# yjh0410/YOLO-Nano

Measured on NVIDIA B200. Metric: images/sec YOLO-Nano-1.0x 416 bs256 fp32-parity e2e (backbone+neck+head+decode+NMS), higher is better.
Workload: dtype f32 (tcgen05 3xTF32 split, fp32 accumulate)

## Files before the change

yolo_nano_b200/csrc/common.cuh:

```cuda
#pragma once
#include <cuda_bf16.h>
#include <cuda_runtime.h>
#include <stdint.h>
#include <limits.h>
#include <stdlib.h>

#include "yolonano_b200.h"

namespace ynb {

constexpr int kNumSMs = 148;

__device__ __forceinline__ float apply_act(float v, int act) {
  if (act == YNB_ACT_RELU) return fmaxf(v, 0.0f);
  if (act == YNB_ACT_LEAKY) return v > 0.0f ? v : 0.1f * v;
  return v;
}

__device__ __forceinline__ float softmax_exp(float d) { return __expf(d); }
__device__ __forceinline__ float class_score(float sum, float obj) { return __fmul_rn(__fdiv_rn(1.0f, sum), obj); }

struct ChanMap {
  int gap_at;
  int gap;
  __host__ __device__ __forceinline__ int slot(int j) const { return j + (j >= gap_at ? gap : 0); }
};
__host__ __device__ inline ChanMap dense_map() { return ChanMap{INT_MAX, 0}; }

using bf16 = __nv_bfloat16;

__device__ __forceinline__ float4 load4(const float* p) { return *reinterpret_cast<const float4*>(p); }
__device__ __forceinline__ float4 load4(const bf16* p) {
  const uint2 u = *reinterpret_cast<const uint2*>(p);
  return make_float4(__uint_as_float(u.x << 16), __uint_as_float(u.x & 0xffff0000u), __uint_as_float(u.y << 16),
                     __uint_as_float(u.y & 0xffff0000u));
}
__device__ __forceinline__ uint32_t pack_bf16x2(float lo, float hi) {
  const __nv_bfloat162 v = __floats2bfloat162_rn(lo, hi);
  return *reinterpret_cast<const uint32_t*>(&v);
}
__device__ __forceinline__ void store4(float* p, float4 v) { *reinterpret_cast<float4*>(p) = v; }
__device__ __forceinline__ void store4(bf16* p, float4 v) {
  *reinterpret_cast<uint2*>(p) = make_uint2(pack_bf16x2(v.x, v.y), pack_bf16x2(v.z, v.w));
}
__device__ __forceinline__ float to_float(float v) { return v; }
__device__ __forceinline__ float to_float(bf16 v) { return __bfloat162float(v); }

inline int round_up(int v, int m) { return (v + m - 1) / m * m; }
inline int64_t round_up64(int64_t v, int64_t m) { return (v + m - 1) / m * m; }

struct LaunchCounter {
  int64_t n = 0;
};
extern thread_local LaunchCounter* g_counter;

__device__ __forceinline__ void pdl_trigger() { asm volatile("griddepcontrol.launch_dependents;" ::: "memory"); }
__device__ __forceinline__ void pdl_wait() { asm volatile("griddepcontrol.wait;" ::: "memory"); }

inline bool pdl_enabled() {
  static int v = -1;
  if (v < 0) v = getenv("YNB_NO_PDL") ? 0 : 1;
  return v == 1;
}

template <typename... KArgs, typename... Args>
inline cudaError_t launch_pdl(void (*kern)(KArgs...), dim3 grid, dim3 block, size_t smem, cudaStream_t st,
                              Args&&... args) {
  cudaLaunchConfig_t cfg{};
  cfg.gridDim = grid;
  cfg.blockDim = block;
  cfg.dynamicSmemBytes = smem;
  cfg.stream = st;
  cudaLaunchAttribute attr[1];
  attr[0].id = cudaLaunchAttributeProgrammaticStreamSerialization;
  attr[0].val.programmaticStreamSerializationAllowed = 1;
  cfg.attrs = attr;
  cfg.numAttrs = pdl_enabled() ? 1 : 0;
  return cudaLaunchKernelEx(&cfg, kern, static_cast<KArgs>(args)...);
}

#define YNB_COUNT_LAUNCH()                  \
  do {                                      \
    if (::ynb::g_counter) ::ynb::g_counter->n++; \
  } while (0)

}
```

yolo_nano_b200/csrc/gemm_tc.cuh:

```cuda
#pragma once
#include <cuda.h>

#include <cstring>

#include "common.cuh"
#include "ptx_sm100.cuh"

namespace ynb {

constexpr int kTcThreads = 512;
constexpr int kTcSplitWarp0 = 8, kTcProducerWarp = 12, kTcMmaWarp = 13;
constexpr int kTcProducers = 3;
constexpr int kTcBM = 128;
constexpr int kTcBK = 32;
constexpr int kTcAStageBytes = kTcBM * 128;
constexpr int kTcMaxStages = 8;
constexpr int kTcSmemBudget = 232448;
constexpr int kTcMaxMain = 4;

struct TcGemmParams {
  int num_steps;
  int chunks_per_tap;
  int is3x3;
  int mode;
  int bf16_in;
  int out_bf16;
  int num_stages;
  int w_resident;
  int64_t M;
  int64_t num_tiles;
  int H, W, TH, TW, tiles_x, tiles_y;
  int N, Npad;
  int nmain;
  int nacc;
  int merge_corr;
  int ksub;
  int presplit;
  int a2_step;
  int stack_b;
  int acc_stages;
  uint32_t tmem_cols;
  uint32_t a_box_bytes;
  float* out;
  int out_ld, out_off, out_step;
  ChanMap omap;
  const float* bias;
  int act;
  const float* pass;
  int pass_ld;
  int tma_store;
  struct Decode {
    float* boxes;
    float* scores;
    int32_t* cls;
    int G, HW;
    float stride, input_size;
    float aw[3], ah[3];
    int64_t Ntot, level_off;
  } dec;
  int* err_flag;
  long long* trace;
  int trace_cap;
};

#define YNB_TRACE(role, a, b)                                                                        \
  do {                                                                                               \
    if (p.trace != nullptr && blockIdx.x == 0) {                                                     \
      const int _lt = (int)(((long long)(a) - (long long)blockIdx.x) / (long long)gridDim.x) & 63;   \
      long long* _e = p.trace + 1 + (long long)((((role) * 64 + _lt) * 32) + ((int)(b) & 31)) * 4;   \
      _e[0] = (role); _e[1] = (a); _e[2] = (b); _e[3] = clock64();                                   \
    }                                                                                                \
  } while (0)

struct TcSmemLayout {
  uint32_t stage_bytes;
  uint32_t w_chunk_bytes;
  uint32_t w_res_off;
  uint32_t bias_off;
  uint32_t stg_off;
  uint32_t bar_off;
  uint32_t total;
};
constexpr int kTcStgBytes = 8 * 4096;

__host__ __device__ inline TcSmemLayout tc_smem_layout(int Npad, int num_steps, int num_stages, bool w_resident,
                                                       bool split) {
  TcSmemLayout L;
  L.w_chunk_bytes = (uint32_t)Npad * 128;
  uint32_t a_bytes = kTcAStageBytes * (split ? 2 : 1);
  uint32_t w_bytes = w_resident ? 0 : L.w_chunk_bytes * (split ? 2 : 1);
  L.stage_bytes = a_bytes + w_bytes;
  L.w_res_off = L.stage_bytes * num_stages;
  uint32_t w_res = w_resident ? L.w_chunk_bytes * (split ? 2 : 1) * num_steps : 0;
  L.bias_off = L.w_res_off + w_res;
  L.stg_off = L.bias_off + 1024;
  L.bar_off = L.stg_off + kTcStgBytes;
  L.total = L.bar_off + 256 + 1024;
  return L;
}

__host__ __device__ __forceinline__ uint32_t rn_tf32_bits(uint32_t u) { return (u + 0x1000u) & 0xffffe000u; }

template <bool kPass, int kDecC>
__global__ void __launch_bounds__(kTcThreads, 1)
tc_gemm_kernel(const __grid_constant__ CUtensorMap tmA, const __grid_constant__ CUtensorMap tmAlo,
               const __grid_constant__ CUtensorMap tmWhi, const __grid_constant__ CUtensorMap tmWlo,
               const __grid_constant__ CUtensorMap tmOut, const TcGemmParams p) {
  extern __shared__ __align__(16) uint8_t smem_raw[];
  uint8_t* smem = smem_raw + ((1024u - (ptx::smem_u32(smem_raw) & 1023u)) & 1023u);

  const bool split = p.mode == YNB_GEMM_TC_3XTF32;
  const int kchunk = p.bf16_in ? 64 : kTcBK;
  const int box_alo = p.presplit ? 1 : -1;
  const int box_whi = p.w_resident ? -1 : 1 + (p.presplit ? 1 : 0);
  const int box_wlo = (p.w_resident || !split) ? -1 : box_whi + 1;
  const int nboxes = 1 + (box_alo >= 0) + (box_whi >= 0) + (box_wlo >= 0);
  const int nprod = nboxes < kTcProducers ? nboxes : kTcProducers;
  const TcSmemLayout lay = tc_smem_layout(p.Npad, p.num_steps, p.num_stages, p.w_resident != 0, split);
  const uint32_t w_chunk_bytes = lay.w_chunk_bytes;
  const uint32_t a_bytes = kTcAStageBytes * (split ? 2 : 1);
  const uint32_t stage_bytes = lay.stage_bytes;
  const uint32_t w_res_bytes = lay.bias_off - lay.w_res_off;
  float* s_bias = reinterpret_cast<float*>(smem + lay.bias_off);
  uint64_t* bars = reinterpret_cast<uint64_t*>(smem + lay.bar_off);
  uint64_t* full = bars;
  uint64_t* ready = bars + kTcMaxStages;
  uint64_t* empty = bars + 2 * kTcMaxStages;
  uint64_t* tmem_full = bars + 3 * kTcMaxStages;
  uint64_t* tmem_empty = bars + 3 * kTcMaxStages + 2;
  uint64_t* w_full = bars + 3 * kTcMaxStages + 4;
  uint32_t* tmem_ptr = reinterpret_cast<uint32_t*>(bars + 3 * kTcMaxStages + 5);

  const int warp = threadIdx.x >> 5, lane = threadIdx.x & 31;
  pdl_trigger();

  if (warp == kTcProducerWarp && lane == 0) {
    ptx::prefetch_tmap(&tmA);
    if (p.presplit || p.a2_step > 0) ptx::prefetch_tmap(&tmAlo);
    ptx::prefetch_tmap(&tmWhi);
    if (split) ptx::prefetch_tmap(&tmWlo);
    if (p.tma_store) ptx::prefetch_tmap(&tmOut);
    for (int s = 0; s < p.num_stages; ++s) {
      ptx::mbar_init(&full[s], nprod);
      ptx::mbar_init(&ready[s], 4);
      ptx::mbar_init(&empty[s], 1);
    }
    for (int a = 0; a < 2; ++a) {
      ptx::mbar_init(&tmem_full[a], 1);
      ptx::mbar_init(&tmem_empty[a], 4);
    }
    ptx::mbar_init(w_full, 1);
    ptx::fence_barrier_init();
  }
  if (warp == kTcMmaWarp) {
    ptx::tmem_alloc(tmem_ptr, p.tmem_cols);
    ptx::tmem_relinquish();
  }
  if (warp < 4) {
    for (int i = threadIdx.x; i < p.Npad; i += 128) s_bias[i] = i < p.N ? __ldg(p.bias + i) : 0.0f;
  }
  ptx::tc_fence_before_sync();
  __syncthreads();
  ptx::tc_fence_after_sync();
  const uint32_t tmem_base = *tmem_ptr;

  auto stage_a = [&](int s) { return smem + (size_t)s * stage_bytes; };
  auto stage_alo = [&](int s) { return smem + (size_t)s * stage_bytes + kTcAStageBytes; };
  auto w_hi_ptr = [&](int s, int step) {
    return p.w_resident ? smem + lay.w_res_off + (size_t)step * w_chunk_bytes * (split ? 2 : 1)
                        : smem + (size_t)s * stage_bytes + a_bytes;
  };
  auto w_lo_ptr = [&](int s, int step) { return w_hi_ptr(s, step) + w_chunk_bytes; };

  const int acc_cols = p.Npad * p.nacc;
  const uint32_t step_tx = p.a_box_bytes * (p.presplit ? 2 : 1) + (p.w_resident ? 0 : w_chunk_bytes * (split ? 2 : 1));
  const bool splitters_on = split && !p.presplit;

  if (warp == kTcProducerWarp && p.w_resident && ptx::elect_one()) {
    ptx::mbar_arrive_expect_tx(w_full, w_res_bytes);
    for (int st = 0; st < p.num_steps; ++st) {
      ptx::tma_load_2d(w_hi_ptr(0, st), &tmWhi, w_full, st * kchunk, 0);
      if (split) ptx::tma_load_2d(w_lo_ptr(0, st), &tmWlo, w_full, st * kchunk, 0);
    }
  }
  pdl_wait();

  const int prole = warp == kTcProducerWarp ? 0 : (warp == 14 ? 1 : (warp == 15 ? 2 : -1));
  if (prole >= 0) {
    if (prole < nprod && ptx::elect_one()) {
      const bool do_a = 0 % nprod == prole;
      const bool do_alo = box_alo >= 0 && box_alo % nprod == prole;
      const bool do_whi = box_whi >= 0 && box_whi % nprod == prole;
      const bool do_wlo = box_wlo >= 0 && box_wlo % nprod == prole;
      const uint32_t my_tx = (do_a ? p.a_box_bytes : 0u) + (do_alo ? p.a_box_bytes : 0u) +
                             (do_whi ? w_chunk_bytes : 0u) + (do_wlo ? w_chunk_bytes : 0u);
      int s = 0;
      uint32_t ph = 0;
      bool ok = true;
      for (int64_t tile = blockIdx.x; tile < p.num_tiles && ok; tile += gridDim.x) {
        int b = 0, y0 = 0, x0 = 0;
        if (p.is3x3) {
          int per_img = p.tiles_x * p.tiles_y;
          b = (int)(tile / per_img);
          int r = (int)(tile - (int64_t)b * per_img);
          y0 = (r / p.tiles_x) * p.TH;
          x0 = (r % p.tiles_x) * p.TW;
        }
        for (int st = 0; st < p.num_steps; ++st) {
          ok = ptx::mbar_wait(&empty[s], ph ^ 1, p.err_flag, 1);
          if (!ok) break;
          ptx::mbar_arrive_expect_tx(&full[s], my_tx);
          if (p.is3x3) {
            int tap = st / p.chunks_per_tap, kc = st - tap * p.chunks_per_tap;
            int dy = tap / 3, dx = tap - dy * 3;
            if (do_a) ptx::tma_load_4d(stage_a(s), &tmA, &full[s], kc * kchunk, x0 + dx - 1, y0 + dy - 1, b);
            if (do_alo) ptx::tma_load_4d(stage_alo(s), &tmAlo, &full[s], kc * kchunk, x0 + dx - 1, y0 + dy - 1, b);
          } else {
            if (do_a) {
              const bool second = p.a2_step > 0 && st >= p.a2_step;
              ptx::tma_load_2d(stage_a(s), second ? &tmAlo : &tmA, &full[s], (second ? st - p.a2_step : st) * kchunk,
                               (int)(tile * kTcBM));
            }
          }
          if (do_whi) ptx::tma_load_2d(w_hi_ptr(s, st), &tmWhi, &full[s], st * kchunk, 0);
          if (do_wlo) ptx::tma_load_2d(w_lo_ptr(s, st), &tmWlo, &full[s], st * kchunk, 0);
          if (prole == 0) YNB_TRACE(1, tile, st);
          if (++s == p.num_stages) { s = 0; ph ^= 1; }
        }
      }
    }
  } else if (warp == kTcMmaWarp) {
    if (ptx::elect_one()) {
      const uint32_t idesc = ptx::make_idesc(2 , kTcBM, p.Npad);
      const uint32_t idesc2 = ptx::make_idesc(2, kTcBM, 2 * p.Npad);
      const uint32_t idesc_bf = ptx::make_idesc(1 , kTcBM, p.Npad);
      int s = 0;
      uint32_t ph = 0;
      int acc = 0;
      uint32_t acc_ph = 0;
      bool ok = true;
      if (p.w_resident) ok = ptx::mbar_wait(w_full, 0, p.err_flag, 2);
      for (int64_t tile = blockIdx.x; tile < p.num_tiles && ok; tile += gridDim.x) {
        ok = ptx::mbar_wait(&tmem_empty[acc], acc_ph ^ 1, p.err_flag, 3);
        if (!ok) break;
        ptx::tc_fence_after_sync();
        const uint32_t d_tmem = tmem_base + (uint32_t)(acc * acc_cols);
        const uint32_t c_tmem = p.merge_corr ? d_tmem : d_tmem + (uint32_t)(p.nmain * p.Npad);
        int t = 0;
        for (int st = 0; st < p.num_steps; ++st) {
          ok = ptx::mbar_wait(splitters_on ? &ready[s] : &full[s], ph, p.err_flag, 4);
          if (!ok) break;
          ptx::tc_fence_after_sync();
          const uint32_t a_hi = ptx::smem_u32(stage_a(s));
          const uint32_t a_lo = ptx::smem_u32(stage_alo(s));
          const uint32_t b_hi = ptx::smem_u32(w_hi_ptr(s, st));
          const uint32_t b_lo = ptx::smem_u32(w_lo_ptr(s, st));
          const int nk = p.ksub > 0 ? min(kTcBK / 8, p.ksub - st * (kTcBK / 8)) : kTcBK / 8;
          if (p.bf16_in) {
#pragma unroll
            for (int k = 0; k < kTcBK / 8; ++k, ++t) {
              if (k >= nk) break;
              ptx::mma_bf16_ss(d_tmem, ptx::make_sw128_kmajor_desc(a_hi + k * 32), ptx::make_sw128_kmajor_desc(b_hi + k * 32),
                               idesc_bf, t != 0);
            }
          } else if (p.stack_b) {
#pragma unroll
            for (int k = 0; k < kTcBK / 8; ++k, ++t) {
              if (k >= nk) break;
              const uint64_t db = ptx::make_sw128_kmajor_desc(b_hi + k * 32);
              ptx::mma_tf32_ss(d_tmem, ptx::make_sw128_kmajor_desc(a_hi + k * 32), db, idesc2, t != 0);
              ptx::mma_tf32_ss(c_tmem, ptx::make_sw128_kmajor_desc(a_lo + k * 32), db, idesc, 1);
            }
          } else {
#pragma unroll
            for (int k = 0; k < kTcBK / 8; ++k, ++t) {
              if (k >= nk) break;
              const uint32_t ko = k * 32;
              const uint64_t da = ptx::make_sw128_kmajor_desc(a_hi + ko);
              const uint64_t db = ptx::make_sw128_kmajor_desc(b_hi + ko);
              const int slot = t % p.nmain;
              if (split) {
                ptx::mma_tf32_ss(c_tmem, ptx::make_sw128_kmajor_desc(a_lo + ko), db, idesc, t != 0);
                ptx::mma_tf32_ss(c_tmem, da, ptx::make_sw128_kmajor_desc(b_lo + ko), idesc, 1);
              }
              ptx::mma_tf32_ss(d_tmem + (uint32_t)(slot * p.Npad), da, db, idesc,
                               (split && p.merge_corr) ? 1 : (t >= p.nmain));
            }
          }
          YNB_TRACE(3, tile, st);
          ptx::mma_commit(&empty[s]);
          if (st == p.num_steps - 1) ptx::mma_commit(&tmem_full[acc]);
          if (++s == p.num_stages) { s = 0; ph ^= 1; }
        }
        if (++acc == p.acc_stages) { acc = 0; acc_ph ^= 1; }
      }
    }
  } else if (warp >= kTcSplitWarp0 && warp < kTcSplitWarp0 + 4) {
    if (splitters_on) {
      const int t = threadIdx.x - kTcSplitWarp0 * 32;
      int s = 0;
      uint32_t ph = 0;
      bool ok = true;
      for (int64_t tile = blockIdx.x; tile < p.num_tiles && ok; tile += gridDim.x) {
        for (int st = 0; st < p.num_steps; ++st) {
          ok = ptx::mbar_wait(&full[s], ph, p.err_flag, 5);
          if (!ok) break;
          uint4* a = reinterpret_cast<uint4*>(stage_a(s));
          uint4* lo = reinterpret_cast<uint4*>(stage_alo(s));
#pragma unroll
          for (int i = 0; i < kTcAStageBytes / 16 / 128; ++i) {
            const uint4 v = a[t + i * 128];
            uint4 h, l;
            h.x = rn_tf32_bits(v.x); h.y = rn_tf32_bits(v.y); h.z = rn_tf32_bits(v.z); h.w = rn_tf32_bits(v.w);
            l.x = rn_tf32_bits(__float_as_uint(__uint_as_float(v.x) - __uint_as_float(h.x)));
            l.y = rn_tf32_bits(__float_as_uint(__uint_as_float(v.y) - __uint_as_float(h.y)));
            l.z = rn_tf32_bits(__float_as_uint(__uint_as_float(v.z) - __uint_as_float(h.z)));
            l.w = rn_tf32_bits(__float_as_uint(__uint_as_float(v.w) - __uint_as_float(h.w)));
            a[t + i * 128] = h;
            lo[t + i * 128] = l;
          }
          ptx::fence_proxy_async_smem();
          __syncwarp();
          if (lane == 0) ptx::mbar_arrive(&ready[s]);
          if (t == 0) YNB_TRACE(2, tile, st);
          if (++s == p.num_stages) { s = 0; ph ^= 1; }
        }
      }
    }
  } else if (warp < 8) {
    const int group = warp >> 2;
    const int q = warp & 3;
    const int row = q * 32 + lane;
    const bool vec = p.out_step == 1 && p.omap.gap == 0;
    const float slope = p.act == YNB_ACT_RELU ? 0.0f : (p.act == YNB_ACT_LEAKY ? 0.1f : 1.0f);
    uint8_t* sbox = smem + lay.stg_off + warp * 4096;
    const int sw = lane & 7;
    const int nloc = (int64_t)blockIdx.x < p.num_tiles
                         ? (int)((p.num_tiles - blockIdx.x + gridDim.x - 1) / gridDim.x) : 0;
    const bool share_last = kDecC == 0;
    const int col_split = min(p.Npad, ((p.Npad / 2 + 31) / 32) * 32);
    bool ok = true;
    for (int lt = 0; lt < nloc && ok; ++lt) {
      const int64_t tile = blockIdx.x + (int64_t)lt * gridDim.x;
      const int acc = p.acc_stages == 2 ? (lt & 1) : 0;
      const bool shared = share_last && lt == nloc - 1 && col_split < p.Npad;
      if (!shared && group != acc) {
        if (p.acc_stages == 1 && share_last) ok = ptx::mbar_wait(&tmem_full[0], (uint32_t)(lt & 1), p.err_flag, 7);
        continue;
      }
      const int col_begin = shared && group == 1 ? col_split : 0;
      const int col_end = shared && group == 0 ? col_split : p.Npad;
      const uint32_t acc_ph = (uint32_t)((lt / p.acc_stages) & 1);
      int64_t m;
      bool valid;
      if (p.is3x3) {
        int per_img = p.tiles_x * p.tiles_y;
        int b = (int)(tile / per_img);
        int r = (int)(tile - (int64_t)b * per_img);
        int y = (r / p.tiles_x) * p.TH + row / p.TW;
        int x = (r % p.tiles_x) * p.TW + row % p.TW;
        valid = row < p.TH * p.TW && y < p.H && x < p.W;
        m = ((int64_t)b * p.H + y) * p.W + x;
      } else {
        m = tile * kTcBM + row;
        valid = m < p.M;
      }
      const int64_t m_base = tile * kTcBM + q * 32;
      float xa[16], xb[16];
      const int rows_left = (int)min((int64_t)32, p.M - m_base);
      auto fetch_x1 = [&](int c0, int r0, float (&x)[16]) {
        const int i = c0 + lane;
        const bool col_ok = kPass && i < p.N;
        const float* src = p.pass + (m_base + r0) * (int64_t)p.pass_ld + i;
        const int nr = col_ok ? rows_left - r0 : 0;
#pragma unroll
        for (int r = 0; r < 16; ++r) x[r] = r < nr ? __ldg(src + r * p.pass_ld) : 0.0f;
      };
      if (kPass) {
        fetch_x1(col_begin, 0, xa);
        fetch_x1(col_begin, 16, xb);
      }
      if (lane == 0 && q == 0) YNB_TRACE(4, tile, group);
      ok = ptx::mbar_wait(&tmem_full[acc], acc_ph, p.err_flag, 6);
      if (!ok) break;
      ptx::tc_fence_after_sync();
      if (lane == 0 && q == 0) YNB_TRACE(6, tile, group);
      const uint32_t t_base = tmem_base + ((uint32_t)(q * 32) << 16) + (uint32_t)(acc * acc_cols);
      if constexpr (kDecC > 0) {
        constexpr int A = 3, C = kDecC, CB = (C + 15) / 16;
        auto ld16 = [&](int c0, float (&v)[16]) {
          uint32_t r[16];
          ptx::tmem_ld_32x16(t_base + c0, r);
          if (p.nacc > 1) {
            for (int a2 = 1; a2 < p.nacc; ++a2) {
              uint32_t r2[16];
              ptx::tmem_ld_32x16(t_base + (uint32_t)(a2 * p.Npad) + c0, r2);
              ptx::tmem_ld_wait();
#pragma unroll
              for (int jj = 0; jj < 16; ++jj) r[jj] = __float_as_uint(__uint_as_float(r[jj]) + __uint_as_float(r2[jj]));
            }
          }
          ptx::tmem_ld_wait();
#pragma unroll
          for (int jj = 0; jj < 16; ++jj) v[jj] = __uint_as_float(r[jj]);
        };
        float objl[A], mx[A], sum[A], tb[4 * A];
        int am[A];
        {
          float v[16];
          ld16(0, v);
#pragma unroll
          for (int a = 0; a < A; ++a) objl[a] = v[a] + s_bias[a];
          constexpr int NPADC = (A * (1 + C + 4) + 15) / 16 * 16;
          constexpr int B0 = (A + A * C) < (NPADC - 16) ? (A + A * C) : (NPADC - 16);
          constexpr int BOFF = A + A * C - B0;
          ld16(B0, v);
#pragma unroll
          for (int k = 0; k < 4 * A; ++k) tb[k] = v[BOFF + k] + s_bias[A + A * C + k];
        }
#pragma unroll
        for (int a = 0; a < A; ++a) {
          const int cbase = A + a * C;
          float m = -INFINITY;
          int arg = 0;
#pragma unroll 1
          for (int blk = 0; blk < CB; ++blk) {
            float v[16];
            ld16(cbase + blk * 16, v);
            const float* bb = s_bias + cbase + blk * 16;
#pragma unroll
            for (int jj = 0; jj < 16; ++jj) {
              const int c = blk * 16 + jj;
              const float x = v[jj] + bb[jj];
              if ((C % 16 == 0 || c < C) && x > m) { m = x; arg = c; }
            }
          }
          float sm = 0.0f;
#pragma unroll 1
          for (int blk = 0; blk < CB; ++blk) {
            float v[16];
            ld16(cbase + blk * 16, v);
            const float* bb = s_bias + cbase + blk * 16;
#pragma unroll
            for (int jj = 0; jj < 16; ++jj) {
              const int c = blk * 16 + jj;
              if (C % 16 == 0 || c < C) sm += softmax_exp((v[jj] + bb[jj]) - m);
            }
          }
          mx[a] = m; am[a] = arg; sum[a] = sm;
        }
        (void)mx;
        {
          ptx::tc_fence_before_sync();
          __syncwarp();
          if (lane == 0) ptx::mbar_arrive(&tmem_empty[acc]);
        }
        if (valid) {
          const int b = (int)(m / p.dec.HW);
          const int pix = (int)(m - (int64_t)b * p.dec.HW);
          const int gy = pix / p.dec.G, gx = pix - gy * p.dec.G;
          const int64_t o0 = (int64_t)b * p.dec.Ntot + p.dec.level_off + (int64_t)pix * A;
#pragma unroll
          for (int a = 0; a < A; ++a) {
            const float obj = 1.0f / (1.0f + expf(-objl[a]));
            const float score = class_score(sum[a], obj);
            const float tx = tb[4 * a], ty = tb[4 * a + 1], tw = tb[4 * a + 2], th = tb[4 * a + 3];
            float cx = __fmul_rn(__fadd_rn(1.0f / (1.0f + expf(-tx)), (float)gx), p.dec.stride);
            float cy = __fmul_rn(__fadd_rn(1.0f / (1.0f + expf(-ty)), (float)gy), p.dec.stride);
            float w = __fmul_rn(expf(tw), p.dec.aw[a]);
            float h = __fmul_rn(expf(th), p.dec.ah[a]);
            float hw = __fmul_rn(w, 0.5f), hh = __fmul_rn(h, 0.5f);
            float x1 = __fdiv_rn(__fsub_rn(cx, hw), p.dec.input_size);
            float y1 = __fdiv_rn(__fsub_rn(cy, hh), p.dec.input_size);
            float x2 = __fdiv_rn(__fadd_rn(cx, hw), p.dec.input_size);
            float y2 = __fdiv_rn(__fadd_rn(cy, hh), p.dec.input_size);
            reinterpret_cast<float4*>(p.dec.boxes)[o0 + a] =
                make_float4(fminf(fmaxf(x1, 0.f), 1.f), fminf(fmaxf(y1, 0.f), 1.f), fminf(fmaxf(x2, 0.f), 1.f),
                            fminf(fmaxf(y2, 0.f), 1.f));
            p.dec.scores[o0 + a] = score;
            p.dec.cls[o0 + a] = am[a];
          }
        }
        if (lane == 0 && q == 0) YNB_TRACE(5, tile, group);
        continue;
      }
      auto box_free = [&]() {
        if (p.tma_store) {
          if (ptx::elect_one()) ptx::bulk_wait_read<0>();
          __syncwarp();
        }
      };
      auto drain16 = [&](int c0, int jc) {
        uint32_t r[16];
        ptx::tmem_ld_32x16(t_base + c0, r);
        if (p.nacc == 2) {
          uint32_t r2[16];
          ptx::tmem_ld_32x16(t_base + (uint32_t)p.Npad + c0, r2);
          ptx::tmem_ld_wait();
#pragma unroll
          for (int j = 0; j < 16; ++j) r[j] = __float_as_uint(__uint_as_float(r[j]) + __uint_as_float(r2[j]));
        } else if (p.nacc > 2) {
          for (int a = 1; a < p.nacc; ++a) {
            uint32_t r2[16];
            ptx::tmem_ld_32x16(t_base + (uint32_t)(a * p.Npad) + c0, r2);
            ptx::tmem_ld_wait();
#pragma unroll
            for (int j = 0; j < 16; ++j) r[j] = __float_as_uint(__uint_as_float(r[j]) + __uint_as_float(r2[j]));
          }
        } else {
          ptx::tmem_ld_wait();
        }
        if (jc == 0) box_free();
#pragma unroll
        for (int j = 0; j < 4; ++j) {
          const float4 b4 = *reinterpret_cast<const float4*>(s_bias + c0 + 4 * j);
          float x0 = __uint_as_float(r[4 * j]) + b4.x, x1 = __uint_as_float(r[4 * j + 1]) + b4.y;
          float x2 = __uint_as_float(r[4 * j + 2]) + b4.z, x3 = __uint_as_float(r[4 * j + 3]) + b4.w;
          *reinterpret_cast<float4*>(sbox + lane * 128 + (((jc + j) ^ sw) << 4)) =
              make_float4(fmaxf(x0, x0 * slope), fmaxf(x1, x1 * slope), fmaxf(x2, x2 * slope), fmaxf(x3, x3 * slope));
        }
      };
      auto staged = [&](int r, int l) {
        return *reinterpret_cast<const float*>(sbox + r * 128 + ((((l >> 2) ^ (r & 7)) << 4) | ((l & 3) << 2)));
      };

      auto drain16_bf16 = [&](int c0, int half) {
        uint32_t r[16];
        ptx::tmem_ld_32x16(t_base + c0, r);
        ptx::tmem_ld_wait();
        if (half == 0) box_free();
        uint32_t w[8];
#pragma unroll
        for (int j = 0; j < 8; ++j) {
          float x0 = __uint_as_float(r[2 * j]) + s_bias[c0 + 2 * j], x1 = __uint_as_float(r[2 * j + 1]) + s_bias[c0 + 2 * j + 1];
          w[j] = pack_bf16x2(fmaxf(x0, x0 * slope), fmaxf(x1, x1 * slope));
        }
        uint4* dst = reinterpret_cast<uint4*>(sbox + lane * 64 + half * 32);
        dst[0] = make_uint4(w[0], w[1], w[2], w[3]);
        dst[1] = make_uint4(w[4], w[5], w[6], w[7]);
      };
      const bool bf16_box = p.out_bf16 && p.tma_store && !kPass;
      bf16* const out_bf = reinterpret_cast<bf16*>(p.out);

      for (int c0 = col_begin; c0 < col_end; c0 += 32) {
        if (bf16_box) {
          drain16_bf16(c0, 0);
          if (c0 + 16 < col_end) drain16_bf16(c0 + 16, 1);
        } else {
          drain16(c0, 0);
          if (c0 + 16 < col_end) drain16(c0 + 16, 4);
        }
        if (c0 + 32 >= col_end && !shared) {
          ptx::tc_fence_before_sync();
          __syncwarp();
          if (lane == 0) ptx::mbar_arrive(&tmem_empty[acc]);
        }
        if (!kPass && p.tma_store) {
          ptx::fence_proxy_async_smem();
          __syncwarp();
          if (ptx::elect_one()) {
            ptx::tma_store_2d(&tmOut, sbox, c0, (int)m_base);
            ptx::bulk_commit();
          }
          continue;
        }
        __syncwarp();
        const int i = c0 + lane;
        const bool col_ok = i < p.N;
        if (kPass) {
          const int nrow = col_ok ? (int)min((int64_t)32, p.M - m_base) : 0;
          float* o = p.out + m_base * p.out_ld + p.omap.slot(2 * (col_ok ? i : 0));
#pragma unroll
          for (int r = 0; r < 16; ++r, o += p.out_ld)
            if (r < nrow) *reinterpret_cast<float2*>(o) = make_float2(xa[r], staged(r, lane));
          if (c0 + 32 < col_end) fetch_x1(c0 + 32, 0, xa);
#pragma unroll
          for (int r = 16; r < 32; ++r, o += p.out_ld)
            if (r < nrow) *reinterpret_cast<float2*>(o) = make_float2(xb[r - 16], staged(r, lane));
          if (c0 + 32 < col_end) fetch_x1(c0 + 32, 16, xb);
        } else {
          const int col = vec ? p.out_off + i : p.omap.slot(p.out_off + (col_ok ? i : 0) * p.out_step);
          if (!p.is3x3) {
            const int nrow = col_ok ? (int)min((int64_t)32, p.M - m_base) : 0;
            if (p.out_bf16) {
              bf16* o = out_bf + m_base * p.out_ld + col;
#pragma unroll 8
              for (int r = 0; r < 32; ++r, o += p.out_ld)
                if (r < nrow) *o = __float2bfloat16_rn(staged(r, lane));
            } else {
              float* o = p.out + m_base * p.out_ld + col;
#pragma unroll 8
              for (int r = 0; r < 32; ++r, o += p.out_ld)
                if (r < nrow) *o = staged(r, lane);
            }
          } else {
            const int64_t off = valid ? m * p.out_ld : -1;
#pragma unroll 8
            for (int r = 0; r < 32; ++r) {
              const int64_t offr = __shfl_sync(0xffffffffu, off, r);
              if (col_ok && offr >= 0) {
                if (p.out_bf16) out_bf[offr + col] = __float2bfloat16_rn(staged(r, lane));
                else p.out[offr + col] = staged(r, lane);
              }
            }
          }
        }
        __syncwarp();
      }
      if (lane == 0 && q == 0) YNB_TRACE(5, tile, group);
    }
    __syncwarp();
    if (p.tma_store && ptx::elect_one()) ptx::bulk_wait<0>();
  }

  ptx::tc_fence_before_sync();
  __syncthreads();
  if (warp == kTcMmaWarp) {
    ptx::tc_fence_after_sync();
    ptx::tmem_dealloc(tmem_base, p.tmem_cols);
  }
}

typedef CUresult (*PFN_encodeTiled)(CUtensorMap*, CUtensorMapDataType, cuuint32_t, void*, const cuuint64_t*,
                                    const cuuint64_t*, const cuuint32_t*, const cuuint32_t*,
                                    CUtensorMapInterleave, CUtensorMapSwizzle, CUtensorMapL2promotion,
                                    CUtensorMapFloatOOBfill);

inline PFN_encodeTiled get_encode_tiled() {
  static PFN_encodeTiled fn = nullptr;
  if (!fn) {
    void* p = nullptr;
    cudaDriverEntryPointQueryResult qres;
    if (cudaGetDriverEntryPoint("cuTensorMapEncodeTiled", &p, cudaEnableDefault, &qres) == cudaSuccess &&
        qres == cudaDriverEntryPointSuccess)
      fn = reinterpret_cast<PFN_encodeTiled>(p);
  }
  return fn;
}

inline bool make_tmap_2d(CUtensorMap* m, const void* base, uint64_t k, uint64_t rows, uint64_t row_stride_elems,
                         uint32_t box_rows, bool bf16 = false) {
  PFN_encodeTiled enc = get_encode_tiled();
  if (!enc) return false;
  const uint64_t es = bf16 ? 2 : 4;
  cuuint64_t dims[2] = {k, rows};
  cuuint64_t strides[1] = {row_stride_elems * es};
  cuuint32_t box[2] = {(cuuint32_t)(128 / es), box_rows};
  cuuint32_t estr[2] = {1, 1};
  return enc(m, bf16 ? CU_TENSOR_MAP_DATA_TYPE_BFLOAT16 : CU_TENSOR_MAP_DATA_TYPE_FLOAT32, 2, const_cast<void*>(base), dims,
             strides, box, estr, CU_TENSOR_MAP_INTERLEAVE_NONE, CU_TENSOR_MAP_SWIZZLE_128B,
             CU_TENSOR_MAP_L2_PROMOTION_L2_128B, CU_TENSOR_MAP_FLOAT_OOB_FILL_NONE) == CUDA_SUCCESS;
}

inline bool make_tmap_nhwc(CUtensorMap* m, const void* base, int C, int W, int H, int B, int ld, int box_w,
                           int box_h, bool bf16 = false, bool swizzle = true) {
  PFN_encodeTiled enc = get_encode_tiled();
  if (!enc) return false;
  const uint64_t es = bf16 ? 2 : 4;
  cuuint64_t dims[4] = {(cuuint64_t)C, (cuuint64_t)W, (cuuint64_t)H, (cuuint64_t)B};
  cuuint64_t strides[3] = {(cuuint64_t)ld * es, (cuuint64_t)ld * es * W, (cuuint64_t)ld * es * W * H};
  cuuint32_t box[4] = {(cuuint32_t)(128 / es), (cuuint32_t)box_w, (cuuint32_t)box_h, 1};
  cuuint32_t estr[4] = {1, 1, 1, 1};
  return enc(m, bf16 ? CU_TENSOR_MAP_DATA_TYPE_BFLOAT16 : CU_TENSOR_MAP_DATA_TYPE_FLOAT32, 4, const_cast<void*>(base), dims,
             strides, box, estr, CU_TENSOR_MAP_INTERLEAVE_NONE,
             swizzle ? CU_TENSOR_MAP_SWIZZLE_128B : CU_TENSOR_MAP_SWIZZLE_NONE,
             CU_TENSOR_MAP_L2_PROMOTION_L2_128B, CU_TENSOR_MAP_FLOAT_OOB_FILL_NONE) == CUDA_SUCCESS;
}

inline bool make_tmap_stem_input(CUtensorMap* m, const float* x, int S, int B) {
  PFN_encodeTiled enc = get_encode_tiled();
  if (!enc || (reinterpret_cast<uintptr_t>(x) & 15u) || (S & 3)) return false;
  cuuint64_t dims[4] = {(cuuint64_t)S, (cuuint64_t)S, 3, (cuuint64_t)B};
  cuuint64_t strides[3] = {(cuuint64_t)S * 4, (cuuint64_t)S * S * 4, (cuuint64_t)S * S * 12};
  cuuint32_t box[4] = {40, 35, 3, 1};
  cuuint32_t estr[4] = {1, 1, 1, 1};
  return enc(m, CU_TENSOR_MAP_DATA_TYPE_FLOAT32, 4, const_cast<float*>(x), dims, strides, box, estr,
             CU_TENSOR_MAP_INTERLEAVE_NONE, CU_TENSOR_MAP_SWIZZLE_NONE, CU_TENSOR_MAP_L2_PROMOTION_L2_128B,
             CU_TENSOR_MAP_FLOAT_OOB_FILL_NONE) == CUDA_SUCCESS;
}

inline bool make_tmap_out(CUtensorMap* m, void* base, uint64_t cols, uint64_t rows, uint64_t ld, bool bf16 = false) {
  PFN_encodeTiled enc = get_encode_tiled();
  if (!enc) return false;
  const uint64_t es = bf16 ? 2 : 4;
  cuuint64_t dims[2] = {cols, rows};
  cuuint64_t strides[1] = {ld * es};
  cuuint32_t box[2] = {32, 32};
  cuuint32_t estr[2] = {1, 1};
  return enc(m, bf16 ? CU_TENSOR_MAP_DATA_TYPE_BFLOAT16 : CU_TENSOR_MAP_DATA_TYPE_FLOAT32, 2, base, dims, strides, box,
             estr, CU_TENSOR_MAP_INTERLEAVE_NONE, bf16 ? CU_TENSOR_MAP_SWIZZLE_NONE : CU_TENSOR_MAP_SWIZZLE_128B,
             CU_TENSOR_MAP_L2_PROMOTION_NONE, CU_TENSOR_MAP_FLOAT_OOB_FILL_NONE) == CUDA_SUCCESS;
}

struct TcWeights {
  float* hi = nullptr;
  float* lo = nullptr;
  bf16* bw = nullptr;
  int N = 0, Npad = 0, Kpad = 0;
  CUtensorMap tm_hi, tm_lo;
};

inline void split_tf32_host(float v, float* hi, float* lo) {
  uint32_t u;
  memcpy(&u, &v, 4);
  uint32_t h = rn_tf32_bits(u);
  float hf;
  memcpy(&hf, &h, 4);
  float l = v - hf;
  uint32_t lu;
  memcpy(&lu, &l, 4);
  lu = rn_tf32_bits(lu);
  memcpy(lo, &lu, 4);
  *hi = hf;
}

struct TcGemmLaunch {
  CUtensorMap tmA;
  CUtensorMap tmOut;
  const TcWeights* w = nullptr;
  CUtensorMap tmAlo;
  TcGemmParams p;
  uint32_t smem = 0;
  unsigned grid = 0;
  int dec_classes = 0;
};

inline void tc_plan_tmem(TcGemmParams& p, bool allow_merge = false) {
  const bool split = p.mode == YNB_GEMM_TC_3XTF32;
  p.merge_corr = 0;
  static const bool merge_all = getenv("YNB_TC_MERGE_ALL") != nullptr;
  if (split && ((allow_merge && p.num_steps * (kTcBK / 8) <= 16) || merge_all) && 2 * p.Npad <= 512) {
    p.merge_corr = 1;
    p.stack_b = 0;
    p.nmain = 1; p.nacc = 1; p.acc_stages = 2;
    p.tmem_cols = 32;
    while ((int)p.tmem_cols < 2 * p.Npad) p.tmem_cols <<= 1;
    return;
  }
  const int corr = split ? 1 : 0;
  int want = 1;
  if (split) {
    const int ksteps = p.num_steps * (kTcBK / 8);
    want = ksteps >= 64 ? 4 : (ksteps >= 24 ? 3 : (ksteps >= 12 ? 2 : 1));
    static const int nmain_cap = getenv("YNB_TC_NMAIN_MAX") ? atoi(getenv("YNB_TC_NMAIN_MAX")) : 1;
    if (want > nmain_cap) want = nmain_cap;
  }
  p.nmain = want;
  while (p.nmain > 1 && (p.nmain + corr) * p.Npad > 512) p.nmain--;
  p.nacc = p.nmain + corr;
  p.acc_stages = 2 * p.nacc * p.Npad <= 512 ? 2 : 1;
  if (p.acc_stages == 1 && want <= 2 && p.nmain > 1 && 2 * (p.nmain - 1 + corr) * p.Npad <= 512) {
    p.nmain--;
    p.nacc--;
    p.acc_stages = 2;
  }
  p.tmem_cols = 32;
  while ((int)p.tmem_cols < p.acc_stages * p.nacc * p.Npad) p.tmem_cols <<= 1;
  static const bool no_stack = getenv("YNB_TC_NO_STACK") != nullptr;
  p.stack_b = (split && !no_stack && p.nmain == 1 && p.nacc == 2 && 2 * p.Npad <= 256 && (2 * p.Npad) % 16 == 0) ? 1 : 0;
}

inline bool tc_plan_smem(TcGemmLaunch& L) {
  TcGemmParams& p = L.p;
  const bool split = p.mode == YNB_GEMM_TC_3XTF32;
  for (int resident = 1; resident >= 0; --resident) {
    for (int stages = kTcMaxStages; stages >= 2; --stages) {
      if (stages > p.num_steps * 4 && stages > 2) continue;
      TcSmemLayout lay = tc_smem_layout(p.Npad, p.num_steps, stages, resident != 0, split);
      static const bool res2 = getenv("YNB_TC_RES2") != nullptr;
      if (lay.total <= (uint32_t)kTcSmemBudget && (resident == 0 || stages >= 3 || p.num_steps <= 2 || res2)) {
        p.num_stages = stages;
        p.w_resident = resident;
        L.smem = lay.total;
        return true;
      }
    }
  }
  return false;
}

inline cudaError_t launch_tc_gemm(const TcGemmLaunch& L, cudaStream_t st) {
  using KernelT = void (*)(CUtensorMap, CUtensorMap, CUtensorMap, CUtensorMap, CUtensorMap, TcGemmParams);
  static const KernelT kernels[4] = {tc_gemm_kernel<false, 0>, tc_gemm_kernel<true, 0>, tc_gemm_kernel<false, 80>,
                                     tc_gemm_kernel<false, 20>};
  static bool attr_set = false;
  if (!attr_set) {
    for (KernelT k : kernels) {
      cudaError_t e = cudaFuncSetAttribute(k, cudaFuncAttributeMaxDynamicSharedMemorySize, kTcSmemBudget);
      if (e != cudaSuccess) return e;
    }
    attr_set = true;
  }
  const CUtensorMap& tmo = L.p.tma_store ? L.tmOut : L.tmA;
  KernelT kern = L.dec_classes == 80 ? kernels[2] : (L.dec_classes == 20 ? kernels[3] : kernels[L.p.pass != nullptr ? 1 : 0]);
  const CUtensorMap& tmalo = (L.p.presplit || L.p.a2_step > 0) ? L.tmAlo : L.tmA;
  cudaError_t r = launch_pdl(kern, dim3(L.grid), dim3(kTcThreads), (size_t)L.smem, st, L.tmA, tmalo, L.w->tm_hi,
                             L.w->tm_lo, tmo, L.p);
  YNB_COUNT_LAUNCH();
  return r;
}

inline void tc_pick_tile(int H, int W, int* TH, int* TW) {
  double best = -1;
  for (int tw = 4; tw <= 64 && tw <= W + 3; ++tw) {
    int th = 128 / tw;
    if (th < 1) continue;
    if (th > H) th = H;
    double eff = (double)H * W / ((double)((W + tw - 1) / tw) * ((H + th - 1) / th) * 128.0);
    if (eff > best + 1e-9) { best = eff; *TH = th; *TW = tw; }
  }
}

}
```

yolo_nano_b200/csrc/ptx_sm100.cuh:

```cuda
#pragma once
#include <cuda.h>
#include <cuda_runtime.h>
#include <stdint.h>

namespace ynb {
namespace ptx {

__device__ __forceinline__ uint32_t smem_u32(const void* p) {
  return (uint32_t)__cvta_generic_to_shared(p);
}

__device__ __forceinline__ void mbar_init(uint64_t* bar, uint32_t count) {
  asm volatile("mbarrier.init.shared::cta.b64 [%0], %1;" ::"r"(smem_u32(bar)), "r"(count));
}
__device__ __forceinline__ void fence_barrier_init() {
  asm volatile("fence.mbarrier_init.release.cluster;" ::: "memory");
}
__device__ __forceinline__ void mbar_arrive(uint64_t* bar) {
  asm volatile("mbarrier.arrive.shared::cta.b64 _, [%0];" ::"r"(smem_u32(bar)) : "memory");
}
__device__ __forceinline__ void mbar_arrive_expect_tx(uint64_t* bar, uint32_t bytes) {
  asm volatile("mbarrier.arrive.expect_tx.shared::cta.b64 _, [%0], %1;" ::"r"(smem_u32(bar)), "r"(bytes)
               : "memory");
}
__device__ __forceinline__ bool mbar_try_wait(uint64_t* bar, uint32_t parity) {
  uint32_t ok;
  asm volatile(
      "{\n\t.reg .pred p;\n\t"
      "mbarrier.try_wait.parity.shared::cta.b64 p, [%1], %2;\n\t"
      "selp.u32 %0, 1, 0, p;\n\t}"
      : "=r"(ok)
      : "r"(smem_u32(bar)), "r"(parity)
      : "memory");
  return ok != 0;
}
__device__ __forceinline__ uint64_t globaltimer_ns() {
  uint64_t t;
  asm volatile("mov.u64 %0, %%globaltimer;" : "=l"(t));
  return t;
}
__device__ __forceinline__ bool mbar_wait(uint64_t* bar, uint32_t parity, int* timeout_flag, int code) {
  uint64_t t0 = 0;
#pragma unroll 1
  for (uint32_t spin = 0;; ++spin) {
    if (mbar_try_wait(bar, parity)) return true;
    if ((spin & 4095u) == 4095u) {
      const uint64_t now = globaltimer_ns();
      if (t0 == 0) t0 = now;
      else if (now - t0 > 2000000000ull) break;
    }
  }
  if (timeout_flag) atomicCAS(timeout_flag, 0, code);
  return false;
}

__device__ __forceinline__ void fence_proxy_async_smem() {
  asm volatile("fence.proxy.async.shared::cta;" ::: "memory");
}
__device__ __forceinline__ void tc_fence_before_sync() {
  asm volatile("tcgen05.fence::before_thread_sync;" ::: "memory");
}
__device__ __forceinline__ void tc_fence_after_sync() {
  asm volatile("tcgen05.fence::after_thread_sync;" ::: "memory");
}

__device__ __forceinline__ void prefetch_tmap(const CUtensorMap* m) {
  asm volatile("prefetch.tensormap [%0];" ::"l"(reinterpret_cast<uint64_t>(m)) : "memory");
}
__device__ __forceinline__ void tma_load_2d(void* smem_dst, const CUtensorMap* m, uint64_t* bar, int c0, int c1) {
  asm volatile(
      "cp.async.bulk.tensor.2d.shared::cluster.global.mbarrier::complete_tx::bytes [%0], [%1, {%3, %4}], [%2];"
      ::"r"(smem_u32(smem_dst)), "l"(reinterpret_cast<uint64_t>(m)), "r"(smem_u32(bar)), "r"(c0), "r"(c1)
      : "memory");
}
__device__ __forceinline__ void tma_load_4d(void* smem_dst, const CUtensorMap* m, uint64_t* bar, int c0, int c1,
                                            int c2, int c3) {
  asm volatile(
      "cp.async.bulk.tensor.4d.shared::cluster.global.mbarrier::complete_tx::bytes [%0], [%1, {%3, %4, %5, %6}], [%2];"
      ::"r"(smem_u32(smem_dst)), "l"(reinterpret_cast<uint64_t>(m)), "r"(smem_u32(bar)), "r"(c0), "r"(c1),
      "r"(c2), "r"(c3)
      : "memory");
}

__device__ __forceinline__ void tma_prefetch_4d(const CUtensorMap* m, int c0, int c1, int c2, int c3) {
  asm volatile("cp.async.bulk.prefetch.tensor.4d.L2.global.tile [%0, {%1, %2, %3, %4}];"
               ::"l"(reinterpret_cast<uint64_t>(m)), "r"(c0), "r"(c1), "r"(c2), "r"(c3)
               : "memory");
}

__device__ __forceinline__ void cp_async_16(void* smem_dst, const void* gsrc, uint32_t src_bytes) {
  asm volatile("cp.async.cg.shared.global [%0], [%1], 16, %2;" ::"r"(smem_u32(smem_dst)), "l"(gsrc), "r"(src_bytes)
               : "memory");
}
__device__ __forceinline__ void cp_async_commit() { asm volatile("cp.async.commit_group;" ::: "memory"); }
__device__ __forceinline__ void cp_async_wait_all() { asm volatile("cp.async.wait_group 0;" ::: "memory"); }

__device__ __forceinline__ void tma_store_2d(const CUtensorMap* m, const void* smem_src, int c0, int c1) {
  asm volatile("cp.async.bulk.tensor.2d.global.shared::cta.bulk_group [%0, {%2, %3}], [%1];"
               ::"l"(reinterpret_cast<uint64_t>(m)), "r"(smem_u32(smem_src)), "r"(c0), "r"(c1)
               : "memory");
}
__device__ __forceinline__ void tma_store_4d(const CUtensorMap* m, const void* smem_src, int c0, int c1, int c2, int c3) {
  asm volatile("cp.async.bulk.tensor.4d.global.shared::cta.bulk_group [%0, {%2, %3, %4, %5}], [%1];"
               ::"l"(reinterpret_cast<uint64_t>(m)), "r"(smem_u32(smem_src)), "r"(c0), "r"(c1), "r"(c2), "r"(c3)
               : "memory");
}
__device__ __forceinline__ void bulk_commit() { asm volatile("cp.async.bulk.commit_group;" ::: "memory"); }
template <int N>
__device__ __forceinline__ void bulk_wait_read() {
  asm volatile("cp.async.bulk.wait_group.read %0;" ::"n"(N) : "memory");
}
template <int N>
__device__ __forceinline__ void bulk_wait() {
  asm volatile("cp.async.bulk.wait_group %0;" ::"n"(N) : "memory");
}

__device__ __forceinline__ void tmem_alloc(uint32_t* smem_result, uint32_t ncols) {
  asm volatile("tcgen05.alloc.cta_group::1.sync.aligned.shared::cta.b32 [%0], %1;" ::"r"(smem_u32(smem_result)),
               "r"(ncols)
               : "memory");
}
__device__ __forceinline__ void tmem_relinquish() {
  asm volatile("tcgen05.relinquish_alloc_permit.cta_group::1.sync.aligned;" ::: "memory");
}
__device__ __forceinline__ void tmem_dealloc(uint32_t taddr, uint32_t ncols) {
  asm volatile("tcgen05.dealloc.cta_group::1.sync.aligned.b32 %0, %1;" ::"r"(taddr), "r"(ncols) : "memory");
}

__device__ __forceinline__ uint64_t make_sw128_kmajor_desc(uint32_t smem_addr) {
  uint64_t d = 0;
  d |= (uint64_t)((smem_addr & 0x3FFFF) >> 4);
  d |= (uint64_t)1 << 16;
  d |= (uint64_t)(1024 >> 4) << 32;
  d |= (uint64_t)1 << 46;
  d |= (uint64_t)2 << 61;
  return d;
}
__host__ __device__ __forceinline__ uint32_t make_idesc(int fmt, int M, int N) {
  return (1u << 4) | ((uint32_t)fmt << 7) | ((uint32_t)fmt << 10) | ((uint32_t)(N >> 3) << 17) |
         ((uint32_t)(M >> 4) << 24);
}
__device__ __forceinline__ void mma_tf32_ss(uint32_t tmem_d, uint64_t adesc, uint64_t bdesc, uint32_t idesc,
                                            uint32_t accumulate) {
  asm volatile(
      "{\n\t.reg .pred p;\n\t"
      "setp.ne.b32 p, %4, 0;\n\t"
      "tcgen05.mma.cta_group::1.kind::tf32 [%0], %1, %2, %3, p;\n\t}"
      ::"r"(tmem_d), "l"(adesc), "l"(bdesc), "r"(idesc), "r"(accumulate)
      : "memory");
}
__device__ __forceinline__ void mma_bf16_ss(uint32_t tmem_d, uint64_t adesc, uint64_t bdesc, uint32_t idesc,
                                            uint32_t accumulate) {
  asm volatile(
      "{\n\t.reg .pred p;\n\t"
      "setp.ne.b32 p, %4, 0;\n\t"
      "tcgen05.mma.cta_group::1.kind::f16 [%0], %1, %2, %3, p;\n\t}"
      ::"r"(tmem_d), "l"(adesc), "l"(bdesc), "r"(idesc), "r"(accumulate)
      : "memory");
}
__device__ __forceinline__ void mma_commit(uint64_t* bar) {
  asm volatile("tcgen05.commit.cta_group::1.mbarrier::arrive::one.shared::cluster.b64 [%0];" ::"r"(smem_u32(bar))
               : "memory");
}

__device__ __forceinline__ void tmem_ld_32x32(uint32_t taddr, uint32_t (&r)[32]) {
  asm volatile(
      "tcgen05.ld.sync.aligned.32x32b.x32.b32 "
      "{%0, %1, %2, %3, %4, %5, %6, %7, %8, %9, %10, %11, %12, %13, %14, %15, "
      "%16, %17, %18, %19, %20, %21, %22, %23, %24, %25, %26, %27, %28, %29, %30, %31}, [%32];"
      : "=r"(r[0]), "=r"(r[1]), "=r"(r[2]), "=r"(r[3]), "=r"(r[4]), "=r"(r[5]), "=r"(r[6]), "=r"(r[7]),
        "=r"(r[8]), "=r"(r[9]), "=r"(r[10]), "=r"(r[11]), "=r"(r[12]), "=r"(r[13]), "=r"(r[14]), "=r"(r[15]),
        "=r"(r[16]), "=r"(r[17]), "=r"(r[18]), "=r"(r[19]), "=r"(r[20]), "=r"(r[21]), "=r"(r[22]), "=r"(r[23]),
        "=r"(r[24]), "=r"(r[25]), "=r"(r[26]), "=r"(r[27]), "=r"(r[28]), "=r"(r[29]), "=r"(r[30]), "=r"(r[31])
      : "r"(taddr)
      : "memory");
}
__device__ __forceinline__ void tmem_ld_32x16(uint32_t taddr, uint32_t (&r)[16]) {
  asm volatile(
      "tcgen05.ld.sync.aligned.32x32b.x16.b32 "
      "{%0, %1, %2, %3, %4, %5, %6, %7, %8, %9, %10, %11, %12, %13, %14, %15}, [%16];"
      : "=r"(r[0]), "=r"(r[1]), "=r"(r[2]), "=r"(r[3]), "=r"(r[4]), "=r"(r[5]), "=r"(r[6]), "=r"(r[7]),
        "=r"(r[8]), "=r"(r[9]), "=r"(r[10]), "=r"(r[11]), "=r"(r[12]), "=r"(r[13]), "=r"(r[14]), "=r"(r[15])
      : "r"(taddr)
      : "memory");
}
__device__ __forceinline__ void tmem_ld_wait() {
  asm volatile("tcgen05.wait::ld.sync.aligned;" ::: "memory");
}

__device__ __forceinline__ void named_bar_sync(int id, int nthreads) {
  asm volatile("bar.sync %0, %1;" ::"r"(id), "r"(nthreads) : "memory");
}

template <int N>
__device__ __forceinline__ void setmaxnreg_inc() {
  asm volatile("setmaxnreg.inc.sync.aligned.u32 %0;" ::"n"(N));
}
template <int N>
__device__ __forceinline__ void setmaxnreg_dec() {
  asm volatile("setmaxnreg.dec.sync.aligned.u32 %0;" ::"n"(N));
}

__device__ __forceinline__ bool elect_one() {
  uint32_t pred;
  asm volatile(
      "{\n\t.reg .pred p;\n\t"
      "elect.sync _|p, 0xffffffff;\n\t"
      "selp.u32 %0, 1, 0, p;\n\t}"
      : "=r"(pred));
  return pred != 0;
}

}
}
```

yolo_nano_b200/csrc/ynb_api.cu:

```cuda
#include <cuda.h>
#include <cuda_runtime.h>

#include <cmath>
#include <cstdio>
#include <cstdlib>
#include <cstring>
#include <deque>
#include <functional>
#include <map>
#include <memory>
#include <string>
#include <tuple>
#include <vector>

#include "yolonano_b200.h"

#include "common.cuh"
#include "decode_nms.cuh"
#include "nms_grid.cuh"
#include "gemm_ffma.cuh"
#include "gemm_tc.cuh"
#include "unit_tc.cuh"
#include "kernels_basic.cuh"
#include "train_ops.cuh"
// ... 257 lines not shown
  for (int i = 0; i < h; ++i) {
    const int r1 = sl.map.slot(2 * i), r2 = sl.map.slot(2 * i + 1);
    for (int k = 0; k < c1.cin; ++k) w[(size_t)r1 * ktot + il1.map.slot(k)] = p1.w_host[(size_t)i * c1.cin + k];
    for (int k = 0; k < c2.cin; ++k) w[(size_t)r2 * ktot + k1p + il2.map.slot(k)] = p2.w_host[(size_t)i * c2.cin + k];
    b[r1] = p1.b_host[i];
    b[r2] = p2.b_host[i];
  }
  const int parts = (sl.ld + 239) / 240;
  const int npart = round_up((sl.ld + parts - 1) / parts, bf ? 8 : 4);
  for (auto& cc : e->cat[si]) {
    if (cc.pc.b_dev) cudaFree(cc.pc.b_dev);
    if (cc.pc.tc.hi) cudaFree(cc.pc.tc.hi);
    if (cc.pc.tc.lo) cudaFree(cc.pc.tc.lo);
    if (cc.pc.tc.bw) cudaFree(cc.pc.tc.bw);
  }
  e->cat[si].clear();
  e->cat[si].resize(parts);
  for (int pi = 0; pi < parts; ++pi) {
    ynb_engine::CatConv& cc = e->cat[si][pi];
    cc.n0 = pi * npart;
    const int n = std::min(npart, sl.ld - cc.n0);
    cc.k1p = k1p; cc.k2p = k2p;
    cc.pc.n = n; cc.pc.ktot = ktot; cc.pc.loaded = true;
    CUDA_TRY(e, cudaMalloc(&cc.pc.b_dev, round_up(n, 4) * 4));
    CUDA_TRY(e, cudaMemset(cc.pc.b_dev, 0, round_up(n, 4) * 4));
    CUDA_TRY(e, cudaMemcpy(cc.pc.b_dev, b.data() + cc.n0, n * 4, cudaMemcpyHostToDevice));
    int rc = pack_tc_matrix(e, cc.pc.tc, w.data() + (size_t)cc.n0 * ktot, n, ktot, 1, bk + "cat");
    if (rc) return rc;
  }
  return YNB_OK;
}

int pack_conv(ynb_engine* e, int i) {
  const ConvSpec& c = e->table[i];
  PackedConv& pc = e->convs[i];
  const bool bf = is_bf16(e);
  InLayout il = in_layout(c, bf);
  std::vector<float> w, b;
  if (c.kind == kDense3x3 && c.cin == 3) {
    w.assign(27 * 24, 0.f);
    for (int co = 0; co < 24; ++co)
      for (int ci = 0; ci < 3; ++ci)
        for (int t = 0; t < 9; ++t) w[(ci * 9 + t) * 24 + co] = pc.w_host[(co * 3 + ci) * 9 + t];
    b = pc.b_host;
    pc.n = 24; pc.ktot = 27;
    memcpy(e->stem_w.w, w.data(), sizeof(e->stem_w.w));
    memcpy(e->stem_w.b, b.data(), sizeof(e->stem_w.b));
  } else if (c.kind == kDw3x3) {
    int c4 = il.ktot;
    w.assign(9 * c4, 0.f);
    b.assign(c4, 0.f);
    for (int ch = 0; ch < c.cin; ++ch) {
      int s = il.map.slot(ch);
      for (int t = 0; t < 9; ++t) w[t * c4 + s] = pc.w_host[ch * 9 + t];
      b[s] = pc.b_host[ch];
    }
    pc.n = c4; pc.ktot = 9;
  } else if (c.kind == kPw1x1) {
    w.assign((size_t)c.cout * il.ktot, 0.f);
    for (int n = 0; n < c.cout; ++n)
      for (int k = 0; k < c.cin; ++k) w[(size_t)n * il.ktot + il.map.slot(k)] = pc.w_host[(size_t)n * c.cin + k];
    b = pc.b_host;
    pc.n = c.cout; pc.ktot = il.ktot;
  } else {
    w.assign((size_t)c.cout * 9 * c.cin, 0.f);
    for (int n = 0; n < c.cout; ++n)
      for (int ci = 0; ci < c.cin; ++ci)
        for (int t = 0; t < 9; ++t)
          w[((size_t)n * 9 + t) * c.cin + ci] = pc.w_host[((size_t)n * c.cin + ci) * 9 + t];
    b = pc.b_host;
    pc.n = c.cout; pc.ktot = 9 * c.cin;
  }
  if (pc.w_dev) cudaFree(pc.w_dev);
  if (pc.b_dev) cudaFree(pc.b_dev);
  pc.w_dev = pc.b_dev = nullptr;
  CUDA_TRY(e, cudaMalloc(&pc.w_dev, w.size() * 4));
  CUDA_TRY(e, cudaMalloc(&pc.b_dev, round_up((int)b.size(), 4) * 4));
  CUDA_TRY(e, cudaMemcpy(pc.w_dev, w.data(), w.size() * 4, cudaMemcpyHostToDevice));
  CUDA_TRY(e, cudaMemset(pc.b_dev, 0, round_up((int)b.size(), 4) * 4));
  CUDA_TRY(e, cudaMemcpy(pc.b_dev, b.data(), b.size() * 4, cudaMemcpyHostToDevice));

  if ((c.kind == kPw1x1) || (c.kind == kDense3x3 && c.cin != 3)) {
    int rc = pack_tc_matrix(e, pc.tc, w.data(), pc.n, pc.ktot, c.kind == kDense3x3 ? 9 : 1, c.name);
    if (rc) return rc;
  }
  return YNB_OK;
}

struct Bump {
  size_t off = 0;
  size_t take(size_t bytes) {
    size_t o = off;
    off += (bytes + 1023) & ~(size_t)1023;
    return o;
  }
};

size_t layout_workspace(ynb_engine* e, int batch, int S, char* base) {
  Bump bump;
  const bool bf = is_bf16(e);
  const int es_act = bf ? 2 : 4, al = bf ? 8 : 4;
  auto tensor = [&](const std::string& name, int C, int ld, int H, ChanMap map = dense_map(), int es = 0) {
    Tensor t;
    t.es = es ? es : es_act;
    t.C = C; t.ld = ld; t.H = H; t.W = H; t.map = map;
    size_t o = bump.take((size_t)batch * H * H * ld * t.es);
    t.p = base ? reinterpret_cast<float*>(base + o) : nullptr;
    e->taps[name] = t;
    return t;
  };
  e->taps.clear();
  const int H1 = S / 4;
  tensor("pool", 24, 24, H1);
  int hin = H1;
  int ld_in = 24;
  ChanMap map_in = dense_map();
  for (int si = 0; si < 3; ++si) {
    int cout = stage_channels()[si + 1], h = cout / 2, cin = stage_channels()[si];
    int hout = hin / 2;
    std::string st = "stage" + std::to_string(si + 2);
    const StageLayout sl = stage_layout(bf, si);
    int ld_h = round_up(h, al);
    tensor(st + ".b1dw", cin, ld_in, hout, map_in);
    tensor(st + ".b2pw", h, ld_h, hin);
    tensor(st + ".mid1", h, ld_h, hout);
    tensor(st + ".mid2", h, ld_h, hout);
    for (int bi = 0; bi < stage_repeats()[si]; ++bi) tensor(st + "." + std::to_string(bi), cout, sl.ld, hout, sl.map);
    hin = hout;
    ld_in = sl.ld;
    map_in = sl.map;
  }
  const int H3 = S / 8, H4 = S / 16, H5 = S / 32;
  const int hs[3] = {H3, H4, H5};
  for (int l = 0; l < 3; ++l) tensor("lat" + std::to_string(l + 3), 96, 96, hs[l]);
  tensor("sum4", 96, 96, H4); tensor("sum4.lo", 96, 96, H4); tensor("fpn4", 96, 96, H4);
  tensor("sum3", 96, 96, H3); tensor("sum3.lo", 96, 96, H3); tensor("p3", 96, 96, H3);
  tensor("sum4b", 96, 96, H4); tensor("sum4b.lo", 96, 96, H4); tensor("p4", 96, 96, H4);
  tensor("sum5", 96, 96, H5); tensor("sum5.lo", 96, 96, H5); tensor("p5", 96, 96, H5);
  const int ch = e->cfg.num_anchors * (1 + e->cfg.num_classes + 4);
  const char* pn[3] = {"pred_s", "pred_m", "pred_l"};
  for (int l = 0; l < 3; ++l) {
    tensor("head" + std::to_string(l) + ".a", 96, 96, hs[l]);
    tensor("head" + std::to_string(l) + ".b", 96, 96, hs[l]);
    tensor("head" + std::to_string(l) + ".c", 96, 96, hs[l]);
    e->raw[l] = tensor(pn[l], ch, round_up(ch, 4), hs[l], dense_map(), 4);
  }
  e->taps["c3"] = e->taps["stage2.3"];
  e->taps["c4"] = e->taps["stage3.7"];
  e->taps["c5"] = e->taps["stage4.3"];

  int64_t n = 0;
  for (int s : {8, 16, 32}) n += (int64_t)e->cfg.num_anchors * (S / s) * (S / s);
  auto raw = [&](size_t bytes) { size_t o = bump.take(bytes); return base ? base + o : nullptr; };
  e->d_boxes = (float*)raw((size_t)batch * n * 16);
  e->d_scores = (float*)raw((size_t)batch * n * 4);
  e->d_cls = (int32_t*)raw((size_t)batch * n * 4);
  e->nms_ws_bytes = std::max(nms_workspace_bytes(batch, n), grid_nms_workspace_bytes(batch, n));
  e->d_nms_ws = raw((size_t)e->nms_ws_bytes);
  for (int k = 0; k < 2; ++k) {
    e->slot[k].x = (float*)raw((size_t)batch * 3 * S * S * 4);
    e->slot[k].boxes = (float*)raw((size_t)batch * n * 16);
    e->slot[k].scores = (float*)raw((size_t)batch * n * 4);
    e->slot[k].cls = (int32_t*)raw((size_t)batch * n * 4);
    e->slot[k].counts = (int32_t*)raw((size_t)batch * 4);
    e->slot[k].img_u8 = (uint8_t*)raw((size_t)batch * 3 * S * S);
    e->slot[k].rects = (int32_t*)raw((size_t)batch * 16);
  }
  e->d_x = e->slot[0].x;
  e->d_out_boxes = e->slot[0].boxes;
  e->d_out_scores = e->slot[0].scores;
  e->d_out_cls = e->slot[0].cls;
  e->d_out_counts = e->slot[0].counts;
  e->d_err = (int*)raw(256);
  return bump.off;
}

int ensure_workspace(ynb_engine* e, int batch) {
  if (e->ws && e->ws_batch >= batch && e->ws_S == e->S) return YNB_OK;
  int nb = std::max(batch, std::max(e->ws_batch, (int)e->cfg.max_batch));
  CUDA_TRY(e, cudaDeviceSynchronize());
  e->plans.clear();
  e->tc_store.clear(); e->dp_store.clear(); e->dw_maps.clear(); e->stem_maps.clear();
  for (auto& kv : e->graphs) cudaGraphExecDestroy(kv.second);
  e->graphs.clear();
  e->graph_seen.clear();
  if (e->ws) { cudaFree(e->ws); e->ws = nullptr; }
  size_t bytes = layout_workspace(e, nb, e->S, nullptr);
  CUDA_TRY(e, cudaMalloc(&e->ws, bytes));
  CUDA_TRY(e, cudaMemset(e->ws, 0, bytes));
  layout_workspace(e, nb, e->S, e->ws);
  e->ws_bytes = bytes;
  e->ws_batch = nb;
  e->ws_S = e->S;
  return YNB_OK;
}

struct Planner {
  ynb_engine* e;
  int B;
  Plan* plan;
  std::deque<TcGemmLaunch>* tc;
  std::deque<DwPwLaunch>* dp;
  std::string error;
  std::vector<Op>* dst = nullptr;
  std::vector<Op>& ops() { return dst ? *dst : plan->net; }

  const PackedConv& conv(const std::string& name) const { return e->convs[e->index.at(name)]; }
  const ConvSpec& spec(const std::string& name) const { return e->table[e->index.at(name)]; }
  Tensor T(const std::string& name) const { return e->taps.at(name); }

  void dw(const std::string& name, const Tensor& in, int in_off, const Tensor& out) {
    const PackedConv& pc = conv(name);
    const ConvSpec& c = spec(name);
    int B_ = B, c4 = pc.n, stride = c.stride, act = c.act;
    const float *w = pc.w_dev, *b = pc.b_dev;
    double px_in = (double)B * in.H * in.W, px_out = (double)B * out.H * out.W;
    const bool bf = is_bf16(e);
    const double bytes = (double)in.es * c.cin * (px_in + px_out) + 40.0 * c.cin, flops = 18.0 * c.cin * px_out;
    static const bool no_tma = getenv("YNB_DW_NO_TMA") != nullptr;
    e->dw_maps.emplace_back();
    CUtensorMap* tm = &e->dw_maps.back();
    if ((!no_tma || bf) && make_tmap_dw(tm, in.p, in.ld, in_off, B, in.H, in.W, c4, stride, bf)) {
      plan->net.push_back({name, "dwconv3x3", bytes, flops, [=](cudaStream_t st) {
        return launch_dwconv3x3_tma(*tm, out.p, out.ld, 0, w, b, B_, in.H, in.W, c4, stride, act, st, false, bf);
      }});
      return;
    }
    if (bf) { error = "bf16 depthwise conv needs a 16-byte aligned view: " + name; return; }
    plan->net.push_back({name, "dwconv3x3", bytes, flops, [=](cudaStream_t st) {
      return launch_dwconv3x3(in.p, in.ld, in_off, out.p, out.ld, 0, w, b, B_, in.H, in.W, c4, stride, act, st);
    }});
  }

  void passthrough(const std::string& name, const Tensor& x, const Tensor& out, int half) {
    int64_t M = (int64_t)B * x.H * x.W;
    Tensor ps = x, o = out;
    Op op{name + "+passthrough", "interleave_copy", 8.0 * M * half, 0.0, [=](cudaStream_t st) {
      return launch_interleave_copy(ps.p, ps.ld, o.p, o.ld, o.map, M, half, st);
    }};
    op.side = true;
    plan->net.push_back(op);
  }

  void pw(const std::string& name, const Tensor& in, int in_off, const Tensor& out, int out_off, int out_step,
          bool join = false, const Tensor* pass = nullptr, const TcGemmParams::Decode* dec = nullptr) {
    const PackedConv& pc = conv(name);
    const ConvSpec& c = spec(name);
    int64_t M = (int64_t)B * in.H * in.W;
    const bool tc_mode = e->cfg.gemm_mode != YNB_GEMM_FP32_FFMA;
    const bool bf = is_bf16(e);
    const double abytes = (double)in.es * M * c.cin + (double)out.es * M * (c.cout + (pass && tc_mode ? 2.0 * c.cout : 0.0)) +
                          (bf ? 2.0 : 4.0) * c.cin * c.cout + 4.0 * c.cout;
    const double aflops = 2.0 * M * c.cin * c.cout;
    if (e->cfg.gemm_mode == YNB_GEMM_FP32_FFMA) {
      GemmParams g{};
      g.a = in.p; g.a_ld = in.ld; g.a_off = in_off; g.a2 = nullptr; g.a2_mode = 0;
      g.w = pc.w_dev; g.bias = pc.b_dev; g.out = out.p; g.out_ld = out.ld;
      g.out_off = out_off; g.out_step = out_step; g.omap = out.map;
      g.M = M; g.N = pc.n; g.Ktot = pc.ktot; g.act = c.act;
      if (pass) { g.out_off = 1; g.out_step = 2; }
      Op op{name, "pw_ffma", abytes, aflops, [=](cudaStream_t st) { return launch_gemm_ffma(g, false, st); }};
      op.join = join;
      ops().push_back(op);
      return;
    }
    tc->emplace_back();
    TcGemmLaunch& L = tc->back();
    L.w = &pc.tc;
    TcGemmParams& p = L.p;
    memset(&p, 0, sizeof(p));
    p.mode = e->cfg.gemm_mode;
    p.is3x3 = 0;
    p.bf16_in = bf ? 1 : 0;
    p.out_bf16 = out.es == 2 ? 1 : 0;
    if (bf && pass) { error = "bf16 mode: the pass-through GEMM epilogue is not built (unit tails go through dwpw): " + name; return; }
    p.num_steps = pc.tc.Kpad / (bf ? 64 : kTcBK);
    p.chunks_per_tap = p.num_steps;
    p.ksub = bf ? (pc.ktot + 15) / 16 : (pc.ktot + 7) / 8;
    p.M = M;
    p.num_tiles = (M + kTcBM - 1) / kTcBM;
    p.N = pc.n; p.Npad = pc.tc.Npad;
    tc_plan_tmem(p, name.size() > 2 && name.compare(0, 8, "head_det") == 0 && name.compare(name.size() - 2, 2, ".4") == 0);
    p.a_box_bytes = kTcAStageBytes;
    p.out = out.p; p.out_ld = out.ld; p.out_off = out_off; p.out_step = out_step; p.omap = out.map;
    p.bias = pc.b_dev; p.act = c.act;
    p.pass = pass ? pass->p : nullptr; p.pass_ld = pass ? pass->ld : 0;
    p.err_flag = e->d_err;
    if (dec) {
      p.dec = *dec;
      L.dec_classes = e->cfg.num_classes;
    }
    const int oal = 16 / out.es;
    p.tma_store = (!dec && !pass && out_step == 1 && out.map.gap == 0 && out_off % oal == 0 && out.ld % oal == 0) ? 1 : 0;
    if (p.tma_store && !make_tmap_out(&L.tmOut, out.at(out_off), (uint64_t)round_up(pc.n, oal), (uint64_t)M,
                                      (uint64_t)out.ld, out.es == 2)) {
      error = "cuTensorMapEncodeTiled failed for output of " + name;
      return;
    }
    if (!make_tmap_2d(&L.tmA, in.at(in_off), (uint64_t)pc.ktot, (uint64_t)M, (uint64_t)in.ld, kTcBM, bf)) {
      error = "cuTensorMapEncodeTiled failed for input of " + name;
      return;
    }
    if (!tc_plan_smem(L)) { error = "no smem configuration for " + name; return; }
    L.grid = (unsigned)std::min<int64_t>(p.num_tiles, kNumSMs);
    const TcGemmLaunch* Lp = &L;
    const double obytes = dec ? abytes - (double)out.es * M * c.cout + 24.0 * M * 3 : abytes;
    Op op{dec ? name + "+decode" : name, dec ? "pw_decode_tcgen05" : "pw_tcgen05", obytes, aflops,
          [=](cudaStream_t st) { return launch_tc_gemm(*Lp, st); }};
    op.join = join;
    ops().push_back(op);
  }

  bool catpw(int si, const std::string& unit, const Tensor& b1dw, const Tensor& mid2, const Tensor& out) {
    static const bool off = getenv("YNB_NO_CAT_GEMM") != nullptr;
    if (off || e->cfg.gemm_mode == YNB_GEMM_FP32_FFMA || e->cat[si].empty()) return false;
    const bool bf = is_bf16(e);
    const int64_t M = (int64_t)B * out.H * out.W;
    const ConvSpec& c1 = spec(unit + "branch1.2");
    const ConvSpec& c2 = spec(unit + "branch2.5");
    for (size_t pi = 0; pi < e->cat[si].size(); ++pi) {
      const ynb_engine::CatConv& cc = e->cat[si][pi];
      tc->emplace_back();
      TcGemmLaunch& L = tc->back();
      L.w = &cc.pc.tc;
      TcGemmParams& p = L.p;
      memset(&p, 0, sizeof(p));
      p.mode = e->cfg.gemm_mode;
      p.bf16_in = bf ? 1 : 0;
      p.out_bf16 = out.es == 2 ? 1 : 0;
      const int ch = bf ? 64 : kTcBK;
      p.num_steps = cc.pc.tc.Kpad / ch;
      p.chunks_per_tap = p.num_steps;
      p.a2_step = cc.k1p / ch;
      p.ksub = 0;
      p.M = M;
      p.num_tiles = (M + kTcBM - 1) / kTcBM;
      p.N = cc.pc.n; p.Npad = cc.pc.tc.Npad;
      tc_plan_tmem(p);
      p.a_box_bytes = kTcAStageBytes;
      p.out = out.p; p.out_ld = out.ld; p.out_off = cc.n0; p.out_step = 1; p.omap = dense_map();
      p.bias = cc.pc.b_dev; p.act = c1.act;
      p.err_flag = e->d_err;
      p.tma_store = 1;
      const int oal = 16 / out.es;
      if (!make_tmap_out(&L.tmOut, out.at(cc.n0), (uint64_t)round_up(cc.pc.n, oal), (uint64_t)M, (uint64_t)out.ld, out.es == 2) ||
          !make_tmap_2d(&L.tmA, b1dw.p, (uint64_t)b1dw.ld, (uint64_t)M, (uint64_t)b1dw.ld, kTcBM, bf) ||
          !make_tmap_2d(&L.tmAlo, mid2.p, (uint64_t)mid2.ld, (uint64_t)M, (uint64_t)mid2.ld, kTcBM, bf)) {
        error = "cuTensorMapEncodeTiled failed for the merged stride-2 conv of " + unit;
        return true;
      }
      if (!tc_plan_smem(L)) { error = "no smem configuration for the merged stride-2 conv of " + unit; return true; }
      L.grid = (unsigned)std::min<int64_t>(p.num_tiles, kNumSMs);
      const TcGemmLaunch* Lp = &L;
      const double frac = (double)cc.pc.n / out.ld;
      const double bytes = (double)b1dw.es * M * (c1.cin + c2.cin) + (double)out.es * M * 2.0 * c1.cout * frac +
                           (bf ? 2.0 : 4.0) * (c1.cin + c2.cin) * c1.cout;
      const double flops = 2.0 * M * (c1.cin + c2.cin) * c1.cout * frac;
      ops().push_back({unit + "branch1.2|branch2.5" + (e->cat[si].size() > 1 ? "." + std::to_string(pi) : ""), "pw_tcgen05", bytes,
                       flops, [=](cudaStream_t st) { return launch_tc_gemm(*Lp, st); }});
    }
    return true;
  }

  bool dwpw(const std::string& dw_name, const std::string& pw_name, const Tensor& in, const Tensor& out,
            const Tensor* pass) {
    static const bool off = getenv("YNB_NO_FUSED_DWPW") != nullptr;
    if (off || e->cfg.gemm_mode == YNB_GEMM_FP32_FFMA) return false;
    const PackedConv& dc = conv(dw_name);
    const PackedConv& pc = conv(pw_name);
    const ConvSpec& ds = spec(dw_name);
    const ConvSpec& ps = spec(pw_name);
    if (ds.stride != 1 || dc.n != pc.ktot) return false;
    dp->emplace_back();
    DwPwLaunch& L = dp->back();
    DwPwParams& p = L.p;
    memset(&p, 0, sizeof(p));
    p.dw_w = dc.w_dev; p.dw_b = dc.b_dev; p.dw_act = ds.act;
    p.out = out.p; p.out_ld = out.ld; p.out_off = 0; p.omap = out.map;
    p.bias = pc.b_dev; p.act = ps.act;
    p.pass = pass ? pass->p : nullptr; p.pass_ld = pass ? pass->ld : 0;
    p.err_flag = e->d_err;
    if (!plan_dwpw(L, in.p, in.ld, B, in.H, in.W, ds.cin, dc.n, &pc.tc, e->cfg.gemm_mode)) {
      dp->pop_back();
      return false;
    }
    const double M = (double)B * in.H * in.W;
    const double bytes = (double)in.es * M * (ds.cin + ps.cout * (pass ? 3.0 : 1.0)) + (double)in.es * ps.cin * ps.cout +
                         4.0 * ps.cout + 40.0 * ds.cin;
    const double flops = 2.0 * M * ps.cin * ps.cout + 18.0 * M * ds.cin;
    const DwPwLaunch* Lp = &L;
    ops().push_back({dw_name + "+pw", "dwpw_tcgen05", bytes, flops,
                     [=](cudaStream_t st) { return launch_dwpw_tc(*Lp, st); }});
    return true;
  }

  void conv3(const std::string& name, const Tensor& a, const Tensor* a2, int a2_mode, const Tensor& sum,
             const Tensor& sum_lo, const Tensor& out) {
    const PackedConv& pc = conv(name);
    const ConvSpec& c = spec(name);
    int64_t M = (int64_t)B * a.H * a.W;
    const bool bf = is_bf16(e);
    const double eb = a.es;
    const double wbytes = eb * 9 * c.cin * c.cout + 4.0 * c.cout;
    const double aflops = 2.0 * M * 9 * c.cin * c.cout;
    const double a2bytes = a2 ? eb * c.cin * M * (a2_mode == 1 ? 0.25 : 1.0) : 0.0;
    if (e->cfg.gemm_mode == YNB_GEMM_FP32_FFMA) {
      GemmParams g{};
      g.a = a.p; g.a_ld = a.ld; g.a_off = 0;
      g.a2 = a2 ? a2->p : nullptr; g.a2_ld = a2 ? a2->ld : 0; g.a2_mode = a2 ? a2_mode : 0;
      g.H = a.H; g.W = a.W; g.C = c.cin;
      g.w = pc.w_dev; g.bias = pc.b_dev; g.out = out.p; g.out_ld = out.ld; g.out_off = 0; g.out_step = 1;
      g.omap = dense_map(); g.M = M; g.N = pc.n; g.Ktot = pc.ktot; g.act = c.act;
      plan->net.push_back({name, "conv3x3_ffma", 4.0 * M * (c.cin + c.cout) + a2bytes + wbytes, aflops,
                           [=](cudaStream_t st) { return launch_gemm_ffma(g, true, st); }});
      return;
    }
    Tensor src = a;
    static const bool no_presplit = getenv("YNB_TC_NO_PRESPLIT") != nullptr;
    const bool presplit = a2 != nullptr && e->cfg.gemm_mode == YNB_GEMM_TC_3XTF32 && !no_presplit;
    if (a2) {
      Tensor a_ = a, a2_ = *a2, s_ = sum, sl_ = sum_lo;
      int B_ = B;
      plan->net.push_back({name + "+merge", "resample_add", (presplit ? 3.0 : 2.0) * eb * M * c.cin + a2bytes,
                           1.0 * M * c.cin, [=](cudaStream_t st) {
        return launch_resample_add(a_.p, a2_.p, s_.p, presplit ? sl_.p : nullptr, B_, a_.H, a_.W, a_.ld, a2_mode, st, bf);
      }});
      src = sum;
    }
    tc->emplace_back();
    TcGemmLaunch& L = tc->back();
    L.w = &pc.tc;
    TcGemmParams& p = L.p;
    memset(&p, 0, sizeof(p));
    p.mode = e->cfg.gemm_mode;
    p.is3x3 = 1;
    p.bf16_in = bf ? 1 : 0;
    p.out_bf16 = out.es == 2 ? 1 : 0;
    p.chunks_per_tap = bf ? (c.cin + 63) / 64 : c.cin / kTcBK;
    p.num_steps = 9 * p.chunks_per_tap;
    p.H = a.H; p.W = a.W;
    tc_pick_tile(p.H, p.W, &p.TH, &p.TW);
    p.tiles_x = (p.W + p.TW - 1) / p.TW;
    p.tiles_y = (p.H + p.TH - 1) / p.TH;
    p.num_tiles = (int64_t)B * p.tiles_x * p.tiles_y;
    p.M = M;
    p.N = pc.n; p.Npad = pc.tc.Npad;
    tc_plan_tmem(p);
    p.a_box_bytes = (uint32_t)(p.TH * p.TW * 128);
    p.out = out.p; p.out_ld = out.ld; p.out_off = 0; p.out_step = 1; p.omap = dense_map();
    p.bias = pc.b_dev; p.act = c.act;
    p.err_flag = e->d_err;
    if (!make_tmap_nhwc(&L.tmA, src.p, c.cin, src.W, src.H, B, src.ld, p.TW, p.TH, bf) ||
        (presplit && !make_tmap_nhwc(&L.tmAlo, sum_lo.p, c.cin, src.W, src.H, B, src.ld, p.TW, p.TH))) {
      error = "cuTensorMapEncodeTiled failed for input of " + name;
      return;
    }
    p.presplit = presplit ? 1 : 0;
    if (!tc_plan_smem(L)) { error = "no smem configuration for " + name; return; }
    L.grid = (unsigned)std::min<int64_t>(p.num_tiles, kNumSMs);
    const TcGemmLaunch* Lp = &L;
    plan->net.push_back({name, "conv3x3_tcgen05", eb * M * (c.cin + c.cout) + wbytes, aflops,
                         [=](cudaStream_t st) { return launch_tc_gemm(*Lp, st); }});
  }
};

int build_plan(ynb_engine* e, int B, Plan** out) {
  auto it = e->plans.find(B);
  if (it != e->plans.end()) { *out = it->second.get(); return YNB_OK; }
  auto plan = std::make_unique<Plan>();
  plan->batch = B;
  e->tc_store.emplace_back();
  e->dp_store.emplace_back();
  Planner P{e, B, plan.get(), &e->tc_store.back(), &e->dp_store.back(), ""};
  const int S = e->S;

  {
    Tensor pool = P.T("pool");
    double px = (double)B * S * S;
    const bool bf = is_bf16(e);
    plan->net.push_back({"backbone.conv1.0+maxpool", "stem_pool", 4.0 * 3 * px + (bf ? 2.0 : 4.0) * 24 * px / 16 + 4.0 * 27 * 24,
                         2.0 * 27 * 24 * px / 4, [=](cudaStream_t st) {
      const float* xin = e->d_x_bound;
      auto key = std::make_tuple(xin, B, S);
      auto it = e->stem_maps.find(key);
      if (it == e->stem_maps.end()) {
        ynb_engine::StemMap sm{};
        sm.ok = make_tmap_stem_input(&sm.tm, xin, S, B) ? 1 : 0;
        if (e->stem_maps.size() > 64) e->stem_maps.clear();
        it = e->stem_maps.emplace(key, sm).first;
      }
      return launch_stem_pool(xin, pool.p, bf, e->stem_w, it->second.tm, it->second.ok, B, S, st);
    }});
  }
  Tensor x = P.T("pool");
  for (int si = 0; si < 3; ++si) {
    std::string st = "stage" + std::to_string(si + 2);
    std::string bk = "backbone." + st + ".";
    int h = stage_channels()[si + 1] / 2;
    Tensor b1dw = P.T(st + ".b1dw"), b2pw = P.T(st + ".b2pw"), mid1 = P.T(st + ".mid1"), mid2 = P.T(st + ".mid2");
    Tensor o0 = P.T(st + ".0");
    P.dw(bk + "0.branch1.0", x, 0, b1dw);
    if (si > 0) plan->net.back().join = true;
    P.pw(bk + "0.branch2.0", x, 0, b2pw, 0, 1);
    P.dw(bk + "0.branch2.3", b2pw, 0, mid2);
    if (!P.catpw(si, bk + "0.", b1dw, mid2, o0)) {
      P.pw(bk + "0.branch1.2", b1dw, 0, o0, 0, 2);
      P.pw(bk + "0.branch2.5", mid2, 0, o0, 1, 2);
    }
    x = o0;
    for (int bi = 1; bi < stage_repeats()[si]; ++bi) {
      std::string u = bk + std::to_string(bi);
      Tensor o = P.T(st + "." + std::to_string(bi));
      const int x2_off = x2_window(stage_layout(is_bf16(e), si), h, is_bf16(e) ? 8 : 4).off;
      const bool ffma = e->cfg.gemm_mode == YNB_GEMM_FP32_FFMA;
      P.pw(u + ".branch2.0", x, x2_off, mid1, 0, 1, ffma && bi > 1);
      if (ffma) {
        plan->net.back().mark = true;
        P.passthrough(u, x, o, h);
      }
      if (!P.dwpw(u + ".branch2.3", u + ".branch2.5", mid1, o, &x)) {
        P.dw(u + ".branch2.3", mid1, 0, mid2);
        P.pw(u + ".branch2.5", mid2, 0, o, 1, 2, false, &x);
      }
      x = o;
    }
  }
  Tensor c3 = P.T("c3"), c4 = P.T("c4"), c5 = P.T("c5");
  Tensor lat3 = P.T("lat3"), lat4 = P.T("lat4"), lat5 = P.T("lat5");
  P.pw("conv1x1_0.convs.0", c3, 0, lat3, 0, 1, true);
  P.pw("conv1x1_1.convs.0", c4, 0, lat4, 0, 1);
  P.pw("conv1x1_2.convs.0", c5, 0, lat5, 0, 1);
  Tensor fpn4 = P.T("fpn4"), p3 = P.T("p3"), p4 = P.T("p4"), p5 = P.T("p5");
  P.conv3("smooth_0.convs.0", lat4, &lat5, 1, P.T("sum4"), P.T("sum4.lo"), fpn4);
  P.conv3("smooth_1.convs.0", lat3, &fpn4, 1, P.T("sum3"), P.T("sum3.lo"), p3);
  P.conv3("smooth_2.convs.0", fpn4, &p3, 2, P.T("sum4b"), P.T("sum4b.lo"), p4);
  P.conv3("smooth_3.convs.0", lat5, &p4, 2, P.T("sum5"), P.T("sum5.lo"), p5);
  Tensor feats[3] = {p3, p4, p5};
  Tensor head_in[3];
  for (int l = 0; l < 3; ++l) {
    std::string hd = "head_det_" + std::to_string(l + 1);
    Tensor ta = P.T("head" + std::to_string(l) + ".a"), tb = P.T("head" + std::to_string(l) + ".b");
    if (!P.dwpw(hd + ".0.convs.0", hd + ".1.convs.0", feats[l], ta, nullptr)) {
      P.dw(hd + ".0.convs.0", feats[l], 0, tb);
      P.pw(hd + ".1.convs.0", tb, 0, ta, 0, 1);
    }
    if (!P.dwpw(hd + ".2.convs.0", hd + ".3.convs.0", ta, tb, nullptr)) {
      Tensor tc2 = P.T("head" + std::to_string(l) + ".c");
      P.dw(hd + ".2.convs.0", ta, 0, tc2);
      P.pw(hd + ".3.convs.0", tc2, 0, tb, 0, 1);
    }
    head_in[l] = tb;
  }
  P.dst = &plan->raw_tail;
  for (int l = 0; l < 3; ++l) P.pw("head_det_" + std::to_string(l + 1) + ".4", head_in[l], 0, e->raw[l], 0, 1);
  plan->fused = e->cfg.gemm_mode != YNB_GEMM_FP32_FFMA && e->cfg.num_anchors == 3 &&
                (e->cfg.num_classes == 80 || e->cfg.num_classes == 20) && !getenv("YNB_NO_FUSED_DECODE");
  if (plan->fused) {
    P.dst = &plan->fused_tail;
    int64_t off = 0;
    for (int l = 0; l < 3; ++l) {
      TcGemmParams::Decode d{};
      const int stride = 8 << l;
      d.boxes = e->d_boxes; d.scores = e->d_scores; d.cls = e->d_cls;
      d.G = S / stride; d.HW = d.G * d.G;
      d.stride = (float)stride; d.input_size = (float)S;
      for (int a = 0; a < 3; ++a) {
        d.aw[a] = e->cfg.anchors[(l * 3 + a) * 2];
        d.ah[a] = e->cfg.anchors[(l * 3 + a) * 2 + 1];
      }
      d.Ntot = e->N(); d.level_off = off;
      off += (int64_t)d.HW * 3;
      P.pw("head_det_" + std::to_string(l + 1) + ".4", head_in[l], 0, e->raw[l], 0, 1, false, nullptr, &d);
    }
  }
  P.dst = nullptr;
  if (!P.error.empty()) return fail(e, YNB_ERR_CUDA, P.error);
  int64_t N = e->N(), off = 0;
  for (int l = 0; l < 3; ++l) {
    DecodeParams d{};
    int stride = 8 << l;
    d.raw = e->raw[l].p; d.ld = e->raw[l].ld;
    d.boxes = e->d_boxes; d.scores = e->d_scores; d.cls = e->d_cls;
    d.batch = B; d.G = S / stride; d.A = e->cfg.num_anchors; d.C = e->cfg.num_classes;
    d.stride = (float)stride; d.input_size = (float)S;
    for (int a = 0; a < d.A; ++a) {
      d.anchor_w[a] = e->cfg.anchors[(l * d.A + a) * 2];
      d.anchor_h[a] = e->cfg.anchors[(l * d.A + a) * 2 + 1];
    }
    d.N = N; d.level_off = off;
    off += (int64_t)d.G * d.G * d.A;
    double cells = (double)B * d.G * d.G;
    plan->decode.push_back({"decode.level" + std::to_string(l), "decode",
                            4.0 * cells * d.A * (1 + d.C + 4) + 24.0 * cells * d.A, 0.0,
                            [=](cudaStream_t st) { return launch_decode_level(d, st); }});
  }
  *out = plan.get();
  e->plans[B] = std::move(plan);
  return YNB_OK;
}

int check_ready(ynb_engine* e, int batch) {
  if (!e) return YNB_ERR_INVALID;
  if (!e->committed) return fail(e, YNB_ERR_STATE, "weights not committed (ynb_load_conv x77, ynb_commit_weights)");
  if (batch <= 0) return fail(e, YNB_ERR_INVALID, "batch must be positive");
  return YNB_OK;
}

cudaEvent_t next_event(ynb_engine* e) {
  cudaEvent_t ev = e->events[e->ev_next];
  e->ev_next = (e->ev_next + 1) % e->events.size();
  return ev;
}

struct SideState {
  cudaEvent_t mark = nullptr, done = nullptr;
};

int run_ops(ynb_engine* e, const std::vector<Op>& ops, SideState* ss = nullptr) {
  cudaStream_t st = e->s_main;
  SideState local;
  if (!ss) ss = &local;
  if (!e->profiling) {
    for (const Op& op : ops) {
      if (op.mark) {
        ss->mark = next_event(e);
        CUDA_TRY(e, cudaEventRecord(ss->mark, st));
      }
      if (op.join && ss->done) {
        CUDA_TRY(e, cudaStreamWaitEvent(st, ss->done, 0));
        ss->done = nullptr;
      }
      cudaError_t r;
      if (op.side) {
        if (!ss->mark) {
          ss->mark = next_event(e);
          CUDA_TRY(e, cudaEventRecord(ss->mark, st));
        }
        CUDA_TRY(e, cudaStreamWaitEvent(e->s_side, ss->mark, 0));
        r = op.fn(e->s_side);
        ss->done = next_event(e);
        CUDA_TRY(e, cudaEventRecord(ss->done, e->s_side));
      } else {
        r = op.fn(st);
      }
      if (r != cudaSuccess)
        return fail(e, YNB_ERR_CUDA, "kernel launch (" + op.name + "): " + cudaGetErrorString(r));
    }
    if (ss == &local && ss->done) CUDA_TRY(e, cudaStreamWaitEvent(st, ss->done, 0));
    return YNB_OK;
  }
  std::vector<cudaEvent_t> ev(ops.size() + 1);
  for (auto& x : ev) CUDA_TRY(e, cudaEventCreate(&x));
  CUDA_TRY(e, cudaEventRecord(ev[0], st));
  for (size_t i = 0; i < ops.size(); ++i) {
    cudaError_t r = ops[i].fn(st);
    if (r != cudaSuccess)
      return fail(e, YNB_ERR_CUDA, "kernel launch (" + ops[i].name + "): " + cudaGetErrorString(r));
    CUDA_TRY(e, cudaEventRecord(ev[i + 1], st));
  }
  CUDA_TRY(e, cudaEventSynchronize(ev.back()));
  for (size_t i = 0; i < ops.size(); ++i) {
    float ms = 0;
    CUDA_TRY(e, cudaEventElapsedTime(&ms, ev[i], ev[i + 1]));
    e->prof.push_back({ops[i].name, ops[i].kind, ops[i].bytes, ops[i].flops, ms});
  }
  for (auto& x : ev) cudaEventDestroy(x);
  return YNB_OK;
}

int enter(ynb_engine* e, cudaStream_t user) {
  CUDA_TRY(e, cudaEventRecord(e->ev_in, user));
  CUDA_TRY(e, cudaStreamWaitEvent(e->s_main, e->ev_in, 0));
  return YNB_OK;
}
int leave(ynb_engine* e, cudaStream_t user) {
  CUDA_TRY(e, cudaEventRecord(e->ev_out, e->s_main));
  CUDA_TRY(e, cudaStreamWaitEvent(user, e->ev_out, 0));
  return YNB_OK;
}

int prepare(ynb_engine* e, int batch, Plan** plan_out) {
  int rc = check_ready(e, batch);
  if (rc) return rc;
  CUDA_TRY(e, cudaSetDevice(e->cfg.device));
  if ((rc = ensure_workspace(e, batch))) return rc;
  return build_plan(e, batch, plan_out);
}

int run_network(ynb_engine* e, const float* x_dev, Plan* plan) {
  e->d_x_bound = x_dev;
  e->prof.clear();
  int rc = run_ops(e, plan->net);
  return rc ? rc : run_ops(e, plan->raw_tail);
}

int run_decoded(ynb_engine* e, const float* x_dev, Plan* plan) {
  if (!plan->fused) {
    int rc = run_network(e, x_dev, plan);
    return rc ? rc : run_ops(e, plan->decode);
  }
  e->d_x_bound = x_dev;
  e->prof.clear();
  int rc = run_ops(e, plan->net);
  return rc ? rc : run_ops(e, plan->fused_tail);
}

int check_device_error(ynb_engine* e) {
  cudaStream_t st = e->s_main;
  int flag = 0;
  CUDA_TRY(e, cudaMemcpyAsync(&flag, e->d_err, 4, cudaMemcpyDeviceToHost, st));
  CUDA_TRY(e, cudaStreamSynchronize(st));
  if (flag != 0) {
    cudaMemsetAsync(e->d_err, 0, 4, st);
    return fail(e, YNB_ERR_CUDA, "tensor-core pipeline timed out waiting on mbarrier (code " +
                                     std::to_string(flag) + ")");
  }
  return YNB_OK;
}

}

static void drop_graphs(ynb_engine* e);

YNB_EXPORT int ynb_abi_version(void) { return YNB_ABI_VERSION; }

YNB_EXPORT const char* ynb_last_error(const ynb_engine* e) { return e ? e->err.c_str() : g_create_error.c_str(); }

YNB_EXPORT int ynb_create(const ynb_config* cfg, ynb_engine** out) {
  if (!cfg || !out) return fail(nullptr, YNB_ERR_INVALID, "null argument");
  *out = nullptr;
  if (cfg->abi_version != YNB_ABI_VERSION) return fail(nullptr, YNB_ERR_INVALID, "ABI version mismatch");
  if (cfg->num_anchors != 3) return fail(nullptr, YNB_ERR_UNSUPPORTED, "num_anchors must be 3");
  if (cfg->num_classes < 1 || cfg->num_classes > 255) return fail(nullptr, YNB_ERR_INVALID, "num_classes out of range");
  if (cfg->input_size < 32 || cfg->input_size % 32 || cfg->input_size > 1024)
    return fail(nullptr, YNB_ERR_INVALID, "input_size must be a multiple of 32 in [32, 1024]");
  if (cfg->gemm_mode < 0 || cfg->gemm_mode > YNB_GEMM_TC_BF16) return fail(nullptr, YNB_ERR_INVALID, "bad gemm_mode");
  int ndev = 0;
  cudaError_t st = cudaGetDeviceCount(&ndev);
  if (st != cudaSuccess || ndev == 0)
    return fail(nullptr, YNB_ERR_NO_DEVICE,
                std::string("no CUDA device: ") + (st != cudaSuccess ? cudaGetErrorString(st) : "count is 0") +
                    " (this library has no CPU path)");
  if (cfg->device < 0 || cfg->device >= ndev) return fail(nullptr, YNB_ERR_INVALID, "device ordinal out of range");
  cudaDeviceProp prop;
  if (cudaGetDeviceProperties(&prop, cfg->device) != cudaSuccess || prop.major != 10)
    return fail(nullptr, YNB_ERR_NO_DEVICE, "device is not compute capability 10.x (built for sm_100a only)");
  if (cudaSetDevice(cfg->device) != cudaSuccess) return fail(nullptr, YNB_ERR_CUDA, "cudaSetDevice failed");
  ynb_engine* e = new ynb_engine();
  e->cfg = *cfg;
  if (e->cfg.max_batch < 1) e->cfg.max_batch = 1;
  e->S = cfg->input_size;
  {
    const float mean[3] = {0.406f, 0.456f, 0.485f}, stdv[3] = {0.225f, 0.224f, 0.229f};
    make_prelut(&e->prelut, mean, stdv);
  }
  e->table = conv_table(cfg->num_classes, cfg->num_anchors);
  e->convs.resize(e->table.size());
  for (size_t i = 0; i < e->table.size(); ++i) e->index[e->table[i].name] = (int)i;
  bool ok = cudaStreamCreateWithFlags(&e->s_main, cudaStreamNonBlocking) == cudaSuccess &&
            cudaStreamCreateWithFlags(&e->s_side, cudaStreamNonBlocking) == cudaSuccess &&
            cudaEventCreateWithFlags(&e->ev_in, cudaEventDisableTiming) == cudaSuccess &&
            cudaEventCreateWithFlags(&e->ev_out, cudaEventDisableTiming) == cudaSuccess;
// ... 237 lines not shown
    cudaGraphExec_t exec = nullptr;
    ce = cudaGraphInstantiate(&exec, graph, 0);
    cudaGraphDestroy(graph);
    if (ce != cudaSuccess) return fail(e, YNB_ERR_CUDA, std::string("cudaGraphInstantiate: ") + cudaGetErrorString(ce));
    it = e->graphs.emplace(key, exec).first;
  }
  CUDA_TRY(e, cudaGraphLaunch(it->second, e->s_main));
  e->counter.n += e->graph_launches[batch];
  return YNB_OK;
}

YNB_EXPORT int ynb_forward_detect(ynb_engine* e, const float* x_dev, int32_t batch, float* ob, float* os,
                                  int32_t* oc, int32_t* on, void* stream) {
  if (!e || !x_dev || !ob || !os || !oc || !on) return fail(e, YNB_ERR_INVALID, "null argument");
  cudaStream_t user = (cudaStream_t)stream;
  CounterScope cs(e);
  int rc = check_ready(e, batch);
  if (rc || (rc = enter(e, user)) || (rc = detect_device(e, x_dev, batch, ob, os, oc, on))) return rc;
  return leave(e, user);
}

static int submit_host_common(ynb_engine* e, int32_t slot_id, const float* x_host, const uint8_t* img_host,
                              const int32_t* rects_host, int32_t batch, float* ob, float* os, int32_t* oc,
                              int32_t* on, void* stream) {
  if (!e || (!x_host && !img_host) || !ob || !os || !oc || !on) return fail(e, YNB_ERR_INVALID, "null argument");
  if (slot_id < 0 || slot_id > 1) return fail(e, YNB_ERR_INVALID, "slot must be 0 or 1");
  cudaStream_t user = (cudaStream_t)stream;
  CounterScope cs(e);
  Plan* plan = nullptr;
  int rc = prepare(e, batch, &plan);
  if (rc) return rc;
  ynb_engine::HostSlot& sl = e->slot[slot_id];
  if (sl.busy) return fail(e, YNB_ERR_STATE, "slot still in flight: call ynb_wait_host first");
  const size_t px = (size_t)3 * e->S * e->S;
  CUDA_TRY(e, cudaEventRecord(e->ev_in, user));
  CUDA_TRY(e, cudaStreamWaitEvent(e->s_copy, e->ev_in, 0));
  if (x_host) {
    const size_t total = px * 4 * batch, half = (total / 2) & ~(size_t)255;
    CUDA_TRY(e, cudaStreamWaitEvent(e->s_copy2, e->ev_in, 0));
    CUDA_TRY(e, cudaMemcpyAsync(sl.x, x_host, half, cudaMemcpyHostToDevice, e->s_copy));
    CUDA_TRY(e, cudaMemcpyAsync(reinterpret_cast<char*>(sl.x) + half, reinterpret_cast<const char*>(x_host) + half,
                                total - half, cudaMemcpyHostToDevice, e->s_copy2));
    CUDA_TRY(e, cudaEventRecord(e->ev_copy2, e->s_copy2));
    CUDA_TRY(e, cudaStreamWaitEvent(e->s_copy, e->ev_copy2, 0));
  } else {
    CUDA_TRY(e, cudaMemcpyAsync(sl.img_u8, img_host, px * batch, cudaMemcpyHostToDevice, e->s_copy));
    if (rects_host)
      CUDA_TRY(e, cudaMemcpyAsync(sl.rects, rects_host, (size_t)batch * 16, cudaMemcpyHostToDevice, e->s_copy));
  }
  CUDA_TRY(e, cudaEventRecord(sl.h2d, e->s_copy));
  CUDA_TRY(e, cudaStreamWaitEvent(e->s_main, sl.h2d, 0));
  if (!x_host)
    CUDA_TRY(e, launch_preprocess_u8(sl.img_u8, rects_host ? sl.rects : nullptr, sl.x, e->d_prelut, batch, e->S,
                                     e->s_main));
  if ((rc = detect_device(e, sl.x, batch, sl.boxes, sl.scores, sl.cls, sl.counts))) return rc;
  CUDA_TRY(e, cudaMemcpyAsync(on, sl.counts, (size_t)batch * 4, cudaMemcpyDeviceToHost, e->s_main));
  CUDA_TRY(e, cudaMemcpyAsync(sl.flag_host, e->d_err, 4, cudaMemcpyDeviceToHost, e->s_main));
  CUDA_TRY(e, cudaEventRecord(sl.done, e->s_main));
  sl.busy = true; sl.batch = batch; sl.ob = ob; sl.os = os; sl.oc = oc; sl.on = on;
  return YNB_OK;
}

YNB_EXPORT int ynb_submit_host(ynb_engine* e, int32_t slot_id, const float* x_host, int32_t batch, float* ob,
                               float* os, int32_t* oc, int32_t* on, void* stream) {
  if (!x_host) return fail(e, YNB_ERR_INVALID, "null argument");
  return submit_host_common(e, slot_id, x_host, nullptr, nullptr, batch, ob, os, oc, on, stream);
}

YNB_EXPORT int ynb_submit_host_u8(ynb_engine* e, int32_t slot_id, const uint8_t* img_host, const int32_t* rects_host,
                                  int32_t batch, float* ob, float* os, int32_t* oc, int32_t* on, void* stream) {
  if (!img_host) return fail(e, YNB_ERR_INVALID, "null argument");
  return submit_host_common(e, slot_id, nullptr, img_host, rects_host, batch, ob, os, oc, on, stream);
}

YNB_EXPORT int ynb_set_normalization(ynb_engine* e, const float* mean_bgr, const float* std_bgr) {
  if (!e || !mean_bgr || !std_bgr) return fail(e, YNB_ERR_INVALID, "null argument");
  for (int c = 0; c < 3; ++c)
    if (!(std_bgr[c] > 0.0f)) return fail(e, YNB_ERR_INVALID, "std must be positive");
  make_prelut(&e->prelut, mean_bgr, std_bgr);
  CUDA_TRY(e, cudaSetDevice(e->cfg.device));
  CUDA_TRY(e, cudaDeviceSynchronize());
  CUDA_TRY(e, cudaMemcpy(e->d_prelut, &e->prelut, sizeof(PreLut), cudaMemcpyHostToDevice));
  return YNB_OK;
}

YNB_EXPORT int ynb_preprocess_u8(ynb_engine* e, const uint8_t* img_dev, const int32_t* rects_dev, int32_t batch,
                                 float* x_dev, void* stream) {
  if (!e || !img_dev || !x_dev || batch <= 0) return fail(e, YNB_ERR_INVALID, "null argument");
  CUDA_TRY(e, cudaSetDevice(e->cfg.device));
  cudaError_t r = launch_preprocess_u8(img_dev, rects_dev, x_dev, e->d_prelut, batch, e->S, (cudaStream_t)stream);
  if (r != cudaSuccess) return fail(e, YNB_ERR_CUDA, std::string("preprocess_u8: ") + cudaGetErrorString(r));
  return YNB_OK;
}

static_assert(sizeof(ynb_image_desc) == sizeof(ImageDesc), "ynb_image_desc and the kernel's ImageDesc must agree");

YNB_EXPORT int ynb_preprocess_letterbox_u8(ynb_engine* e, const uint8_t* src_dev, const ynb_image_desc* descs_dev,
                                           int32_t batch, float* x_dev, void* stream) {
  if (!e || !src_dev || !descs_dev || !x_dev || batch <= 0) return fail(e, YNB_ERR_INVALID, "null argument");
  CUDA_TRY(e, cudaSetDevice(e->cfg.device));
  cudaError_t r = launch_letterbox_preprocess(src_dev, reinterpret_cast<const ImageDesc*>(descs_dev), x_dev, e->d_prelut,
                                              batch, e->S, (cudaStream_t)stream);
  if (r != cudaSuccess) return fail(e, YNB_ERR_CUDA, std::string("letterbox_preprocess: ") + cudaGetErrorString(r));
  return YNB_OK;
}

YNB_EXPORT int ynb_map_boxes(float* boxes_dev, const int32_t* counts_dev, const double* maps_dev, int32_t batch,
                             int64_t n_per_image, void* stream) {
  if (!boxes_dev || !counts_dev || !maps_dev || batch <= 0 || n_per_image <= 0)
    return fail(nullptr, YNB_ERR_INVALID, "ynb_map_boxes: bad arguments");
  cudaError_t r = launch_map_boxes(boxes_dev, counts_dev, maps_dev, batch, n_per_image, (cudaStream_t)stream);
  if (r != cudaSuccess) return fail(nullptr, YNB_ERR_CUDA, std::string("map_boxes: ") + cudaGetErrorString(r));
  return YNB_OK;
}

YNB_EXPORT int ynb_wait_host(ynb_engine* e, int32_t slot_id) {
  if (!e || slot_id < 0 || slot_id > 1) return fail(e, YNB_ERR_INVALID, "bad slot");
  ynb_engine::HostSlot& sl = e->slot[slot_id];
  if (!sl.busy) return fail(e, YNB_ERR_STATE, "nothing submitted on this slot");
  CUDA_TRY(e, cudaSetDevice(e->cfg.device));
  CUDA_TRY(e, cudaEventSynchronize(sl.done));
  sl.busy = false;
  if (*sl.flag_host != 0) {
    int code = *sl.flag_host;
    cudaMemsetAsync(e->d_err, 0, 4, e->s_main);
    return fail(e, YNB_ERR_CUDA, "tensor-core pipeline timed out waiting on mbarrier (code " + std::to_string(code) + ")");
  }
  const int64_t n = e->N();
  size_t kmax = 0;
  for (int b = 0; b < sl.batch; ++b) kmax = std::max(kmax, (size_t)sl.on[b]);
  if (kmax > 0) {
    CUDA_TRY(e, cudaMemcpy2DAsync(sl.ob, (size_t)n * 16, sl.boxes, (size_t)n * 16, kmax * 16, sl.batch,
                                  cudaMemcpyDeviceToHost, e->s_d2h));
    CUDA_TRY(e, cudaMemcpy2DAsync(sl.os, (size_t)n * 4, sl.scores, (size_t)n * 4, kmax * 4, sl.batch,
                                  cudaMemcpyDeviceToHost, e->s_d2h));
    CUDA_TRY(e, cudaMemcpy2DAsync(sl.oc, (size_t)n * 4, sl.cls, (size_t)n * 4, kmax * 4, sl.batch,
                                  cudaMemcpyDeviceToHost, e->s_d2h));
    CUDA_TRY(e, cudaStreamSynchronize(e->s_d2h));
  }
  return YNB_OK;
}

YNB_EXPORT int ynb_detect_host(ynb_engine* e, const float* x_host, int32_t batch, float* ob, float* os,
                               int32_t* oc, int32_t* on, void* stream) {
  if (!e) return YNB_ERR_INVALID;
  if (e->slot[0].busy) return fail(e, YNB_ERR_STATE, "slot 0 in flight (ynb_submit_host without ynb_wait_host)");
  int rc = ynb_submit_host(e, 0, x_host, batch, ob, os, oc, on, stream);
  return rc ? rc : ynb_wait_host(e, 0);
}

YNB_EXPORT int ynb_tap_shape(const ynb_engine* e, const char* tap, int32_t* c, int32_t* h, int32_t* w) {
  if (!e || !tap || !c || !h || !w) return YNB_ERR_INVALID;
  ynb_engine* me = const_cast<ynb_engine*>(e);
  if (me->taps.empty()) {
    ynb_engine tmp;
    tmp.cfg = e->cfg;
    layout_workspace(&tmp, 1, e->S, nullptr);
    me->taps = tmp.taps;
  }
  auto it = me->taps.find(tap);
  if (it == me->taps.end()) return fail(me, YNB_ERR_INVALID, std::string("unknown tap ") + tap);
  int hh = it->second.H;
  if (me->ws_S != me->S) {
    ynb_engine tmp;
    tmp.cfg = e->cfg;
    layout_workspace(&tmp, 1, e->S, nullptr);
    hh = tmp.taps.at(tap).H;
  }
  *c = it->second.C; *h = hh; *w = hh;
  return YNB_OK;
}

YNB_EXPORT int ynb_read_tap(ynb_engine* e, const char* tap, int32_t batch, float* out_dev, void* stream) {
  if (!e || !tap || !out_dev) return fail(e, YNB_ERR_INVALID, "null argument");
  if (!e->ws || e->ws_S != e->S || batch > e->ws_batch) return fail(e, YNB_ERR_STATE, "run a forward first");
  auto it = e->taps.find(tap);
  if (it == e->taps.end() || !it->second.p) return fail(e, YNB_ERR_INVALID, std::string("unknown tap ") + tap);
  const Tensor& t = it->second;
  CounterScope cs(e);
  int rc = enter(e, (cudaStream_t)stream);
  if (rc) return rc;
  CUDA_TRY(e, launch_nhwc_to_nchw(t.p, t.ld, t.map, out_dev, batch, t.C, t.H * t.W, e->s_main, t.es == 2));
  return leave(e, (cudaStream_t)stream);
}

YNB_EXPORT int64_t ynb_launch_count(const ynb_engine* e) { return e ? e->counter.n : 0; }

YNB_EXPORT int ynb_set_profiling(ynb_engine* e, int32_t on) {
  if (!e) return YNB_ERR_INVALID;
  e->profiling = on != 0;
  return YNB_OK;
}

YNB_EXPORT int32_t ynb_profile_count(const ynb_engine* e) { return e ? (int32_t)e->prof.size() : 0; }

YNB_EXPORT int ynb_profile_entry(const ynb_engine* e, int32_t i, const char** name, const char** kind, float* ms,
                                 double* bytes, double* flops) {
  if (!e || i < 0 || i >= (int32_t)e->prof.size() || !name || !kind || !ms || !bytes || !flops) return YNB_ERR_INVALID;
  const ProfEntry& p = e->prof[i];
  *name = p.name.c_str(); *kind = p.kind.c_str(); *ms = p.ms; *bytes = p.bytes; *flops = p.flops;
  return YNB_OK;
}

static thread_local std::string g_unit_error;
#define UNIT_TRY(call)                                                       \
  do {                                                                       \
    cudaError_t _st = (call);                                                \
    if (_st != cudaSuccess) {                                                \
      g_create_error = std::string(#call) + ": " + cudaGetErrorString(_st);  \
      return YNB_ERR_CUDA;                                                   \
    }                                                                        \
  } while (0)

YNB_EXPORT int ynb_dwconv3x3(const float* in, int32_t in_ld, int32_t in_off, float* out, int32_t out_ld,
                             int32_t out_off, int32_t out_step, const float* w, const float* b, int32_t batch,
                             int32_t h_in, int32_t w_in, int32_t channels, int32_t stride, int32_t act, void* stream) {
  if (!in || !out || !w || !b || channels % 4 || in_ld % 4 || in_off % 4 || out_ld % 4 || out_off % 4 ||
      out_step != 1 || (stride != 1 && stride != 2))
    return fail(nullptr, YNB_ERR_INVALID, "ynb_dwconv3x3: channels/ld/off must be multiples of 4, out_step 1");
  CUtensorMap tm;
  if (!getenv("YNB_DW_NO_TMA") && make_tmap_dw(&tm, in, in_ld, in_off, batch, h_in, w_in, channels, stride)) {
    UNIT_TRY(launch_dwconv3x3_tma(tm, out, out_ld, out_off, w, b, batch, h_in, w_in, channels, stride, act,
                                  (cudaStream_t)stream));
    return YNB_OK;
  }
  UNIT_TRY(launch_dwconv3x3(in, in_ld, in_off, out, out_ld, out_off, w, b, batch, h_in, w_in, channels, stride, act,
                            (cudaStream_t)stream));
  return YNB_OK;
}

YNB_EXPORT int ynb_resize_bilinear(const float* in_dev, int32_t batch, int32_t h_in, int32_t w_in, float* out_dev,
                                   int32_t s_out, int32_t with_flip, void* stream) {
  if (!in_dev || !out_dev || batch <= 0 || h_in <= 0 || w_in <= 0 || s_out <= 0)
    return fail(nullptr, YNB_ERR_INVALID, "ynb_resize_bilinear: bad arguments");
  UNIT_TRY(launch_resize_bilinear(in_dev, out_dev, batch, h_in, w_in, s_out, with_flip, (cudaStream_t)stream));
  return YNB_OK;
}

YNB_EXPORT int ynb_pwconv(const float* in, int32_t in_ld, int32_t in_off, float* out, int32_t out_ld,
                          int32_t out_off, int32_t out_step, const float* w, const float* b, int64_t pixels,
                          int32_t cin, int32_t cout, int32_t act, void* stream) {
  if (!in || !out || !w || !b || cin % 4 || in_ld % 4 || in_off % 4)
    return fail(nullptr, YNB_ERR_INVALID, "ynb_pwconv: cin / in_ld / in_off must be multiples of 4");
  GemmParams g{};
  g.a = in; g.a_ld = in_ld; g.a_off = in_off; g.w = w; g.bias = b; g.out = out; g.out_ld = out_ld;
  g.out_off = out_off; g.out_step = out_step; g.omap = dense_map(); g.M = pixels; g.N = cout; g.Ktot = cin;
  g.act = act;
  UNIT_TRY(launch_gemm_ffma(g, false, (cudaStream_t)stream));
  return YNB_OK;
}

YNB_EXPORT int ynb_pwconv_tc(const float* in, int32_t in_ld, int32_t in_off, float* out, int32_t out_ld,
                             int32_t out_off, int32_t out_step, const float* w_dev, const float* b_dev,
                             int64_t pixels, int32_t cin, int32_t cout, int32_t act, int32_t mode, void* stream) {
  if (!in || !out || !w_dev || !b_dev || cin % 4 || in_ld % 4 || in_off % 4 || out_ld % 4 ||
      (out_step == 1 && out_off % 4) || cout > 256 || (mode != YNB_GEMM_TC_3XTF32 && mode != YNB_GEMM_TC_TF32))
    return fail(nullptr, YNB_ERR_INVALID, "ynb_pwconv_tc: bad arguments");
  cudaStream_t st = (cudaStream_t)stream;
  std::vector<float> w((size_t)cout * cin);
  UNIT_TRY(cudaMemcpy(w.data(), w_dev, w.size() * 4, cudaMemcpyDeviceToHost));
  TcWeights t;
  t.N = cout; t.Npad = round_up(cout, 16); t.Kpad = round_up(cin, kTcBK);
  std::vector<float> hi((size_t)t.Npad * t.Kpad, 0.f), lo((size_t)t.Npad * t.Kpad, 0.f);
  for (int n = 0; n < cout; ++n)
    for (int k = 0; k < cin; ++k)
      split_tf32_host(w[(size_t)n * cin + k], &hi[(size_t)n * t.Kpad + k], &lo[(size_t)n * t.Kpad + k]);
  int* d_err = nullptr;
  UNIT_TRY(cudaMalloc(&t.hi, hi.size() * 4));
  UNIT_TRY(cudaMalloc(&t.lo, lo.size() * 4));
  UNIT_TRY(cudaMalloc(&d_err, 4));
  UNIT_TRY(cudaMemset(d_err, 0, 4));
  UNIT_TRY(cudaMemcpy(t.hi, hi.data(), hi.size() * 4, cudaMemcpyHostToDevice));
  UNIT_TRY(cudaMemcpy(t.lo, lo.data(), lo.size() * 4, cudaMemcpyHostToDevice));
  int rc = YNB_OK;
  TcGemmLaunch L;
  L.w = &t;
  TcGemmParams& p = L.p;
  memset(&p, 0, sizeof(p));
  p.mode = mode; p.num_steps = t.Kpad / kTcBK; p.chunks_per_tap = p.num_steps; p.ksub = (cin + 7) / 8;
  p.M = pixels; p.num_tiles = (pixels + kTcBM - 1) / kTcBM; p.N = cout; p.Npad = t.Npad;
  tc_plan_tmem(p);
  p.a_box_bytes = kTcAStageBytes;
  p.out = out; p.out_ld = out_ld; p.out_off = out_off; p.out_step = out_step; p.omap = dense_map();
  p.bias = b_dev; p.act = act; p.err_flag = d_err;
  long long* d_trace = nullptr;
  const int trace_cap = 8 * 64 * 32;
  const bool want_trace = getenv("YNB_TC_TRACE") != nullptr;
  if (want_trace) {
    UNIT_TRY(cudaMalloc(&d_trace, (1 + 4 * trace_cap) * 8));
    UNIT_TRY(cudaMemset(d_trace, 0, (1 + 4 * trace_cap) * 8));
    p.trace = d_trace; p.trace_cap = trace_cap;
  }
  p.tma_store = (out_step == 1 && out_off % 4 == 0 && getenv("YNB_TC_NO_TMA_STORE") == nullptr) ? 1 : 0;
  if (getenv("YNB_TC_PASS") != nullptr && cin >= cout && out_ld >= 2 * cout) {
    p.pass = in; p.pass_ld = in_ld; p.tma_store = 0; p.out_off = 1; p.out_step = 2;
  }
  if (!make_tmap_2d(&t.tm_hi, t.hi, t.Kpad, t.Npad, t.Kpad, t.Npad) ||
      !make_tmap_2d(&t.tm_lo, t.lo, t.Kpad, t.Npad, t.Kpad, t.Npad) ||
      (p.tma_store && !make_tmap_out(&L.tmOut, out + out_off, (uint64_t)round_up(cout, 4), (uint64_t)pixels,
                                     (uint64_t)out_ld)) ||
      !make_tmap_2d(&L.tmA, in + in_off, cin, pixels, in_ld, kTcBM) || !tc_plan_smem(L)) {
    rc = fail(nullptr, YNB_ERR_CUDA, "ynb_pwconv_tc: tensor map / smem planning failed");
  } else {
    L.grid = (unsigned)std::min<int64_t>(p.num_tiles, kNumSMs);
    cudaError_t r = launch_tc_gemm(L, st);
    if (r == cudaSuccess) r = cudaStreamSynchronize(st);
    int flag = 0;
    if (r == cudaSuccess) r = cudaMemcpy(&flag, d_err, 4, cudaMemcpyDeviceToHost);
    if (r != cudaSuccess) rc = fail(nullptr, YNB_ERR_CUDA, std::string("ynb_pwconv_tc: ") + cudaGetErrorString(r));
    else if (flag) rc = fail(nullptr, YNB_ERR_CUDA, "ynb_pwconv_tc: mbarrier timeout code " + std::to_string(flag));
    if (want_trace && r == cudaSuccess) {
      std::vector<long long> h(1 + 4 * trace_cap);
      cudaMemcpy(h.data(), d_trace, h.size() * 8, cudaMemcpyDeviceToHost);
      int n = 0;
      for (int i = 0; i < trace_cap; ++i) n += h[4 + 4 * i] != 0;
      fprintf(stderr, "YNB_TC_TRACE stages=%d resident=%d nmain=%d acc_stages=%d steps=%d grid=%u events=%d\n",
              p.num_stages, p.w_resident, p.nmain, p.acc_stages, p.num_steps, L.grid, n);
      for (int i = 0; i < trace_cap; ++i)
        if (h[4 + 4 * i] != 0)
          fprintf(stderr, "TRACE %lld %lld %lld %lld\n", h[1 + 4 * i], h[2 + 4 * i], h[3 + 4 * i], h[4 + 4 * i]);
    }
  }
  if (d_trace) cudaFree(d_trace);
  cudaFree(t.hi); cudaFree(t.lo); cudaFree(d_err);
  return rc;
}

YNB_EXPORT int ynb_dwpw_tc(const float* in, int32_t in_ld, const float* dw_w, const float* dw_b, int32_t dw_act,
                           const float* pw_w, const float* pw_b, int32_t act, float* out, int32_t out_ld,
                           const float* pass, int32_t pass_ld, int32_t batch, int32_t h, int32_t w_, int32_t channels,
                           int32_t cout, int32_t mode, void* stream) {
  const bool bfm = mode == YNB_GEMM_TC_BF16;
  const int al = bfm ? 8 : 4;
  if (!in || !dw_w || !dw_b || !pw_w || !pw_b || !out || channels % al || in_ld % al || out_ld % al || cout > (bfm ? 240 : 128) ||
      cout < 1 || batch < 1 || h < 1 || w_ < 1 ||
      (mode != YNB_GEMM_TC_3XTF32 && mode != YNB_GEMM_TC_TF32 && mode != YNB_GEMM_TC_BF16) ||
      (pass && (out_ld < 2 * cout || pass_ld < cout || pass_ld % 4 || ((uintptr_t)pass & 15u))) || (!pass && out_ld < cout) ||
      ((uintptr_t)out & 15u))
    return fail(nullptr, YNB_ERR_INVALID, "ynb_dwpw_tc: bad arguments");
  cudaStream_t st = (cudaStream_t)stream;
  std::vector<float> wv((size_t)cout * channels);
  UNIT_TRY(cudaMemcpy(wv.data(), pw_w, wv.size() * 4, cudaMemcpyDeviceToHost));
  TcWeights t;
  t.N = cout; t.Npad = round_up(cout, 16); t.Kpad = round_up(channels, bfm ? 64 : kTcBK);
  std::vector<float> hi((size_t)t.Npad * t.Kpad, 0.f), lo((size_t)t.Npad * t.Kpad, 0.f);
  std::vector<bf16> bwv((size_t)t.Npad * t.Kpad, __float2bfloat16(0.0f));
  for (int n = 0; n < cout; ++n)
    for (int k = 0; k < channels; ++k) {
      split_tf32_host(wv[(size_t)n * channels + k], &hi[(size_t)n * t.Kpad + k], &lo[(size_t)n * t.Kpad + k]);
      bwv[(size_t)n * t.Kpad + k] = __float2bfloat16_rn(wv[(size_t)n * channels + k]);
    }
  int* d_err = nullptr;
  UNIT_TRY(cudaMalloc(&t.hi, hi.size() * 4));
  UNIT_TRY(cudaMalloc(&t.lo, lo.size() * 4));
  UNIT_TRY(cudaMalloc(&d_err, 4));
  UNIT_TRY(cudaMemset(d_err, 0, 4));
  UNIT_TRY(cudaMemcpy(t.hi, hi.data(), hi.size() * 4, cudaMemcpyHostToDevice));
  UNIT_TRY(cudaMemcpy(t.lo, lo.data(), lo.size() * 4, cudaMemcpyHostToDevice));
  if (bfm) UNIT_TRY(cudaMemcpy(t.hi, bwv.data(), bwv.size() * 2, cudaMemcpyHostToDevice));
  int rc = YNB_OK;
  DwPwLaunch L;
  DwPwParams& p = L.p;
  memset(&p, 0, sizeof(p));
  p.dw_w = dw_w; p.dw_b = dw_b; p.dw_act = dw_act;
  p.out = out; p.out_ld = out_ld; p.out_off = 0; p.omap = dense_map();
  p.bias = pw_b; p.act = act; p.pass = pass; p.pass_ld = pass ? pass_ld : 0; p.err_flag = d_err;
  long long* d_trace = nullptr;
  const bool want_trace = getenv("YNB_DP_TRACE") != nullptr;
  if (want_trace) {
    UNIT_TRY(cudaMalloc(&d_trace, 6 * 16 * 8 * 8));
    UNIT_TRY(cudaMemset(d_trace, 0, 6 * 16 * 8 * 8));
    p.trace = d_trace;
  }
  if (!make_tmap_2d(&t.tm_hi, t.hi, t.Kpad, t.Npad, t.Kpad, t.Npad, bfm) ||
      !make_tmap_2d(&t.tm_lo, t.lo, t.Kpad, t.Npad, t.Kpad, t.Npad) ||
      !plan_dwpw(L, in, in_ld, batch, h, w_, channels, channels, &t, mode)) {
    rc = fail(nullptr, YNB_ERR_CUDA, "ynb_dwpw_tc: tensor map / smem planning failed");
  } else {
    cudaError_t r = launch_dwpw_tc(L, st);
    if (r == cudaSuccess) r = cudaStreamSynchronize(st);
    int flag = 0;
    if (r == cudaSuccess) r = cudaMemcpy(&flag, d_err, 4, cudaMemcpyDeviceToHost);
    if (r != cudaSuccess) rc = fail(nullptr, YNB_ERR_CUDA, std::string("ynb_dwpw_tc: ") + cudaGetErrorString(r));
    else if (flag) rc = fail(nullptr, YNB_ERR_CUDA, "ynb_dwpw_tc: mbarrier timeout code " + std::to_string(flag));
    if (want_trace && r == cudaSuccess) {
      std::vector<long long> h(6 * 16 * 8);
      cudaMemcpy(h.data(), d_trace, h.size() * 8, cudaMemcpyDeviceToHost);
      long long t0 = 0;
      for (long long v : h) if (v && (!t0 || v < t0)) t0 = v;
      fprintf(stderr, "YNB_DP_TRACE chunks=%d a_stages=%d raw_stages=%d resident=%d lgTW=%d tiles=%lld grid=%u\n", L.p.num_chunks,
              L.p.a_stages, L.p.raw_stages, L.p.w_resident, L.p.lgTW, (long long)L.p.num_tiles, L.grid);
      const char* names[6] = {"raw_issued", "raw_landed", "A_written", "mma_issued", "acc_ready", "epi_done"};
      for (int lt = 0; lt < 16; ++lt)
        for (int role = 0; role < 6; ++role) {
          std::string line;
          for (int kc = 0; kc < 8; ++kc)
            if (h[(role * 16 + lt) * 8 + kc]) line += " " + std::to_string(h[(role * 16 + lt) * 8 + kc] - t0);
          if (!line.empty()) fprintf(stderr, "TRACE tile %2d %-11s%s\n", lt, names[role], line.c_str());
        }
    }
  }
  if (d_trace) cudaFree(d_trace);
  cudaFree(t.hi); cudaFree(t.lo); cudaFree(d_err);
  return rc;
}

YNB_EXPORT int ynb_stem_pool(const float* x, float* out, const float* w, const float* b, int32_t batch,
                             int32_t input_size, void* stream) {
  if (!x || !out || !w || !b || input_size % 32) return fail(nullptr, YNB_ERR_INVALID, "ynb_stem_pool: bad arguments");
  StemWeights wt;
  UNIT_TRY(cudaMemcpy(wt.w, w, sizeof(wt.w), cudaMemcpyDeviceToHost));
  UNIT_TRY(cudaMemcpy(wt.b, b, sizeof(wt.b), cudaMemcpyDeviceToHost));
  CUtensorMap tmx{};
  const int use_tma = make_tmap_stem_input(&tmx, x, input_size, batch) ? 1 : 0;
  UNIT_TRY(launch_stem_pool(x, out, false, wt, tmx, use_tma, batch, input_size, (cudaStream_t)stream));
  return YNB_OK;
}

YNB_EXPORT int ynb_decode_level(const float* raw, int32_t raw_ld, float* boxes, float* scores, int32_t* cls,
                                int32_t batch, int32_t grid, int32_t stride_px, int32_t input_size,
                                const float* anchors_wh, int32_t num_anchors, int32_t num_classes,
                                int64_t boxes_per_image, int64_t level_off, void* stream) {
  if (!raw || !boxes || !scores || !cls || !anchors_wh || num_anchors > 4)
    return fail(nullptr, YNB_ERR_INVALID, "ynb_decode_level: bad arguments");
  DecodeParams d{};
  d.raw = raw; d.ld = raw_ld; d.boxes = boxes; d.scores = scores; d.cls = cls; d.batch = batch; d.G = grid;
  d.A = num_anchors; d.C = num_classes; d.stride = (float)stride_px; d.input_size = (float)input_size;
  for (int a = 0; a < num_anchors; ++a) { d.anchor_w[a] = anchors_wh[2 * a]; d.anchor_h[a] = anchors_wh[2 * a + 1]; }
  d.N = boxes_per_image; d.level_off = level_off;
  UNIT_TRY(launch_decode_level(d, (cudaStream_t)stream));
  return YNB_OK;
}

YNB_EXPORT int64_t ynb_nms_workspace_bytes(int32_t batch, int64_t n) { return nms_workspace_bytes(batch, n); }

YNB_EXPORT int64_t ynb_nms_grid_workspace_bytes(int32_t batch, int32_t input_size) {
  return grid_nms_workspace_bytes(batch, make_grid_geom(input_size).N);
}

YNB_EXPORT int ynb_nms_grid(const float* boxes, const float* scores, const int32_t* cls, int32_t batch,
                            int32_t input_size, int32_t num_classes, float conf, float thr, int32_t diou, float* ob,
                            float* os, int32_t* oc, int32_t* on, uint8_t* keep, void* ws, int64_t ws_bytes,
                            void* stream) {
  if (!boxes || !scores || !cls || !ob || !os || !oc || !on || !ws || input_size <= 0 || input_size % 32 ||
      ws_bytes < ynb_nms_grid_workspace_bytes(batch, input_size))
    return fail(nullptr, YNB_ERR_INVALID, "ynb_nms_grid: bad arguments / workspace too small");
  GridNmsWorkspace w = grid_nms_carve(ws, batch, make_grid_geom(input_size).N);
  UNIT_TRY(launch_nms_grid(boxes, scores, cls, batch, input_size, num_classes, conf, thr, diou, ob, os, oc, on, keep,
                           w, (cudaStream_t)stream));
  return YNB_OK;
}

YNB_EXPORT int ynb_nms(const float* boxes, const float* scores, const int32_t* cls, int32_t batch, int64_t n,
                       int32_t num_classes, float conf, float thr, int32_t diou, float* ob, float* os, int32_t* oc,
                       int32_t* on, uint8_t* keep, void* ws, int64_t ws_bytes, void* stream) {
  if (!boxes || !scores || !cls || !ob || !os || !oc || !on || !ws || ws_bytes < nms_workspace_bytes(batch, n))
    return fail(nullptr, YNB_ERR_INVALID, "ynb_nms: bad arguments / workspace too small");
  NmsWorkspace w = nms_carve(ws, batch, n);
  UNIT_TRY(launch_nms(boxes, scores, cls, batch, n, num_classes, conf, thr, diou, ob, os, oc, on, keep, w,
                      (cudaStream_t)stream));
  return YNB_OK;
}


namespace {
bool level_geometry(int input_size, int grid[3], int stride[3]) {
  if (input_size <= 0 || input_size % 32) return false;
  const int st[3] = {8, 16, 32};
  for (int l = 0; l < 3; ++l) { stride[l] = st[l]; grid[l] = input_size / st[l]; }
  return true;
}
}

YNB_EXPORT int64_t ynb_train_loss_workspace_bytes(int32_t batch, int32_t input_size) {
  return (int64_t)train_loss_blocks(batch, input_size) * 4 * sizeof(double);
}

YNB_EXPORT int ynb_train_loss(const float* raw_s, const float* raw_m, const float* raw_l, int32_t raw_ld,
                              const float* target, int32_t batch, int32_t input_size, const float* anchors_wh,
                              int32_t num_anchors, int32_t num_classes, float* losses, float* grad_s, float* grad_m,
                              float* grad_l, void* ws, int64_t ws_bytes, void* stream) {
  TrainLossParams p{};
  if (!raw_s || !raw_m || !raw_l || !target || !anchors_wh || !losses || !grad_s || !grad_m || !grad_l || !ws ||
      batch <= 0 || num_anchors <= 0 || num_anchors > kTrainMaxAnchors || num_classes <= 0 ||
      raw_ld < num_anchors * (1 + num_classes + 4) || !level_geometry(input_size, p.grid, p.stride) ||
      ws_bytes < ynb_train_loss_workspace_bytes(batch, input_size))
    return fail(nullptr, YNB_ERR_INVALID, "ynb_train_loss: bad arguments / workspace too small");
  p.raw[0] = raw_s; p.raw[1] = raw_m; p.raw[2] = raw_l;
  p.grad[0] = grad_s; p.grad[1] = grad_m; p.grad[2] = grad_l;
  p.target = target; p.partials = (double*)ws; p.ld = raw_ld; p.B = batch; p.A = num_anchors; p.C = num_classes;
  p.S = input_size;
  int off = 0;
  for (int l = 0; l < 3; ++l) {
    p.cells[l] = p.grid[l] * p.grid[l];
    p.cell_off[l] = off;
    off += p.cells[l];
    for (int a = 0; a < num_anchors; ++a) {
      p.anchors[l][a][0] = anchors_wh[(l * num_anchors + a) * 2];
      p.anchors[l][a][1] = anchors_wh[(l * num_anchors + a) * 2 + 1];
    }
  }
  p.cells_total = off;
  UNIT_TRY(launch_train_loss(p, losses, (cudaStream_t)stream));
  return YNB_OK;
}

YNB_EXPORT int ynb_build_targets(const float* labels, const int32_t* counts, int32_t batch, int32_t max_labels,
                                 int32_t input_size, const float* anchors_wh, int32_t num_anchors, float* target,
                                 void* stream) {
  TargetParams p{};
  if (!labels || !target || !anchors_wh || batch <= 0 || max_labels < 0 || num_anchors <= 0 ||
      num_anchors > kTrainMaxAnchors || !level_geometry(input_size, p.grid, p.stride))
    return fail(nullptr, YNB_ERR_INVALID, "ynb_build_targets: bad arguments");
  p.labels = labels; p.counts = counts; p.target = target; p.B = batch; p.L = max_labels; p.A = num_anchors;
  p.S = input_size;
  long long off = 0;
  for (int l = 0; l < 3; ++l) {
    p.row_off[l] = off;
    off += (long long)p.grid[l] * p.grid[l] * num_anchors;
  }
  p.N = off;
  for (int k = 0; k < 3 * num_anchors; ++k) {
    p.anchors[k][0] = (double)anchors_wh[2 * k];
    p.anchors[k][1] = (double)anchors_wh[2 * k + 1];
  }
  UNIT_TRY(launch_build_targets(p, (cudaStream_t)stream));
  return YNB_OK;
}

YNB_EXPORT int ynb_sgd_step(float* params, const float* grads, float* momentum_buf, int64_t n, float lr,
                            float momentum, float weight_decay, int32_t first_step, float grad_scale, void* stream) {
  if (!params || !grads || !momentum_buf || n <= 0 || ((uintptr_t)params | (uintptr_t)grads | (uintptr_t)momentum_buf) % 16)
    return fail(nullptr, YNB_ERR_INVALID, "ynb_sgd_step: null / unaligned (16 B) buffers");
  UNIT_TRY(launch_sgd_step(params, grads, momentum_buf, n, lr, momentum, weight_decay, first_step, grad_scale,
                           (cudaStream_t)stream));
  return YNB_OK;
}

YNB_EXPORT int32_t ynb_ema_chunk_elems(void) { return kEmaChunk; }

YNB_EXPORT int ynb_ema_update(const uint64_t* ema_ptrs_dev, const uint64_t* model_ptrs_dev, const int64_t* sizes_dev,
                              const int32_t* chunk_tensor_dev, const int32_t* chunk_index_dev, int32_t num_chunks,
                              float d, float one_minus_d, void* stream) {
  if (!ema_ptrs_dev || !model_ptrs_dev || !sizes_dev || !chunk_tensor_dev || !chunk_index_dev || num_chunks < 0)
    return fail(nullptr, YNB_ERR_INVALID, "ynb_ema_update: bad arguments");
  UNIT_TRY(launch_ema_update(reinterpret_cast<const unsigned long long*>(ema_ptrs_dev),
                             reinterpret_cast<const unsigned long long*>(model_ptrs_dev),
                             reinterpret_cast<const long long*>(sizes_dev), chunk_tensor_dev, chunk_index_dev, num_chunks,
                             d, one_minus_d, (cudaStream_t)stream));
  return YNB_OK;
}

YNB_EXPORT int ynb_dwconv3x3_bwd_data(const float* dout, int32_t do_ld, int32_t do_off, float* din, int32_t di_ld,
                                      int32_t di_off, const float* w, int32_t batch, int32_t h_in, int32_t w_in,
                                      int32_t channels, int32_t stride, void* stream) {
  if (!dout || !din || !w || batch <= 0 || h_in <= 0 || w_in <= 0 || channels <= 0 || (stride != 1 && stride != 2))
    return fail(nullptr, YNB_ERR_INVALID, "ynb_dwconv3x3_bwd_data: bad arguments");
  cudaStream_t st = (cudaStream_t)stream;
  const bool vec = channels % 4 == 0 && do_ld % 4 == 0 && do_off % 4 == 0 && di_ld % 4 == 0 && di_off % 4 == 0 &&
                   ((uintptr_t)dout | (uintptr_t)din | (uintptr_t)w) % 16 == 0;
  CUtensorMap tm;
  if (stride == 1 && vec && !getenv("YNB_DW_NO_TMA") &&
      make_tmap_dw(&tm, dout, do_ld, do_off, batch, h_in, w_in, channels, 1)) {
    UNIT_TRY(launch_dwconv3x3_tma(tm, din, di_ld, di_off, w, nullptr, batch, h_in, w_in, channels, 1, YNB_ACT_NONE, st,
                                  true));
    return YNB_OK;
  }
  if (stride == 2 && vec && 9 * channels * 4 <= 48 * 1024) {
    const long long items = (long long)batch * ((h_in + 1) / 2) * ((w_in + 1) / 2) * (channels / 4);
    const int nb = (int)std::min<long long>((items + 255) / 256, (long long)kNumSMs * 8);
    dwconv3x3_s2_bwd_data_kernel<<<nb, 256, 9 * channels * sizeof(float), st>>>(dout, do_ld, do_off, din, di_ld, di_off, w,
                                                                               batch, h_in, w_in, channels);
    YNB_COUNT_LAUNCH();
    UNIT_TRY(cudaGetLastError());
    return YNB_OK;
  }
  const long long total = (long long)batch * h_in * w_in * ((channels + 3) / 4);
  const int blocks = (int)std::min<long long>((total + 255) / 256, (long long)kNumSMs * 16);
  if (vec)
    dwconv3x3_bwd_data_kernel<true><<<blocks, 256, 0, st>>>(dout, do_ld, do_off, din, di_ld, di_off, w, batch, h_in, w_in,
                                                            channels, stride);
  else
    dwconv3x3_bwd_data_kernel<false><<<blocks, 256, 0, st>>>(dout, do_ld, do_off, din, di_ld, di_off, w, batch, h_in, w_in,
                                                             channels, stride);
  YNB_COUNT_LAUNCH();
  UNIT_TRY(cudaGetLastError());
  return YNB_OK;
}

YNB_EXPORT int64_t ynb_dwconv3x3_bwd_weight_workspace_bytes(int32_t batch, int32_t h_in, int32_t w_in, int32_t channels,
                                                            int32_t stride) {
  const int h_out = (h_in - 1) / stride + 1, w_out = (w_in - 1) / stride + 1;
  return (int64_t)dw_bwd_chunks(batch, h_out, w_out) * 10 * channels * sizeof(float);
}

YNB_EXPORT int ynb_dwconv3x3_bwd_weight(const float* dout, int32_t do_ld, int32_t do_off, const float* in, int32_t in_ld,
                                        int32_t in_off, float* dwdb, int32_t batch, int32_t h_in, int32_t w_in,
                                        int32_t channels, int32_t stride, void* ws, int64_t ws_bytes, void* stream) {
  if (!dout || !in || !dwdb || !ws || batch <= 0 || h_in <= 0 || w_in <= 0 || channels <= 0 ||
      (stride != 1 && stride != 2) ||
      ws_bytes < ynb_dwconv3x3_bwd_weight_workspace_bytes(batch, h_in, w_in, channels, stride))
    return fail(nullptr, YNB_ERR_INVALID, "ynb_dwconv3x3_bwd_weight: bad arguments / workspace too small");
  const int h_out = (h_in - 1) / stride + 1, w_out = (w_in - 1) / stride + 1;
  const int chunks = dw_bwd_chunks(batch, h_out, w_out);
  const bool vec = channels % 4 == 0 && do_ld % 4 == 0 && do_off % 4 == 0 && in_ld % 4 == 0 && in_off % 4 == 0 &&
                   ((uintptr_t)dout | (uintptr_t)in) % 16 == 0;
  dim3 grid(chunks, (channels + kDwBwdCg * 4 - 1) / (kDwBwdCg * 4)), block(kDwBwdCg, kDwBwdSlices);
  cudaStream_t st = (cudaStream_t)stream;
  float* part = (float*)ws;
#define YNB_DWBW(S, V) \
  dwconv3x3_bwd_weight_kernel<S, V><<<grid, block, 0, st>>>(dout, do_ld, do_off, in, in_ld, in_off, part, batch, h_in, w_in, channels)
  if (stride == 1) { if (vec) YNB_DWBW(1, true); else YNB_DWBW(1, false); }
  else             { if (vec) YNB_DWBW(2, true); else YNB_DWBW(2, false); }
#undef YNB_DWBW
  YNB_COUNT_LAUNCH();
  launch_reduce_partials(part, chunks, 10LL * channels, dwdb, st);
  UNIT_TRY(cudaGetLastError());
  return YNB_OK;
}

// ... 19 lines not shown
    int* err = (int*)((char*)ws + ynb_pwconv_bwd_weight_workspace_bytes(pixels, cin, cout) - 16);
    UNIT_TRY(cudaMemsetAsync(err, 0, 4, st));
    WgradParams p{};
    p.dout = dout; p.do_ld = do_ld; p.do_off = do_off; p.in = in; p.in_ld = in_ld; p.in_off = in_off;
    p.partial = (float*)ws; p.M = pixels; p.K = cin; p.N = cout; p.err = err;
    UNIT_TRY(launch_pw_wgrad_tc(p, chunks, st));
    {
      const int ntiles = (cout + 127) / 128, kpad = wgrad_tc_kpad(cin);
      const long long elems = (long long)ntiles * 128 * kpad;
      launch_wgrad_reduce((const float*)ws, chunks, ntiles, kpad, cout, cin, dw, db, st);
      YNB_COUNT_LAUNCH();
    }
    UNIT_TRY(cudaGetLastError());
    if (getenv("YNB_SYNC_CHECK")) {
      int flag = 0;
      UNIT_TRY(cudaStreamSynchronize(st));
      UNIT_TRY(cudaMemcpy(&flag, err, 4, cudaMemcpyDeviceToHost));
      if (flag) return fail(nullptr, YNB_ERR_CUDA, "ynb_pwconv_bwd_weight: mbarrier timeout code " + std::to_string(flag));
    }
    return YNB_OK;
  }
  const int chunks = pw_bwd_chunks(pixels, cin, cout);
  long long m_per_chunk = (pixels + chunks - 1) / chunks;
  m_per_chunk = (m_per_chunk + kPwBwdSlab - 1) / kPwBwdSlab * kPwBwdSlab;
  float* pw = (float*)ws;
  float* pb = pw + (long long)chunks * cout * cin;
  cudaStream_t st = (cudaStream_t)stream;
  const int vec = cin % 4 == 0 && cout % 4 == 0 && do_ld % 4 == 0 && do_off % 4 == 0 && in_ld % 4 == 0 &&
                  in_off % 4 == 0 && ((uintptr_t)dout | (uintptr_t)in) % 16 == 0;
  dim3 grid(chunks, (cout + kPwBwdTile - 1) / kPwBwdTile, (cin + kPwBwdTile - 1) / kPwBwdTile);
  if (vec && !getenv("YNB_PWBW_NO_ASYNC")) {
    UNIT_TRY(cudaFuncSetAttribute(pwconv_bwd_weight_async_kernel, cudaFuncAttributeMaxDynamicSharedMemorySize,
                                  (int)kPwBwdAsyncSmem));
    pwconv_bwd_weight_async_kernel<<<grid, 256, kPwBwdAsyncSmem, st>>>(dout, do_ld, do_off, in, in_ld, in_off, pw, pb,
                                                                       pixels, cin, cout, m_per_chunk);
  } else {
    pwconv_bwd_weight_kernel<<<grid, 256, 0, st>>>(dout, do_ld, do_off, in, in_ld, in_off, pw, pb, pixels, cin, cout,
                                                   m_per_chunk, vec);
  }
  YNB_COUNT_LAUNCH();
  launch_reduce_partials(pw, chunks, (long long)cout * cin, dw, st);
  launch_reduce_partials(pb, chunks, cout, db, st);
  UNIT_TRY(cudaGetLastError());
  return YNB_OK;
}

YNB_EXPORT int ynb_act_bwd(const float* dout, int32_t do_ld, int32_t do_off, const float* out, int32_t o_ld,
                           int32_t o_off, float* dpre, int32_t dp_ld, int32_t dp_off, int64_t pixels, int32_t channels,
                           int32_t act, void* stream) {
  if (!dout || !out || !dpre || pixels <= 0 || channels <= 0 || (act != YNB_ACT_RELU && act != YNB_ACT_LEAKY))
    return fail(nullptr, YNB_ERR_INVALID, "ynb_act_bwd: bad arguments");
  const long long total = (long long)pixels * channels;
  const int blocks = (int)std::min<long long>((total + 255) / 256, (long long)kNumSMs * 16);
  act_bwd_kernel<<<blocks, 256, 0, (cudaStream_t)stream>>>(dout, do_ld, do_off, out, o_ld, o_off, dpre, dp_ld, dp_off,
                                                           pixels, channels, act == YNB_ACT_RELU ? 0.0f : 0.1f);
  YNB_COUNT_LAUNCH();
  UNIT_TRY(cudaGetLastError());
  return YNB_OK;
}

YNB_EXPORT int ynb_forward_train_loss(ynb_engine* e, const float* x_dev, int32_t batch, const float* target,
                                      float* losses, float* grad_s, float* grad_m, float* grad_l, void* ws,
                                      int64_t ws_bytes, void* stream) {
  if (!e || !x_dev || !target || !losses || !grad_s || !grad_m || !grad_l || !ws)
    return fail(e, YNB_ERR_INVALID, "null argument");
  if (ws_bytes < ynb_train_loss_workspace_bytes(batch, e->S))
    return fail(e, YNB_ERR_INVALID, "ynb_forward_train_loss: workspace too small");
  cudaStream_t user = (cudaStream_t)stream;
  CounterScope cs(e);
  Plan* plan = nullptr;
  int rc = prepare(e, batch, &plan);
  if (rc || (rc = enter(e, user)) || (rc = run_network(e, x_dev, plan))) return rc;
  TrainLossParams p{};
  level_geometry(e->S, p.grid, p.stride);
  float* grads[3] = {grad_s, grad_m, grad_l};
  int off = 0;
  for (int l = 0; l < 3; ++l) {
    p.raw[l] = e->raw[l].p; p.grad[l] = grads[l];
    p.cells[l] = p.grid[l] * p.grid[l];
    p.cell_off[l] = off;
    off += p.cells[l];
    for (int a = 0; a < e->cfg.num_anchors; ++a) {
      p.anchors[l][a][0] = e->cfg.anchors[(l * e->cfg.num_anchors + a) * 2];
      p.anchors[l][a][1] = e->cfg.anchors[(l * e->cfg.num_anchors + a) * 2 + 1];
    }
  }
  p.cells_total = off;
  p.target = target; p.partials = (double*)ws; p.ld = e->raw[0].ld; p.B = batch; p.A = e->cfg.num_anchors;
  p.C = e->cfg.num_classes; p.S = e->S;
  if (p.ld != ynb_raw_ld(e)) return fail(e, YNB_ERR_STATE, "ynb_forward_train_loss: head map stride changed");
  CUDA_TRY(e, launch_train_loss(p, losses, e->s_main));
  if ((rc = leave(e, user))) return rc;
  return e->cfg.gemm_mode == YNB_GEMM_FP32_FFMA ? YNB_OK : check_device_error(e);
}

YNB_EXPORT int32_t ynb_raw_ld(const ynb_engine* e) {
  return e ? round_up(e->cfg.num_anchors * (1 + e->cfg.num_classes + 4), 4) : 0;
}

YNB_EXPORT int ynb_conv3x3_bwd_weight(const float* dout, int32_t do_ld, int32_t do_off, const float* in, int32_t in_ld,
                                      int32_t in_off, float* dw9, float* db, int32_t batch, int32_t h, int32_t w_,
                                      int32_t cin, int32_t cout, void* ws, int64_t ws_bytes, void* stream) {
  const int64_t pixels = (int64_t)batch * h * w_;
  const bool aligned = cin % 4 == 0 && cout % 4 == 0 && do_ld % 4 == 0 && do_off % 4 == 0 && in_ld % 4 == 0 &&
                       in_off % 4 == 0 && ((uintptr_t)dout | (uintptr_t)in) % 16 == 0;
  if (!dout || !in || !dw9 || !db || !ws || batch <= 0 || h <= 0 || w_ <= 0 || cin <= 0 || cout <= 0 ||
      pixels >= (1LL << 31) || ws_bytes < ynb_pwconv_bwd_weight_workspace_bytes(pixels, cin, cout))
    return fail(nullptr, YNB_ERR_INVALID, "ynb_conv3x3_bwd_weight: bad arguments / workspace too small");
  if (!aligned || !wgrad_tc_kpad(cin))
    return fail(nullptr, YNB_ERR_UNSUPPORTED, "ynb_conv3x3_bwd_weight: needs 16-byte aligned views and cin <= 255");
  cudaStream_t st = (cudaStream_t)stream;
  const int chunks = wgrad_tc_chunks(pixels, cout);
  int* err = (int*)((char*)ws + ynb_pwconv_bwd_weight_workspace_bytes(pixels, cin, cout) - 16);
  UNIT_TRY(cudaMemsetAsync(err, 0, 4, st));
  const int ntiles = (cout + 127) / 128, kpad = wgrad_tc_kpad(cin);
  const long long elems = (long long)ntiles * 128 * kpad;
  for (int t = 0; t < 9; ++t) {
    WgradParams p{};
    p.dout = dout; p.do_ld = do_ld; p.do_off = do_off; p.in = in; p.in_ld = in_ld; p.in_off = in_off;
    p.partial = (float*)ws; p.M = pixels; p.K = cin; p.N = cout; p.err = err;
    p.H = h; p.W = w_; p.dy = t / 3 - 1; p.dx = t % 3 - 1;
    UNIT_TRY(launch_pw_wgrad_tc(p, chunks, st));
    launch_wgrad_reduce((const float*)ws, chunks, ntiles, kpad, cout, cin, dw9 + (long long)t * cout * cin, db, st);
    YNB_COUNT_LAUNCH();
  }
  UNIT_TRY(cudaGetLastError());
  if (getenv("YNB_SYNC_CHECK")) {
    int flag = 0;
    UNIT_TRY(cudaStreamSynchronize(st));
    UNIT_TRY(cudaMemcpy(&flag, err, 4, cudaMemcpyDeviceToHost));
    if (flag) return fail(nullptr, YNB_ERR_CUDA, "ynb_conv3x3_bwd_weight: mbarrier timeout code " + std::to_string(flag));
  }
  return YNB_OK;
}

YNB_EXPORT int ynb_stem_conv_fwd(const float* x, const float* w2724, float* out, int32_t batch, int32_t input_size,
                                 void* stream) {
  if (!x || !w2724 || !out || batch <= 0 || input_size <= 0 || input_size % 2)
    return fail(nullptr, YNB_ERR_INVALID, "ynb_stem_conv_fwd: bad arguments");
  const long long items = (long long)batch * (input_size / 2) * (input_size / 2) * 6;
  stem_conv_fwd_kernel<<<grid_for(items), 256, 0, (cudaStream_t)stream>>>(x, w2724, out, batch, input_size);
  YNB_COUNT_LAUNCH();
  UNIT_TRY(cudaGetLastError());
  return YNB_OK;
}

YNB_EXPORT int64_t ynb_stem_conv_bwd_weight_workspace_bytes(int32_t batch, int32_t input_size) {
  return (int64_t)stem_wg_chunks(batch, input_size) * kStemWgOut * sizeof(float);
}

YNB_EXPORT int ynb_stem_conv_bwd_weight(const float* dout, const float* x, float* dw2724, int32_t batch, int32_t input_size,
                                        void* ws, int64_t ws_bytes, void* stream) {
  if (!dout || !x || !dw2724 || !ws || batch <= 0 || input_size <= 0 || input_size % 2 ||
      ws_bytes < ynb_stem_conv_bwd_weight_workspace_bytes(batch, input_size))
    return fail(nullptr, YNB_ERR_INVALID, "ynb_stem_conv_bwd_weight: bad arguments / workspace too small");
  if (((uintptr_t)dout | (uintptr_t)ws) & 15u)
    return fail(nullptr, YNB_ERR_INVALID, "ynb_stem_conv_bwd_weight: dout / workspace must be 16-byte aligned");
  const int grid = stem_wg_grid(batch, input_size), nseg = stem_wg_nseg(input_size);
  const long long items = (long long)batch * (input_size / 2) * nseg;
  if (items > INT32_MAX) return fail(nullptr, YNB_ERR_INVALID, "ynb_stem_conv_bwd_weight: batch too large");
  cudaStream_t st = (cudaStream_t)stream;
  stem_conv_bwd_weight_kernel<<<grid, kStemWgThreads, 0, st>>>(dout, x, (float*)ws, batch, input_size, (int)items, nseg);
  YNB_COUNT_LAUNCH();
  launch_reduce_partials((const float*)ws, 2 * grid, kStemWgOut, dw2724, st);
  UNIT_TRY(cudaGetLastError());
  return YNB_OK;
}

YNB_EXPORT int ynb_maxpool3x3s2_fwd(const float* in, float* out, int32_t batch, int32_t h, int32_t w_, int32_t channels,
                                    void* stream) {
  if (!in || !out || batch <= 0 || h <= 0 || w_ <= 0 || channels <= 0 || channels % 4)
    return fail(nullptr, YNB_ERR_INVALID, "ynb_maxpool3x3s2_fwd: bad arguments");
  const long long items = (long long)batch * ((h - 1) / 2 + 1) * ((w_ - 1) / 2 + 1) * (channels / 4);
  maxpool3x3s2_fwd_kernel<<<grid_for(items), 256, 0, (cudaStream_t)stream>>>(in, out, batch, h, w_, channels);
  YNB_COUNT_LAUNCH();
  UNIT_TRY(cudaGetLastError());
  return YNB_OK;
}

YNB_EXPORT int ynb_maxpool3x3s2_bwd(const float* dout, const float* in, float* din, int32_t batch, int32_t h, int32_t w_,
                                    int32_t channels, void* stream) {
  if (!dout || !in || !din || batch <= 0 || h <= 0 || w_ <= 0 || channels <= 0)
    return fail(nullptr, YNB_ERR_INVALID, "ynb_maxpool3x3s2_bwd: bad arguments");
  const long long items = (long long)batch * h * w_ * channels;
  maxpool3x3s2_bwd_kernel<<<grid_for(items), 256, 0, (cudaStream_t)stream>>>(dout, in, din, batch, h, w_, channels);
  YNB_COUNT_LAUNCH();
  UNIT_TRY(cudaGetLastError());
  return YNB_OK;
}

YNB_EXPORT int ynb_shuffle_unit_move(float* x, float* a, float* b, int64_t rows, int32_t half, int32_t half_padded,
                                     int32_t op, void* stream) {
  if (!x || !a || !b || rows <= 0 || half <= 0 || half_padded < half || op < 0 || op > 3 || (((uintptr_t)x) & 7u))
    return fail(nullptr, YNB_ERR_INVALID, "ynb_shuffle_unit_move: bad arguments");
  shuffle_unit_move_kernel<<<grid_for(rows * half_padded), 256, 0, (cudaStream_t)stream>>>(x, a, b, rows, half, half_padded, op);
  YNB_COUNT_LAUNCH();
  UNIT_TRY(cudaGetLastError());
  return YNB_OK;
}

YNB_EXPORT int ynb_maxpool3x3s2_fwd_idx(const float* in, float* out, uint8_t* idx, int32_t batch, int32_t h, int32_t w_,
                                        int32_t channels, void* stream) {
  if (!in || !out || !idx || batch <= 0 || h <= 0 || w_ <= 0 || channels <= 0 || channels % 4 ||
      (((uintptr_t)in | (uintptr_t)out) & 15u) || ((uintptr_t)idx & 3u))
    return fail(nullptr, YNB_ERR_INVALID, "ynb_maxpool3x3s2_fwd_idx: bad arguments");
  const long long items = (long long)batch * ((h - 1) / 2 + 1) * ((w_ - 1) / 2 + 1) * (channels / 4);
  maxpool3x3s2_fwd_idx_kernel<<<grid_for(items), 256, 0, (cudaStream_t)stream>>>(in, out, idx, batch, h, w_, channels);
  YNB_COUNT_LAUNCH();
  UNIT_TRY(cudaGetLastError());
  return YNB_OK;
}

YNB_EXPORT int ynb_maxpool3x3s2_bwd_idx(const float* dout, const uint8_t* idx, float* din, int32_t batch, int32_t h,
                                        int32_t w_, int32_t channels, void* stream) {
  if (!dout || !idx || !din || batch <= 0 || h <= 0 || w_ <= 0 || channels <= 0 || channels % 4 ||
      (((uintptr_t)dout | (uintptr_t)din) & 15u) || ((uintptr_t)idx & 3u))
    return fail(nullptr, YNB_ERR_INVALID, "ynb_maxpool3x3s2_bwd_idx: bad arguments");
  const long long items = (long long)batch * h * w_ * (channels / 4);
  maxpool3x3s2_bwd_idx_kernel<<<grid_for(items), 256, 0, (cudaStream_t)stream>>>(dout, idx, din, batch, h, w_, channels);
  YNB_COUNT_LAUNCH();
  UNIT_TRY(cudaGetLastError());
  return YNB_OK;
}

YNB_EXPORT int ynb_resample_add(const float* a, const float* a2, float* out, int32_t batch, int32_t h, int32_t w_,
                                int32_t channels, int32_t mode, void* stream) {
  if (!a || !a2 || !out || batch <= 0 || h <= 0 || w_ <= 0 || channels <= 0 || channels % 4 || (mode != 1 && mode != 2) ||
      (mode == 1 && ((h | w_) & 1)))
    return fail(nullptr, YNB_ERR_INVALID, "ynb_resample_add: bad arguments");
  UNIT_TRY(launch_resample_add(a, a2, out, nullptr, batch, h, w_, channels, mode, (cudaStream_t)stream));
  return YNB_OK;
}

YNB_EXPORT int ynb_resample_bwd(const float* dout, float* da2, int32_t batch, int32_t h, int32_t w_, int32_t channels,
                                int32_t mode, void* stream) {
  if (!dout || !da2 || batch <= 0 || h <= 0 || w_ <= 0 || channels <= 0 || channels % 4 || (mode != 1 && mode != 2) ||
      (mode == 1 && ((h | w_) & 1)))
    return fail(nullptr, YNB_ERR_INVALID, "ynb_resample_bwd: bad arguments");
  const int h2 = mode == 1 ? h / 2 : h * 2, w2 = mode == 1 ? w_ / 2 : w_ * 2;
  const long long items = (long long)batch * h2 * w2 * (channels / 4);
  resample_bwd_kernel<<<grid_for(items), 256, 0, (cudaStream_t)stream>>>(dout, da2, batch, h, w_, channels, mode);
  YNB_COUNT_LAUNCH();
  UNIT_TRY(cudaGetLastError());
  return YNB_OK;
}

YNB_EXPORT int ynb_add(const float* a, const float* b, float* out, int64_t n, void* stream) {
  if (!a || !b || !out || n <= 0 || n % 4 || (((uintptr_t)a | (uintptr_t)b | (uintptr_t)out) & 15u))
    return fail(nullptr, YNB_ERR_INVALID, "ynb_add: n must be a multiple of 4, buffers 16-byte aligned");
  add_kernel<<<grid_for(n / 4), 256, 0, (cudaStream_t)stream>>>(a, b, out, n / 4);
  YNB_COUNT_LAUNCH();
  UNIT_TRY(cudaGetLastError());
  return YNB_OK;
}

YNB_EXPORT int ynb_conv3x3_tc(const float* in, int32_t in_ld, float* out, int32_t out_ld, const float* w_dev,
                              const float* b_dev, int32_t batch, int32_t h, int32_t w_, int32_t cin, int32_t cout,
                              int32_t act, int32_t mode, void* stream) {
  if (!in || !out || !w_dev || !b_dev || batch <= 0 || h <= 0 || w_ <= 0 || cin <= 0 || cin % kTcBK || in_ld % 4 ||
      out_ld % 4 || cout < 1 || cout > 256 || (mode != YNB_GEMM_TC_3XTF32 && mode != YNB_GEMM_TC_TF32) ||
      (((uintptr_t)in | (uintptr_t)out) & 15u))
    return fail(nullptr, YNB_ERR_INVALID, "ynb_conv3x3_tc: bad arguments");
  cudaStream_t st = (cudaStream_t)stream;
  const int ktot = 9 * cin;
  std::vector<float> wv((size_t)cout * ktot);
  UNIT_TRY(cudaMemcpy(wv.data(), w_dev, wv.size() * 4, cudaMemcpyDeviceToHost));
  TcWeights t;
  t.N = cout; t.Npad = round_up(cout, 16); t.Kpad = ktot;
  std::vector<float> hi((size_t)t.Npad * t.Kpad, 0.f), lo((size_t)t.Npad * t.Kpad, 0.f);
  for (int n = 0; n < cout; ++n)
    for (int k = 0; k < ktot; ++k)
      split_tf32_host(wv[(size_t)n * ktot + k], &hi[(size_t)n * t.Kpad + k], &lo[(size_t)n * t.Kpad + k]);
  int* d_err = nullptr;
  UNIT_TRY(cudaMalloc(&t.hi, hi.size() * 4));
  UNIT_TRY(cudaMalloc(&t.lo, lo.size() * 4));
  UNIT_TRY(cudaMalloc(&d_err, 4));
  UNIT_TRY(cudaMemset(d_err, 0, 4));
  UNIT_TRY(cudaMemcpy(t.hi, hi.data(), hi.size() * 4, cudaMemcpyHostToDevice));
  UNIT_TRY(cudaMemcpy(t.lo, lo.data(), lo.size() * 4, cudaMemcpyHostToDevice));
  int rc = YNB_OK;
  TcGemmLaunch L;
  L.w = &t;
  TcGemmParams& p = L.p;
  memset(&p, 0, sizeof(p));
  p.mode = mode; p.is3x3 = 1;
  p.chunks_per_tap = cin / kTcBK;
  p.num_steps = 9 * p.chunks_per_tap;
  p.H = h; p.W = w_;
  tc_pick_tile(p.H, p.W, &p.TH, &p.TW);
  p.tiles_x = (p.W + p.TW - 1) / p.TW;
  p.tiles_y = (p.H + p.TH - 1) / p.TH;
  p.num_tiles = (int64_t)batch * p.tiles_x * p.tiles_y;
  p.M = (int64_t)batch * h * w_;
  p.N = cout; p.Npad = t.Npad;
  tc_plan_tmem(p);
  p.a_box_bytes = (uint32_t)(p.TH * p.TW * 128);
  p.out = out; p.out_ld = out_ld; p.out_off = 0; p.out_step = 1; p.omap = dense_map();
  p.bias = b_dev; p.act = act; p.err_flag = d_err;
  if (!make_tmap_2d(&t.tm_hi, t.hi, t.Kpad, t.Npad, t.Kpad, t.Npad) ||
      !make_tmap_2d(&t.tm_lo, t.lo, t.Kpad, t.Npad, t.Kpad, t.Npad) ||
      !make_tmap_nhwc(&L.tmA, in, cin, w_, h, batch, in_ld, p.TW, p.TH) || !tc_plan_smem(L)) {
    rc = fail(nullptr, YNB_ERR_CUDA, "ynb_conv3x3_tc: tensor map / smem planning failed");
  } else {
    L.grid = (unsigned)std::min<int64_t>(p.num_tiles, kNumSMs);
    cudaError_t r = launch_tc_gemm(L, st);
    if (r == cudaSuccess) r = cudaStreamSynchronize(st);
    int flag = 0;
    if (r == cudaSuccess) r = cudaMemcpy(&flag, d_err, 4, cudaMemcpyDeviceToHost);
    if (r != cudaSuccess) rc = fail(nullptr, YNB_ERR_CUDA, std::string("ynb_conv3x3_tc: ") + cudaGetErrorString(r));
    else if (flag) rc = fail(nullptr, YNB_ERR_CUDA, "ynb_conv3x3_tc: mbarrier timeout code " + std::to_string(flag));
  }
  cudaFree(t.hi); cudaFree(t.lo); cudaFree(d_err);
  return rc;
}

namespace {
__global__ void pack_tc_weights_kernel(const float* __restrict__ w, int w_ld, int rows, int cols, int trans,
                                       float* __restrict__ hi, float* __restrict__ lo, int Npad, int Kpad, int* err_flag) {
  const int i = blockIdx.x * blockDim.x + threadIdx.x;
  if (i == 0 && err_flag) *err_flag = 0;
  if (i >= Npad * Kpad) return;
  const int n = i / Kpad, k = i - n * Kpad;
  float v = 0.f;
  if (n < rows && k < cols) v = trans ? w[(size_t)k * w_ld + n] : w[(size_t)n * w_ld + k];
  const uint32_t h = rn_tf32_bits(__float_as_uint(v));
  hi[i] = __uint_as_float(h);
  lo[i] = __uint_as_float(rn_tf32_bits(__float_as_uint(v - __uint_as_float(h))));
}

struct AsyncWs { float* hi; float* lo; int* flag; };
int64_t tc_async_bytes(int Npad, int Kpad) { return (int64_t)2 * Npad * Kpad * 4 + 256; }
bool carve_async(void* ws, int64_t bytes, int Npad, int Kpad, AsyncWs* o) {
  if (!ws || ((uintptr_t)ws & 255u) || bytes < tc_async_bytes(Npad, Kpad)) return false;
  o->hi = (float*)ws;
  o->lo = o->hi + (size_t)Npad * Kpad;
  o->flag = (int*)(o->lo + (size_t)Npad * Kpad);
  return true;
}
}

YNB_EXPORT int64_t ynb_tc_async_workspace_bytes(int32_t cout, int32_t ktot) {
  return tc_async_bytes(round_up(cout, 16), round_up(ktot, kTcBK));
}

YNB_EXPORT int ynb_pwconv_tc_async(const float* in, int32_t in_ld, int32_t in_off, float* out, int32_t out_ld,
                                   int32_t out_off, int32_t out_step, const float* w_dev, int32_t w_ld, int32_t w_rows,
                                   int32_t w_cols, int32_t w_trans, const float* b_dev, int64_t pixels, int32_t cin, int32_t cout, int32_t act,
                                   int32_t mode, void* workspace, int64_t workspace_bytes, void* stream) {
  if (!in || !out || !w_dev || !b_dev || cin % 4 || in_ld % 4 || in_off % 4 || out_ld % 4 || pixels < 1 || cout < 1 ||
      w_cols < 1 || w_cols > cin || w_rows < 1 || w_rows > cout || w_ld < (w_trans ? w_rows : w_cols) ||
      (out_step == 1 && out_off % 4) || cout > 256 || (mode != YNB_GEMM_TC_3XTF32 && mode != YNB_GEMM_TC_TF32))
    return fail(nullptr, YNB_ERR_INVALID, "ynb_pwconv_tc_async: bad arguments");
  cudaStream_t st = (cudaStream_t)stream;
  TcWeights t;
  t.N = cout; t.Npad = round_up(cout, 16); t.Kpad = round_up(cin, kTcBK);
  AsyncWs a;
  if (!carve_async(workspace, workspace_bytes, t.Npad, t.Kpad, &a))
    return fail(nullptr, YNB_ERR_INVALID, "ynb_pwconv_tc_async: workspace too small or not 256-byte aligned");
  t.hi = a.hi; t.lo = a.lo;
  const int total = t.Npad * t.Kpad;
  pack_tc_weights_kernel<<<(total + 255) / 256, 256, 0, st>>>(w_dev, w_ld, w_rows, w_cols, w_trans, t.hi, t.lo, t.Npad,
                                                              t.Kpad, a.flag);
  TcGemmLaunch L;
  L.w = &t;
  TcGemmParams& p = L.p;
  memset(&p, 0, sizeof(p));
  p.mode = mode; p.num_steps = t.Kpad / kTcBK; p.chunks_per_tap = p.num_steps; p.ksub = (cin + 7) / 8;
  p.M = pixels; p.num_tiles = (pixels + kTcBM - 1) / kTcBM; p.N = cout; p.Npad = t.Npad;
  tc_plan_tmem(p);
  p.a_box_bytes = kTcAStageBytes;
  p.out = out; p.out_ld = out_ld; p.out_off = out_off; p.out_step = out_step; p.omap = dense_map();
  p.bias = b_dev; p.act = act; p.err_flag = a.flag;
  p.tma_store = (out_step == 1 && out_off % 4 == 0) ? 1 : 0;
  if (!make_tmap_2d(&t.tm_hi, t.hi, t.Kpad, t.Npad, t.Kpad, t.Npad) ||
      !make_tmap_2d(&t.tm_lo, t.lo, t.Kpad, t.Npad, t.Kpad, t.Npad) ||
      (p.tma_store && !make_tmap_out(&L.tmOut, out + out_off, (uint64_t)round_up(cout, 4), (uint64_t)pixels,
                                     (uint64_t)out_ld)) ||
      !make_tmap_2d(&L.tmA, in + in_off, cin, pixels, in_ld, kTcBM) || !tc_plan_smem(L))
    return fail(nullptr, YNB_ERR_CUDA, "ynb_pwconv_tc_async: tensor map / smem planning failed");
  L.grid = (unsigned)std::min<int64_t>(p.num_tiles, kNumSMs);
  UNIT_TRY(launch_tc_gemm(L, st));
  return YNB_OK;
}

YNB_EXPORT int ynb_conv3x3_tc_async(const float* in, int32_t in_ld, float* out, int32_t out_ld, const float* w_dev,
                                    const float* b_dev, int32_t batch, int32_t h, int32_t w_, int32_t cin, int32_t cout,
                                    int32_t act, int32_t mode, void* workspace, int64_t workspace_bytes, void* stream) {
  if (!in || !out || !w_dev || !b_dev || batch <= 0 || h <= 0 || w_ <= 0 || cin <= 0 || cin % kTcBK || in_ld % 4 ||
      out_ld % 4 || cout < 1 || cout > 256 || (mode != YNB_GEMM_TC_3XTF32 && mode != YNB_GEMM_TC_TF32) ||
      (((uintptr_t)in | (uintptr_t)out) & 15u))
    return fail(nullptr, YNB_ERR_INVALID, "ynb_conv3x3_tc_async: bad arguments");
  cudaStream_t st = (cudaStream_t)stream;
  const int ktot = 9 * cin;
  TcWeights t;
  t.N = cout; t.Npad = round_up(cout, 16); t.Kpad = ktot;
  AsyncWs a;
  if (!carve_async(workspace, workspace_bytes, t.Npad, t.Kpad, &a))
    return fail(nullptr, YNB_ERR_INVALID, "ynb_conv3x3_tc_async: workspace too small or not 256-byte aligned");
  t.hi = a.hi; t.lo = a.lo;
  const int total = t.Npad * t.Kpad;
  pack_tc_weights_kernel<<<(total + 255) / 256, 256, 0, st>>>(w_dev, ktot, cout, ktot, 0, t.hi, t.lo, t.Npad, t.Kpad, a.flag);
  TcGemmLaunch L;
  L.w = &t;
  TcGemmParams& p = L.p;
  memset(&p, 0, sizeof(p));
  p.mode = mode; p.is3x3 = 1;
  p.chunks_per_tap = cin / kTcBK;
  p.num_steps = 9 * p.chunks_per_tap;
  p.H = h; p.W = w_;
  tc_pick_tile(p.H, p.W, &p.TH, &p.TW);
  p.tiles_x = (p.W + p.TW - 1) / p.TW;
  p.tiles_y = (p.H + p.TH - 1) / p.TH;
  p.num_tiles = (int64_t)batch * p.tiles_x * p.tiles_y;
  p.M = (int64_t)batch * h * w_;
  p.N = cout; p.Npad = t.Npad;
  tc_plan_tmem(p);
  p.a_box_bytes = (uint32_t)(p.TH * p.TW * 128);
  p.out = out; p.out_ld = out_ld; p.out_off = 0; p.out_step = 1; p.omap = dense_map();
  p.bias = b_dev; p.act = act; p.err_flag = a.flag;
  if (!make_tmap_2d(&t.tm_hi, t.hi, t.Kpad, t.Npad, t.Kpad, t.Npad) ||
      !make_tmap_2d(&t.tm_lo, t.lo, t.Kpad, t.Npad, t.Kpad, t.Npad) ||
      !make_tmap_nhwc(&L.tmA, in, cin, w_, h, batch, in_ld, p.TW, p.TH) || !tc_plan_smem(L))
    return fail(nullptr, YNB_ERR_CUDA, "ynb_conv3x3_tc_async: tensor map / smem planning failed");
  L.grid = (unsigned)std::min<int64_t>(p.num_tiles, kNumSMs);
  UNIT_TRY(launch_tc_gemm(L, st));
  return YNB_OK;
}

namespace {
bool bn_args_ok(long long M, int C, std::initializer_list<int> strides, std::initializer_list<const void*> ptrs) {
  if (M <= 0 || C <= 0 || C % 4) return false;
  for (int v : strides) if (v % 4) return false;
  for (const void* q : ptrs) if (!q || ((uintptr_t)q & 15u)) return false;
  return true;
}
}

YNB_EXPORT int64_t ynb_bn_workspace_bytes(int64_t pixels, int32_t channels) {
  return ((int64_t)bn_chunks(pixels) * 2 * channels + 2 * channels) * sizeof(float);
}

YNB_EXPORT int ynb_bn_train_fwd(const float* x, int32_t x_ld, int32_t x_off, float* y, int32_t y_ld, int32_t y_off,
                                const float* gamma, const float* beta, float* running_mean, float* running_var,
                                float* save_mean, float* save_rstd, int64_t pixels, int32_t channels, float eps,
                                float momentum, int32_t act, void* ws, int64_t ws_bytes, void* stream) {
  if (!bn_args_ok(pixels, channels, {x_ld, x_off, y_ld, y_off}, {x, y, gamma, beta, save_mean, save_rstd, ws}) ||
      ws_bytes < ynb_bn_workspace_bytes(pixels, channels) || act < 0 || act > 2)
    return fail(nullptr, YNB_ERR_INVALID, "ynb_bn_train_fwd: bad arguments (channels / strides multiples of 4, 16-byte aligned)");
  cudaStream_t st = (cudaStream_t)stream;
  const int chunks = bn_chunks(pixels);
  const long long rpc = (pixels + chunks - 1) / chunks;
  float* part = (float*)ws;
  float* sums = part + (long long)chunks * 2 * channels;
  dim3 grid(chunks, (channels + kBnCg * 4 - 1) / (kBnCg * 4)), block(kBnCg, kBnSlices);
  bn_colsum_kernel<0><<<grid, block, 0, st>>>(x, x_ld, x_off, nullptr, 0, 0, nullptr, 0, 0, nullptr, nullptr, 0.f, 0, part,
                                              pixels, channels, rpc);
  YNB_COUNT_LAUNCH();
  bn_reduce_finalize_kernel<<<(channels + 31) / 32, dim3(32, kRedSlices), 0, st>>>(part, chunks, pixels, channels, eps, momentum,
                                                                                sums, save_mean, save_rstd, running_mean,
                                                                                running_var);
  YNB_COUNT_LAUNCH();
  const long long total = pixels * (channels / 4);
  const int blocks = (int)std::min<long long>((total + 255) / 256, (long long)kNumSMs * 16);
  bn_apply_kernel<0><<<blocks, 256, 0, st>>>(x, x_ld, x_off, nullptr, 0, 0, nullptr, 0, 0, y, y_ld, y_off, gamma, beta,
                                             save_mean, save_rstd, nullptr, act == YNB_ACT_LEAKY ? 0.1f : 0.0f, act, pixels,
                                             channels);
  YNB_COUNT_LAUNCH();
  UNIT_TRY(cudaGetLastError());
  return YNB_OK;
}

YNB_EXPORT int ynb_bn_train_bwd(const float* dy, int32_t dy_ld, int32_t dy_off, const float* x, int32_t x_ld, int32_t x_off,
                                const float* y, int32_t y_ld, int32_t y_off, const float* gamma, const float* save_mean,
                                const float* save_rstd, float* dx, int32_t dx_ld, int32_t dx_off, float* dgamma_dbeta,
                                int64_t pixels, int32_t channels, int32_t act, void* ws, int64_t ws_bytes, void* stream) {
  if (!bn_args_ok(pixels, channels, {dy_ld, dy_off, x_ld, x_off, dx_ld, dx_off},
                  {dy, x, gamma, save_mean, save_rstd, dx, dgamma_dbeta, ws}) ||
      ws_bytes < ynb_bn_workspace_bytes(pixels, channels) || act < 0 || act > 2 ||
      (act != YNB_ACT_NONE && (!y || y_ld % 4 || y_off % 4)))
    return fail(nullptr, YNB_ERR_INVALID, "ynb_bn_train_bwd: bad arguments (channels / strides multiples of 4, 16-byte aligned)");
  cudaStream_t st = (cudaStream_t)stream;
  const int chunks = bn_chunks(pixels);
  const long long rpc = (pixels + chunks - 1) / chunks;
  float* part = (float*)ws;
  float* sums = part + (long long)chunks * 2 * channels;
  const float slope = act == YNB_ACT_LEAKY ? 0.1f : 0.0f;
  dim3 grid(chunks, (channels + kBnCg * 4 - 1) / (kBnCg * 4)), block(kBnCg, kBnSlices);
  bn_colsum_kernel<1><<<grid, block, 0, st>>>(x, x_ld, x_off, dy, dy_ld, dy_off, y, y_ld, y_off, save_mean, save_rstd, slope,
                                              act != YNB_ACT_NONE, part, pixels, channels, rpc);
  YNB_COUNT_LAUNCH();
  launch_reduce_partials(part, chunks, 2LL * channels, sums, st);
  const long long total = pixels * (channels / 4);
  const int blocks = (int)std::min<long long>((total + 255) / 256, (long long)kNumSMs * 16);
  bn_apply_kernel<1><<<blocks, 256, 0, st>>>(x, x_ld, x_off, dy, dy_ld, dy_off, y, y_ld, y_off, dx, dx_ld, dx_off, gamma,
                                             nullptr, save_mean, save_rstd, sums, slope, act, pixels, channels);
  YNB_COUNT_LAUNCH();
  UNIT_TRY(cudaMemcpyAsync(dgamma_dbeta, sums + channels, channels * sizeof(float), cudaMemcpyDeviceToDevice, st));
  UNIT_TRY(cudaMemcpyAsync(dgamma_dbeta + channels, sums, channels * sizeof(float), cudaMemcpyDeviceToDevice, st));
  UNIT_TRY(cudaGetLastError());
  return YNB_OK;
}
```

Before: 35350.

## Add 2-CTA cluster pair mode for tcgen05 GEMM with split weight loads

Adds a paired-CTA (cta_group::2) variant of the tcgen05 GEMM kernel. Two CTAs in a cluster share one MMA issued by the leader over a 256-row M tile, and each CTA loads half of the weight rows. TMEM allocation, commits and barriers are made cluster-aware, and grid sizing moves out of the call sites into the planner. The aim is to halve per-CTA weight smem and traffic and to use the larger 2-CTA MMA shape. The cost is cross-CTA synchronisation and a more complex barrier protocol.

```diff
diff --git a/yolo_nano_b200/csrc/common.cuh b/yolo_nano_b200/csrc/common.cuh
--- a/yolo_nano_b200/csrc/common.cuh
+++ b/yolo_nano_b200/csrc/common.cuh
@@ -64,19 +64,36 @@
 }
 
 template <typename... KArgs, typename... Args>
-inline cudaError_t launch_pdl(void (*kern)(KArgs...), dim3 grid, dim3 block, size_t smem, cudaStream_t st,
-                              Args&&... args) {
+inline cudaError_t launch_pdl_cluster(unsigned cluster_x, void (*kern)(KArgs...), dim3 grid, dim3 block, size_t smem,
+                                      cudaStream_t st, Args&&... args) {
   cudaLaunchConfig_t cfg{};
   cfg.gridDim = grid;
   cfg.blockDim = block;
   cfg.dynamicSmemBytes = smem;
   cfg.stream = st;
-  cudaLaunchAttribute attr[1];
-  attr[0].id = cudaLaunchAttributeProgrammaticStreamSerialization;
-  attr[0].val.programmaticStreamSerializationAllowed = 1;
+  cudaLaunchAttribute attr[2];
+  int n = 0;
+  if (pdl_enabled()) {
+    attr[n].id = cudaLaunchAttributeProgrammaticStreamSerialization;
+    attr[n].val.programmaticStreamSerializationAllowed = 1;
+    ++n;
+  }
+  if (cluster_x > 1) {
+    attr[n].id = cudaLaunchAttributeClusterDimension;
+    attr[n].val.clusterDim.x = cluster_x;
+    attr[n].val.clusterDim.y = 1;
+    attr[n].val.clusterDim.z = 1;
+    ++n;
+  }
   cfg.attrs = attr;
-  cfg.numAttrs = pdl_enabled() ? 1 : 0;
+  cfg.numAttrs = n;
   return cudaLaunchKernelEx(&cfg, kern, static_cast<KArgs>(args)...);
+}
+
+template <typename... KArgs, typename... Args>
+inline cudaError_t launch_pdl(void (*kern)(KArgs...), dim3 grid, dim3 block, size_t smem, cudaStream_t st,
+                              Args&&... args) {
+  return launch_pdl_cluster(1u, kern, grid, block, smem, st, static_cast<Args&&>(args)...);
 }
 
 #define YNB_COUNT_LAUNCH()                  \
diff --git a/yolo_nano_b200/csrc/gemm_tc.cuh b/yolo_nano_b200/csrc/gemm_tc.cuh
--- a/yolo_nano_b200/csrc/gemm_tc.cuh
+++ b/yolo_nano_b200/csrc/gemm_tc.cuh
@@ -1,6 +1,7 @@
 #pragma once
 #include <cuda.h>
 
+#include <algorithm>
 #include <cstring>
 
 #include "common.cuh"
@@ -38,6 +39,7 @@
   int presplit;
   int a2_step;
   int stack_b;
+  int pair;
   int acc_stages;
   uint32_t tmem_cols;
   uint32_t a_box_bytes;
@@ -66,7 +68,7 @@
 #define YNB_TRACE(role, a, b)                                                                        \
   do {                                                                                               \
     if (p.trace != nullptr && blockIdx.x == 0) {                                                     \
-      const int _lt = (int)(((long long)(a) - (long long)blockIdx.x) / (long long)gridDim.x) & 63;   \
+      const int _lt = (int)(((long long)(a) - (long long)tile0) / (long long)tstep) & 63;            \
       long long* _e = p.trace + 1 + (long long)((((role) * 64 + _lt) * 32) + ((int)(b) & 31)) * 4;   \
       _e[0] = (role); _e[1] = (a); _e[2] = (b); _e[3] = clock64();                                   \
     }                                                                                                \
@@ -101,13 +103,22 @@
 
 __host__ __device__ __forceinline__ uint32_t rn_tf32_bits(uint32_t u) { return (u + 0x1000u) & 0xffffe000u; }
 
-template <bool kPass, int kDecC>
+template <bool kPass, int kDecC, bool kPair = false>
 __global__ void __launch_bounds__(kTcThreads, 1)
 tc_gemm_kernel(const __grid_constant__ CUtensorMap tmA, const __grid_constant__ CUtensorMap tmAlo,
                const __grid_constant__ CUtensorMap tmWhi, const __grid_constant__ CUtensorMap tmWlo,
                const __grid_constant__ CUtensorMap tmOut, const TcGemmParams p) {
+  static_assert(!kPair || kDecC == 0, "pair mode: plain / interleave / merged stride-2 epilogues only");
+  constexpr int CG = kPair ? 2 : 1;
   extern __shared__ __align__(16) uint8_t smem_raw[];
   uint8_t* smem = smem_raw + ((1024u - (ptx::smem_u32(smem_raw) & 1023u)) & 1023u);
+
+  const uint32_t rank = kPair ? ptx::cluster_ctarank() : 0u;
+  const bool leader = rank == 0;
+  const int64_t tile0 = kPair ? (int64_t)(blockIdx.x >> 1) : (int64_t)blockIdx.x;
+  const int64_t tstep = kPair ? (int64_t)(gridDim.x >> 1) : (int64_t)gridDim.x;
+  auto tile_row0 = [&](int64_t tile) { return (kPair ? 2 * tile + rank : tile) * kTcBM; };
+  const int w_rows = kPair ? p.Npad / 2 : p.Npad;
 
   const bool split = p.mode == YNB_GEMM_TC_3XTF32;
   const int kchunk = p.bf16_in ? 64 : kTcBK;
@@ -116,7 +127,7 @@
   const int box_wlo = (p.w_resident || !split) ? -1 : box_whi + 1;
   const int nboxes = 1 + (box_alo >= 0) + (box_whi >= 0) + (box_wlo >= 0);
   const int nprod = nboxes < kTcProducers ? nboxes : kTcProducers;
-  const TcSmemLayout lay = tc_smem_layout(p.Npad, p.num_steps, p.num_stages, p.w_resident != 0, split);
+  const TcSmemLayout lay = tc_smem_layout(w_rows, p.num_steps, p.num_stages, p.w_resident != 0, split);
   const uint32_t w_chunk_bytes = lay.w_chunk_bytes;
   const uint32_t a_bytes = kTcAStageBytes * (split ? 2 : 1);
   const uint32_t stage_bytes = lay.stage_bytes;
@@ -134,6 +145,8 @@
   const int warp = threadIdx.x >> 5, lane = threadIdx.x & 31;
   pdl_trigger();
 
+  const bool splitters_on = split && !p.presplit;
+  const int ready_warps = splitters_on ? 4 : 1;
   if (warp == kTcProducerWarp && lane == 0) {
     ptx::prefetch_tmap(&tmA);
     if (p.presplit || p.a2_step > 0) ptx::prefetch_tmap(&tmAlo);
@@ -142,25 +155,26 @@
     if (p.tma_store) ptx::prefetch_tmap(&tmOut);
     for (int s = 0; s < p.num_stages; ++s) {
       ptx::mbar_init(&full[s], nprod);
-      ptx::mbar_init(&ready[s], 4);
+      ptx::mbar_init(&ready[s], ready_warps * CG);
       ptx::mbar_init(&empty[s], 1);
     }
     for (int a = 0; a < 2; ++a) {
       ptx::mbar_init(&tmem_full[a], 1);
-      ptx::mbar_init(&tmem_empty[a], 4);
+      ptx::mbar_init(&tmem_empty[a], 4 * CG);
     }
-    ptx::mbar_init(w_full, 1);
+    ptx::mbar_init(w_full, kPair && leader ? 2 : 1);
     ptx::fence_barrier_init();
   }
   if (warp == kTcMmaWarp) {
-    ptx::tmem_alloc(tmem_ptr, p.tmem_cols);
-    ptx::tmem_relinquish();
+    ptx::tmem_alloc<CG>(tmem_ptr, p.tmem_cols);
+    ptx::tmem_relinquish<CG>();
   }
   if (warp < 4) {
     for (int i = threadIdx.x; i < p.Npad; i += 128) s_bias[i] = i < p.N ? __ldg(p.bias + i) : 0.0f;
   }
   ptx::tc_fence_before_sync();
-  __syncthreads();
+  if constexpr (kPair) ptx::cluster_sync();
+  else __syncthreads();
   ptx::tc_fence_after_sync();
   const uint32_t tmem_base = *tmem_ptr;
 
@@ -174,13 +188,13 @@
 
   const int acc_cols = p.Npad * p.nacc;
   const uint32_t step_tx = p.a_box_bytes * (p.presplit ? 2 : 1) + (p.w_resident ? 0 : w_chunk_bytes * (split ? 2 : 1));
-  const bool splitters_on = split && !p.presplit;
+  const int w_row0 = (int)rank * w_rows;
 
   if (warp == kTcProducerWarp && p.w_resident && ptx::elect_one()) {
     ptx::mbar_arrive_expect_tx(w_full, w_res_bytes);
     for (int st = 0; st < p.num_steps; ++st) {
-      ptx::tma_load_2d(w_hi_ptr(0, st), &tmWhi, w_full, st * kchunk, 0);
-      if (split) ptx::tma_load_2d(w_lo_ptr(0, st), &tmWlo, w_full, st * kchunk, 0);
+      ptx::tma_load_2d(w_hi_ptr(0, st), &tmWhi, w_full, st * kchunk, w_row0);
+      if (split) ptx::tma_load_2d(w_lo_ptr(0, st), &tmWlo, w_full, st * kchunk, w_row0);
     }
   }
   pdl_wait();
@@ -197,7 +211,7 @@
       int s = 0;
       uint32_t ph = 0;
       bool ok = true;
-      for (int64_t tile = blockIdx.x; tile < p.num_tiles && ok; tile += gridDim.x) {
+      for (int64_t tile = tile0; tile < p.num_tiles && ok; tile += tstep) {
         int b = 0, y0 = 0, x0 = 0;
         if (p.is3x3) {
           int per_img = p.tiles_x * p.tiles_y;
@@ -219,28 +233,34 @@
             if (do_a) {
               const bool second = p.a2_step > 0 && st >= p.a2_step;
               ptx::tma_load_2d(stage_a(s), second ? &tmAlo : &tmA, &full[s], (second ? st - p.a2_step : st) * kchunk,
-                               (int)(tile * kTcBM));
+                               (int)tile_row0(tile));
             }
           }
-          if (do_whi) ptx::tma_load_2d(w_hi_ptr(s, st), &tmWhi, &full[s], st * kchunk, 0);
-          if (do_wlo) ptx::tma_load_2d(w_lo_ptr(s, st), &tmWlo, &full[s], st * kchunk, 0);
+          if (do_whi) ptx::tma_load_2d(w_hi_ptr(s, st), &tmWhi, &full[s], st * kchunk, w_row0);
+          if (do_wlo) ptx::tma_load_2d(w_lo_ptr(s, st), &tmWlo, &full[s], st * kchunk, w_row0);
           if (prole == 0) YNB_TRACE(1, tile, st);
           if (++s == p.num_stages) { s = 0; ph ^= 1; }
         }
       }
     }
   } else if (warp == kTcMmaWarp) {
-    if (ptx::elect_one()) {
-      const uint32_t idesc = ptx::make_idesc(2 , kTcBM, p.Npad);
+    if (kPair && !leader) {
+      if (p.w_resident && ptx::elect_one() && ptx::mbar_wait(w_full, 0, p.err_flag, 2)) ptx::mbar_arrive_cluster(w_full, 0);
+    } else if (ptx::elect_one()) {
+      const uint32_t idesc = ptx::make_idesc(2 , kTcBM * CG, p.Npad);
       const uint32_t idesc2 = ptx::make_idesc(2, kTcBM, 2 * p.Npad);
-      const uint32_t idesc_bf = ptx::make_idesc(1 , kTcBM, p.Npad);
+      const uint32_t idesc_bf = ptx::make_idesc(1 , kTcBM * CG, p.Npad);
+      auto commit = [&](uint64_t* bar) {
+        if constexpr (kPair) ptx::mma_commit_pair(bar, 0x3);
+        else ptx::mma_commit(bar);
+      };
       int s = 0;
       uint32_t ph = 0;
       int acc = 0;
       uint32_t acc_ph = 0;
       bool ok = true;
       if (p.w_resident) ok = ptx::mbar_wait(w_full, 0, p.err_flag, 2);
-      for (int64_t tile = blockIdx.x; tile < p.num_tiles && ok; tile += gridDim.x) {
+      for (int64_t tile = tile0; tile < p.num_tiles && ok; tile += tstep) {
         ok = ptx::mbar_wait(&tmem_empty[acc], acc_ph ^ 1, p.err_flag, 3);
         if (!ok) break;
         ptx::tc_fence_after_sync();
@@ -248,7 +268,7 @@
         const uint32_t c_tmem = p.merge_corr ? d_tmem : d_tmem + (uint32_t)(p.nmain * p.Npad);
         int t = 0;
         for (int st = 0; st < p.num_steps; ++st) {
-          ok = ptx::mbar_wait(splitters_on ? &ready[s] : &full[s], ph, p.err_flag, 4);
+          ok = ptx::mbar_wait((splitters_on || kPair) ? &ready[s] : &full[s], ph, p.err_flag, 4);
           if (!ok) break;
           ptx::tc_fence_after_sync();
           const uint32_t a_hi = ptx::smem_u32(stage_a(s));
@@ -260,16 +280,23 @@
 #pragma unroll
             for (int k = 0; k < kTcBK / 8; ++k, ++t) {
               if (k >= nk) break;
-              ptx::mma_bf16_ss(d_tmem, ptx::make_sw128_kmajor_desc(a_hi + k * 32), ptx::make_sw128_kmajor_desc(b_hi + k * 32),
-                               idesc_bf, t != 0);
+              ptx::mma_bf16_ss<CG>(d_tmem, ptx::make_sw128_kmajor_desc(a_hi + k * 32),
+                                   ptx::make_sw128_kmajor_desc(b_hi + k * 32), idesc_bf, t != 0);
             }
           } else if (p.stack_b) {
 #pragma unroll
             for (int k = 0; k < kTcBK / 8; ++k, ++t) {
               if (k >= nk) break;
+              const uint64_t da = ptx::make_sw128_kmajor_desc(a_hi + k * 32);
               const uint64_t db = ptx::make_sw128_kmajor_desc(b_hi + k * 32);
-              ptx::mma_tf32_ss(d_tmem, ptx::make_sw128_kmajor_desc(a_hi + k * 32), db, idesc2, t != 0);
-              ptx::mma_tf32_ss(c_tmem, ptx::make_sw128_kmajor_desc(a_lo + k * 32), db, idesc, 1);
+              if constexpr (kPair) {
+                ptx::mma_tf32_ss<CG>(c_tmem, da, ptx::make_sw128_kmajor_desc(b_lo + k * 32), idesc, t != 0);
+                ptx::mma_tf32_ss<CG>(c_tmem, ptx::make_sw128_kmajor_desc(a_lo + k * 32), db, idesc, 1);
+                ptx::mma_tf32_ss<CG>(d_tmem, da, db, idesc, t != 0);
+              } else {
+                ptx::mma_tf32_ss(d_tmem, da, db, idesc2, t != 0);
+                ptx::mma_tf32_ss(c_tmem, ptx::make_sw128_kmajor_desc(a_lo + k * 32), db, idesc, 1);
+              }
             }
           } else {
 #pragma unroll
@@ -280,48 +307,53 @@
               const uint64_t db = ptx::make_sw128_kmajor_desc(b_hi + ko);
               const int slot = t % p.nmain;
               if (split) {
-                ptx::mma_tf32_ss(c_tmem, ptx::make_sw128_kmajor_desc(a_lo + ko), db, idesc, t != 0);
-                ptx::mma_tf32_ss(c_tmem, da, ptx::make_sw128_kmajor_desc(b_lo + ko), idesc, 1);
+                ptx::mma_tf32_ss<CG>(c_tmem, ptx::make_sw128_kmajor_desc(a_lo + ko), db, idesc, t != 0);
+                ptx::mma_tf32_ss<CG>(c_tmem, da, ptx::make_sw128_kmajor_desc(b_lo + ko), idesc, 1);
               }
-              ptx::mma_tf32_ss(d_tmem + (uint32_t)(slot * p.Npad), da, db, idesc,
-                               (split && p.merge_corr) ? 1 : (t >= p.nmain));
+              ptx::mma_tf32_ss<CG>(d_tmem + (uint32_t)(slot * p.Npad), da, db, idesc,
+                                   (split && p.merge_corr) ? 1 : (t >= p.nmain));
             }
           }
           YNB_TRACE(3, tile, st);
-          ptx::mma_commit(&empty[s]);
-          if (st == p.num_steps - 1) ptx::mma_commit(&tmem_full[acc]);
+          commit(&empty[s]);
+          if (st == p.num_steps - 1) commit(&tmem_full[acc]);
           if (++s == p.num_stages) { s = 0; ph ^= 1; }
         }
         if (++acc == p.acc_stages) { acc = 0; acc_ph ^= 1; }
       }
     }
   } else if (warp >= kTcSplitWarp0 && warp < kTcSplitWarp0 + 4) {
-    if (splitters_on) {
+    if (splitters_on || (kPair && warp == kTcSplitWarp0)) {
       const int t = threadIdx.x - kTcSplitWarp0 * 32;
       int s = 0;
       uint32_t ph = 0;
       bool ok = true;
-      for (int64_t tile = blockIdx.x; tile < p.num_tiles && ok; tile += gridDim.x) {
+      for (int64_t tile = tile0; tile < p.num_tiles && ok; tile += tstep) {
         for (int st = 0; st < p.num_steps; ++st) {
           ok = ptx::mbar_wait(&full[s], ph, p.err_flag, 5);
           if (!ok) break;
-          uint4* a = reinterpret_cast<uint4*>(stage_a(s));
-          uint4* lo = reinterpret_cast<uint4*>(stage_alo(s));
-#pragma unroll
-          for (int i = 0; i < kTcAStageBytes / 16 / 128; ++i) {
-            const uint4 v = a[t + i * 128];
-            uint4 h, l;
-            h.x = rn_tf32_bits(v.x); h.y = rn_tf32_bits(v.y); h.z = rn_tf32_bits(v.z); h.w = rn_tf32_bits(v.w);
-            l.x = rn_tf32_bits(__float_as_uint(__uint_as_float(v.x) - __uint_as_float(h.x)));
-            l.y = rn_tf32_bits(__float_as_uint(__uint_as_float(v.y) - __uint_as_float(h.y)));
-            l.z = rn_tf32_bits(__float_as_uint(__uint_as_float(v.z) - __uint_as_float(h.z)));
-            l.w = rn_tf32_bits(__float_as_uint(__uint_as_float(v.w) - __uint_as_float(h.w)));
-            a[t + i * 128] = h;
-            lo[t + i * 128] = l;
-          }
-          ptx::fence_proxy_async_smem();
+          if (splitters_on) {
+            uint4* a = reinterpret_cast<uint4*>(stage_a(s));
+            uint4* lo = reinterpret_cast<uint4*>(stage_alo(s));
+#pragma unroll
+            for (int i = 0; i < kTcAStageBytes / 16 / 128; ++i) {
+              const uint4 v = a[t + i * 128];
+              uint4 h, l;
+              h.x = rn_tf32_bits(v.x); h.y = rn_tf32_bits(v.y); h.z = rn_tf32_bits(v.z); h.w = rn_tf32_bits(v.w);
+              l.x = rn_tf32_bits(__float_as_uint(__uint_as_float(v.x) - __uint_as_float(h.x)));
+              l.y = rn_tf32_bits(__float_as_uint(__uint_as_float(v.y) - __uint_as_float(h.y)));
+              l.z = rn_tf32_bits(__float_as_uint(__uint_as_float(v.z) - __uint_as_float(h.z)));
+              l.w = rn_tf32_bits(__float_as_uint(__uint_as_float(v.w) - __uint_as_float(h.w)));
+              a[t + i * 128] = h;
+              lo[t + i * 128] = l;
+            }
+            ptx::fence_proxy_async_smem();
+          }
           __syncwarp();
-          if (lane == 0) ptx::mbar_arrive(&ready[s]);
+          if (lane == 0) {
+            if constexpr (kPair) ptx::mbar_arrive_cluster(&ready[s], 0);
+            else ptx::mbar_arrive(&ready[s]);
+          }
           if (t == 0) YNB_TRACE(2, tile, st);
           if (++s == p.num_stages) { s = 0; ph ^= 1; }
         }
@@ -335,13 +367,12 @@
     const float slope = p.act == YNB_ACT_RELU ? 0.0f : (p.act == YNB_ACT_LEAKY ? 0.1f : 1.0f);
     uint8_t* sbox = smem + lay.stg_off + warp * 4096;
     const int sw = lane & 7;
-    const int nloc = (int64_t)blockIdx.x < p.num_tiles
-                         ? (int)((p.num_tiles - blockIdx.x + gridDim.x - 1) / gridDim.x) : 0;
+    const int nloc = tile0 < p.num_tiles ? (int)((p.num_tiles - tile0 + tstep - 1) / tstep) : 0;
     const bool share_last = kDecC == 0;
     const int col_split = min(p.Npad, ((p.Npad / 2 + 31) / 32) * 32);
     bool ok = true;
     for (int lt = 0; lt < nloc && ok; ++lt) {
-      const int64_t tile = blockIdx.x + (int64_t)lt * gridDim.x;
+      const int64_t tile = tile0 + (int64_t)lt * tstep;
       const int acc = p.acc_stages == 2 ? (lt & 1) : 0;
       const bool shared = share_last && lt == nloc - 1 && col_split < p.Npad;
       if (!shared && group != acc) {
@@ -362,10 +393,10 @@
         valid = row < p.TH * p.TW && y < p.H && x < p.W;
         m = ((int64_t)b * p.H + y) * p.W + x;
       } else {
-        m = tile * kTcBM + row;
+        m = tile_row0(tile) + row;
         valid = m < p.M;
       }
-      const int64_t m_base = tile * kTcBM + q * 32;
+      const int64_t m_base = tile_row0(tile) + q * 32;
       float xa[16], xb[16];
       const int rows_left = (int)min((int64_t)32, p.M - m_base);
       auto fetch_x1 = [&](int c0, int r0, float (&x)[16]) {
@@ -553,7 +584,10 @@
         if (c0 + 32 >= col_end && !shared) {
           ptx::tc_fence_before_sync();
           __syncwarp();
-          if (lane == 0) ptx::mbar_arrive(&tmem_empty[acc]);
+          if (lane == 0) {
+            if constexpr (kPair) ptx::mbar_arrive_cluster(&tmem_empty[acc], 0);
+            else ptx::mbar_arrive(&tmem_empty[acc]);
+          }
         }
         if (!kPass && p.tma_store) {
           ptx::fence_proxy_async_smem();
@@ -614,10 +648,11 @@
   }
 
   ptx::tc_fence_before_sync();
-  __syncthreads();
+  if constexpr (kPair) ptx::cluster_sync();
+  else __syncthreads();
   if (warp == kTcMmaWarp) {
     ptx::tc_fence_after_sync();
-    ptx::tmem_dealloc(tmem_base, p.tmem_cols);
+    ptx::tmem_dealloc<CG>(tmem_base, p.tmem_cols);
   }
 }
 
@@ -719,6 +754,7 @@
   CUtensorMap tmOut;
   const TcWeights* w = nullptr;
   CUtensorMap tmAlo;
+  CUtensorMap tmWhi, tmWlo;
   TcGemmParams p;
   uint32_t smem = 0;
   unsigned grid = 0;
@@ -760,18 +796,17 @@
   p.stack_b = (split && !no_stack && p.nmain == 1 && p.nacc == 2 && 2 * p.Npad <= 256 && (2 * p.Npad) % 16 == 0) ? 1 : 0;
 }
 
-inline bool tc_plan_smem(TcGemmLaunch& L) {
-  TcGemmParams& p = L.p;
+inline bool tc_plan_stages(const TcGemmParams& p, int w_rows, int* stages_out, int* resident_out, uint32_t* smem_out) {
   const bool split = p.mode == YNB_GEMM_TC_3XTF32;
   for (int resident = 1; resident >= 0; --resident) {
     for (int stages = kTcMaxStages; stages >= 2; --stages) {
       if (stages > p.num_steps * 4 && stages > 2) continue;
-      TcSmemLayout lay = tc_smem_layout(p.Npad, p.num_steps, stages, resident != 0, split);
+      TcSmemLayout lay = tc_smem_layout(w_rows, p.num_steps, stages, resident != 0, split);
       static const bool res2 = getenv("YNB_TC_RES2") != nullptr;
       if (lay.total <= (uint32_t)kTcSmemBudget && (resident == 0 || stages >= 3 || p.num_steps <= 2 || res2)) {
-        p.num_stages = stages;
-        p.w_resident = resident;
-        L.smem = lay.total;
+        *stages_out = stages;
+        *resident_out = resident;
+        *smem_out = lay.total;
         return true;
       }
     }
@@ -779,23 +814,84 @@
   return false;
 }
 
-inline cudaError_t launch_tc_gemm(const TcGemmLaunch& L, cudaStream_t st) {
-  using KernelT = void (*)(CUtensorMap, CUtensorMap, CUtensorMap, CUtensorMap, CUtensorMap, TcGemmParams);
-  static const KernelT kernels[4] = {tc_gemm_kernel<false, 0>, tc_gemm_kernel<true, 0>, tc_gemm_kernel<false, 80>,
-                                     tc_gemm_kernel<false, 20>};
+using TcKernelT = void (*)(CUtensorMap, CUtensorMap, CUtensorMap, CUtensorMap, CUtensorMap, TcGemmParams);
+
+inline TcKernelT tc_kernel_for(const TcGemmLaunch& L) {
+  static const TcKernelT kernels[6] = {tc_gemm_kernel<false, 0>,       tc_gemm_kernel<true, 0>,
+                                       tc_gemm_kernel<false, 80>,      tc_gemm_kernel<false, 20>,
+                                       tc_gemm_kernel<false, 0, true>, tc_gemm_kernel<true, 0, true>};
   static bool attr_set = false;
   if (!attr_set) {
-    for (KernelT k : kernels) {
-      cudaError_t e = cudaFuncSetAttribute(k, cudaFuncAttributeMaxDynamicSharedMemorySize, kTcSmemBudget);
-      if (e != cudaSuccess) return e;
-    }
+    for (TcKernelT k : kernels)
+      if (cudaFuncSetAttribute(k, cudaFuncAttributeMaxDynamicSharedMemorySize, kTcSmemBudget) != cudaSuccess) return nullptr;
     attr_set = true;
   }
+  if (L.dec_classes == 80) return kernels[2];
+  if (L.dec_classes == 20) return kernels[3];
+  return kernels[(L.p.pair ? 4 : 0) + (L.p.pass != nullptr ? 1 : 0)];
+}
+
+inline bool tc_plan_smem(TcGemmLaunch& L) {
+  TcGemmParams& p = L.p;
+  int stages = 0, resident = 0;
+  uint32_t smem = 0;
+  if (!tc_plan_stages(p, p.Npad, &stages, &resident, &smem)) return false;
+  p.num_stages = stages;
+  p.w_resident = resident;
+  p.pair = 0;
+  L.smem = smem;
+  L.grid = (unsigned)std::min<int64_t>(p.num_tiles, kNumSMs);
+
+  const bool pair_shape = !p.is3x3 && !p.presplit && L.dec_classes == 0 && !p.merge_corr && p.Npad % 16 == 0 &&
+                          L.w != nullptr && getenv("YNB_TC_NO_PAIR") == nullptr;
+  int pstages = 0, president = 0;
+  uint32_t psmem = 0;
+  if (!pair_shape || !tc_plan_stages(p, p.Npad / 2, &pstages, &president, &psmem) ||
+      !((president && !resident) || pstages > stages))
+    return true;
+  TcGemmLaunch Lp = L;
+  Lp.p.pair = 1;
+  const TcKernelT kern = tc_kernel_for(Lp);
+  if (kern == nullptr) return false;
+  cudaLaunchConfig_t cfg{};
+  cfg.gridDim = dim3(kNumSMs);
+  cfg.blockDim = dim3(kTcThreads);
+  cfg.dynamicSmemBytes = psmem;
+  cudaLaunchAttribute attr[1];
+  attr[0].id = cudaLaunchAttributeClusterDimension;
+  attr[0].val.clusterDim.x = 2;
+  attr[0].val.clusterDim.y = 1;
+  attr[0].val.clusterDim.z = 1;
+  cfg.attrs = attr;
+  cfg.numAttrs = 1;
+  int slots = 0;
+  if (cudaOccupancyMaxActiveClusters(&slots, kern, &cfg) != cudaSuccess) return false;
+  if (slots <= 0) return true;
+  const TcWeights& w = *L.w;
+  const bool bf = p.bf16_in != 0, split = p.mode == YNB_GEMM_TC_3XTF32;
+  if (!make_tmap_2d(&L.tmWhi, bf ? (const void*)w.bw : (const void*)w.hi, w.Kpad, w.Npad, w.Kpad, w.Npad / 2, bf))
+    return false;
+  if (split) {
+    if (!make_tmap_2d(&L.tmWlo, w.lo, w.Kpad, w.Npad, w.Kpad, w.Npad / 2)) return false;
+  } else {
+    L.tmWlo = L.tmWhi;
+  }
+  p.pair = 1;
+  p.num_stages = pstages;
+  p.w_resident = president;
+  p.num_tiles = (p.M + 2 * kTcBM - 1) / (2 * kTcBM);
+  L.smem = psmem;
+  L.grid = 2 * (unsigned)std::min<int64_t>(p.num_tiles, slots);
+  return true;
+}
+
+inline cudaError_t launch_tc_gemm(const TcGemmLaunch& L, cudaStream_t st) {
+  const TcKernelT kern = tc_kernel_for(L);
+  if (kern == nullptr) return cudaErrorInvalidDeviceFunction;
   const CUtensorMap& tmo = L.p.tma_store ? L.tmOut : L.tmA;
-  KernelT kern = L.dec_classes == 80 ? kernels[2] : (L.dec_classes == 20 ? kernels[3] : kernels[L.p.pass != nullptr ? 1 : 0]);
   const CUtensorMap& tmalo = (L.p.presplit || L.p.a2_step > 0) ? L.tmAlo : L.tmA;
-  cudaError_t r = launch_pdl(kern, dim3(L.grid), dim3(kTcThreads), (size_t)L.smem, st, L.tmA, tmalo, L.w->tm_hi,
-                             L.w->tm_lo, tmo, L.p);
+  cudaError_t r = launch_pdl_cluster(L.p.pair ? 2u : 1u, kern, dim3(L.grid), dim3(kTcThreads), (size_t)L.smem, st, L.tmA,
+                                     tmalo, L.p.pair ? L.tmWhi : L.w->tm_hi, L.p.pair ? L.tmWlo : L.w->tm_lo, tmo, L.p);
   YNB_COUNT_LAUNCH();
   return r;
 }
diff --git a/yolo_nano_b200/csrc/ptx_sm100.cuh b/yolo_nano_b200/csrc/ptx_sm100.cuh
--- a/yolo_nano_b200/csrc/ptx_sm100.cuh
+++ b/yolo_nano_b200/csrc/ptx_sm100.cuh
@@ -33,6 +33,20 @@
       : "r"(smem_u32(bar)), "r"(parity)
       : "memory");
   return ok != 0;
+}
+
+__device__ __forceinline__ uint32_t cluster_ctarank() {
+  uint32_t r;
+  asm volatile("mov.u32 %0, %%cluster_ctarank;" : "=r"(r));
+  return r;
+}
+__device__ __forceinline__ void mbar_arrive_cluster(uint64_t* bar, uint32_t rank) {
+  uint32_t remote;
+  asm volatile("mapa.shared::cluster.u32 %0, %1, %2;" : "=r"(remote) : "r"(smem_u32(bar)), "r"(rank));
+  asm volatile("mbarrier.arrive.shared::cluster.b64 _, [%0];" ::"r"(remote) : "memory");
+}
+__device__ __forceinline__ void cluster_sync() {
+  asm volatile("barrier.cluster.arrive.release.aligned;\n\tbarrier.cluster.wait.acquire.aligned;" ::: "memory");
 }
 __device__ __forceinline__ uint64_t globaltimer_ns() {
   uint64_t t;
@@ -115,16 +129,28 @@
   asm volatile("cp.async.bulk.wait_group %0;" ::"n"(N) : "memory");
 }
 
+template <int CG = 1>
 __device__ __forceinline__ void tmem_alloc(uint32_t* smem_result, uint32_t ncols) {
-  asm volatile("tcgen05.alloc.cta_group::1.sync.aligned.shared::cta.b32 [%0], %1;" ::"r"(smem_u32(smem_result)),
-               "r"(ncols)
-               : "memory");
-}
+  if constexpr (CG == 2)
+    asm volatile("tcgen05.alloc.cta_group::2.sync.aligned.shared::cta.b32 [%0], %1;" ::"r"(smem_u32(smem_result)),
+                 "r"(ncols)
+                 : "memory");
+  else
+    asm volatile("tcgen05.alloc.cta_group::1.sync.aligned.shared::cta.b32 [%0], %1;" ::"r"(smem_u32(smem_result)),
+                 "r"(ncols)
+                 : "memory");
+}
+template <int CG = 1>
 __device__ __forceinline__ void tmem_relinquish() {
-  asm volatile("tcgen05.relinquish_alloc_permit.cta_group::1.sync.aligned;" ::: "memory");
-}
+  if constexpr (CG == 2) asm volatile("tcgen05.relinquish_alloc_permit.cta_group::2.sync.aligned;" ::: "memory");
+  else asm volatile("tcgen05.relinquish_alloc_permit.cta_group::1.sync.aligned;" ::: "memory");
+}
+template <int CG = 1>
 __device__ __forceinline__ void tmem_dealloc(uint32_t taddr, uint32_t ncols) {
-  asm volatile("tcgen05.dealloc.cta_group::1.sync.aligned.b32 %0, %1;" ::"r"(taddr), "r"(ncols) : "memory");
+  if constexpr (CG == 2)
+    asm volatile("tcgen05.dealloc.cta_group::2.sync.aligned.b32 %0, %1;" ::"r"(taddr), "r"(ncols) : "memory");
+  else
+    asm volatile("tcgen05.dealloc.cta_group::1.sync.aligned.b32 %0, %1;" ::"r"(taddr), "r"(ncols) : "memory");
 }
 
 __device__ __forceinline__ uint64_t make_sw128_kmajor_desc(uint32_t smem_addr) {
@@ -140,27 +166,51 @@
   return (1u << 4) | ((uint32_t)fmt << 7) | ((uint32_t)fmt << 10) | ((uint32_t)(N >> 3) << 17) |
          ((uint32_t)(M >> 4) << 24);
 }
+template <int CG = 1>
 __device__ __forceinline__ void mma_tf32_ss(uint32_t tmem_d, uint64_t adesc, uint64_t bdesc, uint32_t idesc,
                                             uint32_t accumulate) {
-  asm volatile(
-      "{\n\t.reg .pred p;\n\t"
-      "setp.ne.b32 p, %4, 0;\n\t"
-      "tcgen05.mma.cta_group::1.kind::tf32 [%0], %1, %2, %3, p;\n\t}"
-      ::"r"(tmem_d), "l"(adesc), "l"(bdesc), "r"(idesc), "r"(accumulate)
-      : "memory");
-}
+  if constexpr (CG == 2)
+    asm volatile(
+        "{\n\t.reg .pred p;\n\t"
+        "setp.ne.b32 p, %4, 0;\n\t"
+        "tcgen05.mma.cta_group::2.kind::tf32 [%0], %1, %2, %3, p;\n\t}"
+        ::"r"(tmem_d), "l"(adesc), "l"(bdesc), "r"(idesc), "r"(accumulate)
+        : "memory");
+  else
+    asm volatile(
+        "{\n\t.reg .pred p;\n\t"
+        "setp.ne.b32 p, %4, 0;\n\t"
+        "tcgen05.mma.cta_group::1.kind::tf32 [%0], %1, %2, %3, p;\n\t}"
+        ::"r"(tmem_d), "l"(adesc), "l"(bdesc), "r"(idesc), "r"(accumulate)
+        : "memory");
+}
+template <int CG = 1>
 __device__ __forceinline__ void mma_bf16_ss(uint32_t tmem_d, uint64_t adesc, uint64_t bdesc, uint32_t idesc,
                                             uint32_t accumulate) {
-  asm volatile(
-      "{\n\t.reg .pred p;\n\t"
-      "setp.ne.b32 p, %4, 0;\n\t"
-      "tcgen05.mma.cta_group::1.kind::f16 [%0], %1, %2, %3, p;\n\t}"
-      ::"r"(tmem_d), "l"(adesc), "l"(bdesc), "r"(idesc), "r"(accumulate)
-      : "memory");
+  if constexpr (CG == 2)
+    asm volatile(
+        "{\n\t.reg .pred p;\n\t"
+        "setp.ne.b32 p, %4, 0;\n\t"
+        "tcgen05.mma.cta_group::2.kind::f16 [%0], %1, %2, %3, p;\n\t}"
+        ::"r"(tmem_d), "l"(adesc), "l"(bdesc), "r"(idesc), "r"(accumulate)
+        : "memory");
+  else
+    asm volatile(
+        "{\n\t.reg .pred p;\n\t"
+        "setp.ne.b32 p, %4, 0;\n\t"
+        "tcgen05.mma.cta_group::1.kind::f16 [%0], %1, %2, %3, p;\n\t}"
+        ::"r"(tmem_d), "l"(adesc), "l"(bdesc), "r"(idesc), "r"(accumulate)
+        : "memory");
 }
 __device__ __forceinline__ void mma_commit(uint64_t* bar) {
   asm volatile("tcgen05.commit.cta_group::1.mbarrier::arrive::one.shared::cluster.b64 [%0];" ::"r"(smem_u32(bar))
                : "memory");
+}
+__device__ __forceinline__ void mma_commit_pair(uint64_t* bar, uint16_t cta_mask) {
+  asm volatile(
+      "tcgen05.commit.cta_group::2.mbarrier::arrive::one.shared::cluster.multicast::cluster.b64 [%0], %1;"
+      ::"r"(smem_u32(bar)), "h"(cta_mask)
+      : "memory");
 }
 
 __device__ __forceinline__ void tmem_ld_32x32(uint32_t taddr, uint32_t (&r)[32]) {
diff --git a/yolo_nano_b200/csrc/ynb_api.cu b/yolo_nano_b200/csrc/ynb_api.cu
--- a/yolo_nano_b200/csrc/ynb_api.cu
+++ b/yolo_nano_b200/csrc/ynb_api.cu
@@ -583,7 +583,6 @@
       return;
     }
     if (!tc_plan_smem(L)) { error = "no smem configuration for " + name; return; }
-    L.grid = (unsigned)std::min<int64_t>(p.num_tiles, kNumSMs);
     const TcGemmLaunch* Lp = &L;
     const double obytes = dec ? abytes - (double)out.es * M * c.cout + 24.0 * M * 3 : abytes;
     Op op{dec ? name + "+decode" : name, dec ? "pw_decode_tcgen05" : "pw_tcgen05", obytes, aflops,
@@ -631,7 +630,6 @@
         return true;
       }
       if (!tc_plan_smem(L)) { error = "no smem configuration for the merged stride-2 conv of " + unit; return true; }
-      L.grid = (unsigned)std::min<int64_t>(p.num_tiles, kNumSMs);
       const TcGemmLaunch* Lp = &L;
       const double frac = (double)cc.pc.n / out.ld;
       const double bytes = (double)b1dw.es * M * (c1.cin + c2.cin) + (double)out.es * M * 2.0 * c1.cout * frac +
@@ -738,7 +736,6 @@
     }
     p.presplit = presplit ? 1 : 0;
     if (!tc_plan_smem(L)) { error = "no smem configuration for " + name; return; }
-    L.grid = (unsigned)std::min<int64_t>(p.num_tiles, kNumSMs);
     const TcGemmLaunch* Lp = &L;
     plan->net.push_back({name, "conv3x3_tcgen05", eb * M * (c.cin + c.cout) + wbytes, aflops,
                          [=](cudaStream_t st) { return launch_tc_gemm(*Lp, st); }});
@@ -1582,7 +1579,6 @@
       !make_tmap_2d(&L.tmA, in + in_off, cin, pixels, in_ld, kTcBM) || !tc_plan_smem(L)) {
     rc = fail(nullptr, YNB_ERR_CUDA, "ynb_pwconv_tc: tensor map / smem planning failed");
   } else {
-    L.grid = (unsigned)std::min<int64_t>(p.num_tiles, kNumSMs);
     cudaError_t r = launch_tc_gemm(L, st);
     if (r == cudaSuccess) r = cudaStreamSynchronize(st);
     int flag = 0;
@@ -1594,8 +1590,8 @@
       cudaMemcpy(h.data(), d_trace, h.size() * 8, cudaMemcpyDeviceToHost);
       int n = 0;
       for (int i = 0; i < trace_cap; ++i) n += h[4 + 4 * i] != 0;
-      fprintf(stderr, "YNB_TC_TRACE stages=%d resident=%d nmain=%d acc_stages=%d steps=%d grid=%u events=%d\n",
-              p.num_stages, p.w_resident, p.nmain, p.acc_stages, p.num_steps, L.grid, n);
+      fprintf(stderr, "YNB_TC_TRACE stages=%d resident=%d pair=%d nmain=%d acc_stages=%d steps=%d grid=%u events=%d\n",
+              p.num_stages, p.w_resident, p.pair, p.nmain, p.acc_stages, p.num_steps, L.grid, n);
       for (int i = 0; i < trace_cap; ++i)
         if (h[4 + 4 * i] != 0)
           fprintf(stderr, "TRACE %lld %lld %lld %lld\n", h[1 + 4 * i], h[2 + 4 * i], h[3 + 4 * i], h[4 + 4 * i]);
@@ -2221,7 +2217,6 @@
       !make_tmap_nhwc(&L.tmA, in, cin, w_, h, batch, in_ld, p.TW, p.TH) || !tc_plan_smem(L)) {
     rc = fail(nullptr, YNB_ERR_CUDA, "ynb_conv3x3_tc: tensor map / smem planning failed");
   } else {
-    L.grid = (unsigned)std::min<int64_t>(p.num_tiles, kNumSMs);
     cudaError_t r = launch_tc_gemm(L, st);
     if (r == cudaSuccess) r = cudaStreamSynchronize(st);
     int flag = 0;
@@ -2297,7 +2292,6 @@
                                      (uint64_t)out_ld)) ||
       !make_tmap_2d(&L.tmA, in + in_off, cin, pixels, in_ld, kTcBM) || !tc_plan_smem(L))
     return fail(nullptr, YNB_ERR_CUDA, "ynb_pwconv_tc_async: tensor map / smem planning failed");
-  L.grid = (unsigned)std::min<int64_t>(p.num_tiles, kNumSMs);
   UNIT_TRY(launch_tc_gemm(L, st));
   return YNB_OK;
 }
@@ -2341,7 +2335,6 @@
       !make_tmap_2d(&t.tm_lo, t.lo, t.Kpad, t.Npad, t.Kpad, t.Npad) ||
       !make_tmap_nhwc(&L.tmA, in, cin, w_, h, batch, in_ld, p.TW, p.TH) || !tc_plan_smem(L))
     return fail(nullptr, YNB_ERR_CUDA, "ynb_conv3x3_tc_async: tensor map / smem planning failed");
-  L.grid = (unsigned)std::min<int64_t>(p.num_tiles, kNumSMs);
   UNIT_TRY(launch_tc_gemm(L, st));
   return YNB_OK;
 }
```

New measurement: 36310 (median of 6 runs). 1.03x the previous value.
